# AlbertoEsc/PyFaceAnalysis

Measured on AMD Instinct MI355X. Metric: 128x128 sub-images/sec through 11L HiGSFA net, higher is better.
Workload: dtype f32; 1 GPU; configs[1]: U11L-128 (11-layer net, trained random-init weights), 4096 synthetic 128x128 sub-images per GPU per step, float32 input resident in HBM, first 20 slow features out; rows_per_gpu=4096, global_rows=4096, plan=fused, parallelism=row-shard x1

## Files before the change

### pyfaceanalysis_amd/csrc/hg_fused.hip

```cpp
#include <hip/hip_runtime.h>

#include <algorithm>
#include <cmath>
#include <cstdlib>
#include <map>
#include <sstream>
#include <tuple>

#include "hg_fused_dev.hpp"

namespace hg {

namespace {

using namespace fused;

#ifndef HG_A_PINGPONG
#define HG_A_PINGPONG 1
#endif
#ifdef HIGSFA_DIAG
#define HG_HOT(blk) ((P.whatif & 1) ? ((blk) & 1) : (blk))
#else
#define HG_HOT(blk) (blk)
#endif
// ... 348 lines not shown
#pragma unroll
                                for (int t = 0; t < T; ++t) z[t] = MFMA16(a1[k][r], bf[k][t][r], z[t]);
                            }
                    }
                }
            }
        }
        if (rem1) {
#pragma unroll
            for (int t = 0; t < T; ++t) add_rem4(z[t], d4[t]);
        }
        if (!P.has_exp) {
#pragma unroll
            for (int t = 0; t < T; ++t)
                if (tile[t] < P.n_tiles) P.out[((size_t)tile[t] * P.nb_out + node * P.mto + w) * 64 + lane] = z[t];
            return;
        }
        for (int fi = 0; fi < nf; ++fi) {
            const int fk = (P.funcp >> (4 * fi)) & 15;
            const float ex = P.expo[fi];
#pragma unroll
            for (int t = 0; t < T; ++t) smem[((fi * mt1n + w) * T + t) * 64 + lane] = apply_func_uniform(fk, ex, z[t]);
        }
    } else if (!P.has_exp) {
        return;
    }
    __syncthreads();
    if (w >= mt2n) return;
#pragma unroll
    for (int t = 0; t < T; ++t) d4[t] = f32x4{0.f, 0.f, 0.f, 0.f};
    f32x4 y[T];
    {
        const f32x4 bb = *(const f32x4*)(bnode + (mt1n + w) * 16);
#pragma unroll
        for (int t = 0; t < T; ++t) y[t] = bb;
    }
#pragma unroll
    for (int k = 0; k < KB; ++k) {
        if (k >= k2n) continue;
        const int mt1 = k / nf, fi = k - mt1 * nf;
        const int nk = (P.nk2p[mt1] >> (4 * fi)) & 15;
        f32x4 e[T];
#pragma unroll
        for (int t = 0; t < T; ++t) e[t] = smem[((fi * mt1n + mt1) * T + t) * 64 + lane];
        if (REM && rem2) {
#pragma unroll
            for (int r = 0; r < 4; ++r)
                if (r < nk) {
#pragma unroll
                    for (int t = 0; t < T; ++t) d4[t] = MFMA4(a2[k][r], e[t][r], d4[t]);
                }
        } else if (nk == 4) {
#pragma unroll
            for (int r = 0; r < 4; ++r)
#pragma unroll
                for (int t = 0; t < T; ++t) y[t] = MFMA16(a2[k][r], e[t][r], y[t]);
        } else {
#pragma unroll
            for (int r = 0; r < 4; ++r)
                if (r < nk) {
#pragma unroll
                    for (int t = 0; t < T; ++t) y[t] = MFMA16(a2[k][r], e[t][r], y[t]);
                }
        }
    }
    if (rem2) {
#pragma unroll
        for (int t = 0; t < T; ++t) add_rem4(y[t], d4[t]);
    }
    if (REM && P.pack_base > 0) {
        if (rem2) {
            const int slot = __builtin_amdgcn_readfirstlane(P.pack_slot[node]);
#pragma unroll
            for (int t = 0; t < T; ++t)
                if (tile[t] < P.n_tiles) *packed_slot_ptr(P, tile[t], slot, lane) = y[t][0];
        } else {
#pragma unroll
            for (int t = 0; t < T; ++t)
                if (tile[t] < P.n_tiles) P.out[((size_t)tile[t] * P.nb_out + node * (mt2n - 1) + w) * 64 + lane] = y[t];
        }
        return;
    }
#pragma unroll
    for (int t = 0; t < T; ++t)
        if (tile[t] < P.n_tiles) P.out[((size_t)tile[t] * P.nb_out + node * P.mto + w) * 64 + lane] = y[t];
}

template <typename YT>
__global__ void k_unpack(const float* __restrict__ act, int nb, const int32_t* __restrict__ col_base, YT* __restrict__ y,
                         int64_t ldy, int64_t n, int cols) {
    int64_t total = n * cols;
    for (int64_t idx = (int64_t)blockIdx.x * blockDim.x + threadIdx.x; idx < total; idx += (int64_t)gridDim.x * blockDim.x) {
        int64_t row = idx / cols;
        int c = (int)(idx - row * cols);
        int64_t tile = row >> 4;
        int jj = (int)(row & 15);
        y[row * ldy + c] = (YT)act[tile * nb * 256 + col_base[c] + jj * 4];
    }
}


template <int MT1, int MT2>
StageFn pick_stage_t(int T) {
    if (T == 2) return k_stage<MT1, MT2, 2>;
    return k_stage<MT1, MT2, 1>;
}
template <int MT1>
StageFn pick_stage_m2(int mt2, int T) {
    switch (mt2) {
        case 1: return pick_stage_t<MT1, 1>(T);
        case 2: return pick_stage_t<MT1, 2>(T);
        case 3: return pick_stage_t<MT1, 3>(T);
        default: return pick_stage_t<MT1, 4>(T);
    }
}
StageFn pick_stage(int mt1, int mt2, int T, bool rem = false, int kbf = 0, bool fs = false, int pk = -1) {
    if (pk >= 0) {
        if (pk == 1 && kbf == 3 && T == 2 && rem && mt1 == 3 && mt2 == 3) return fs ? (StageFn)k_stage<3, 3, 2, false, true, 3, true, 1> : (StageFn)k_stage<3, 3, 2, false, true, 3, false, 1>;
        if (pk == 1 && kbf == 3 && T == 2 && rem && mt1 == 2 && mt2 == 2) return (StageFn)k_stage<2, 2, 2, false, true, 3, false, 1>;
        return nullptr;
    }
    if (fs) {
        if (kbf == 3 && T == 2 && rem && mt1 == 3 && mt2 == 3) return (StageFn)k_stage<3, 3, 2, false, true, 3, true>;
        if (kbf == 4 && T == 2 && !rem && mt1 == 3 && mt2 == 3) return (StageFn)k_stage<3, 3, 2, false, false, 4, true>;
        if (kbf == 0 && !rem && mt1 == 4 && mt2 == 4) return T == 2 ? (StageFn)k_stage<4, 4, 2, false, false, 0, true> : (StageFn)k_stage<4, 4, 1, false, false, 0, true>;
    }
    if (kbf == 4 && T == 2) {
        if (rem && mt1 == 3 && mt2 == 3) return (StageFn)k_stage<3, 3, 2, false, true, 4>;
        if (rem && mt1 == 2 && mt2 == 2) return (StageFn)k_stage<2, 2, 2, false, true, 4>;
        if (!rem && mt1 == 3 && mt2 == 3) return (StageFn)k_stage<3, 3, 2, false, false, 4>;
        if (!rem && mt1 == 2 && mt2 == 2) return (StageFn)k_stage<2, 2, 2, false, false, 4>;
    }
    if (kbf == 3 && T == 2) {
        if (rem && mt1 == 3 && mt2 == 3) return (StageFn)k_stage<3, 3, 2, false, true, 3>;
        if (rem && mt1 == 2 && mt2 == 2) return (StageFn)k_stage<2, 2, 2, false, true, 3>;
    }
    if (rem) {
        if (mt1 == 3 && mt2 == 3) return T == 2 ? (StageFn)k_stage<3, 3, 2, false, true> : (StageFn)k_stage<3, 3, 1, false, true>;
        if (mt1 == 2 && mt2 == 2) return T == 2 ? (StageFn)k_stage<2, 2, 2, false, true> : (StageFn)k_stage<2, 2, 1, false, true>;
    }
    switch (mt1) {
        case 1: return pick_stage_m2<1>(mt2, T);
        case 2: return pick_stage_m2<2>(mt2, T);
        case 3: return pick_stage_m2<3>(mt2, T);
        default: return pick_stage_m2<4>(mt2, T);
    }
}


constexpr int kWeightLdsKiB = 64;

struct StageDev {
    DevBuf afrag, bias, kb1tab, chunks, runs, piece, koff, kmean, kcol, gcol, etab, pack_slot;
};
struct SubRunDev {
    DevBuf nodes[kMaxTail], tab[kMaxTail];
};

struct WorkQueue {
    DevBuf ctr;
    uint32_t base = 0;
};

constexpr int kMaxLanes = 2;
struct Lane {
    DevBuf bufA, bufB;
    int64_t cap_rows = 0;
    WorkQueue wq_front, wq_direct, wq_direct_wg;
    int32_t* err_host = nullptr;
    int32_t* err_dev = nullptr;
};

class FusedExecutor : public Executor {
public:
    explicit FusedExecutor(std::unique_ptr<const FusedPlan> plan) : plan_(std::move(plan)) {}

    int plan_kind() const override { return HG_PLAN_FUSED; }
    int n_stages() const override { return (int)plan_->stages.size() + 1; }
    std::string stage_name(int i) const override {
        if (i < (int)plan_->stages.size()) return plan_->stages[i].name;
        return plan_->tail_begin >= 0 ? std::string("row-major y written by the top-of-hierarchy launch (no unpack pass)")
                                      : std::string("fused unpack (fragment order -> row-major y)");
    }
    std::string describe() const override {
        std::ostringstream os;
        os << "plan: FUSED (fragment-order activations, v_mfma_f32_16x16x4_f32)\n";
        for (int i = 0; i < n_stages(); ++i) os << "  [" << i << "] " << stage_name(i) << "\n";
        return os.str();
    }
    int64_t weight_bytes() const override {
        int64_t t = 0;
        for (auto& s : plan_->stages) t += (int64_t)(s.afrag.size() + s.bias.size()) * 4;
        return t;
    }
    int64_t padded_flops_per_row() const override { return plan_->padded_flops_given; }
    int64_t workspace_bytes() const override {
        int64_t t = 0;
        for (int l = 0; l < n_lanes_; ++l) t += (int64_t)(lanes_[l].bufA.bytes + lanes_[l].bufB.bytes);
        return t;
    }

    void to_device() override {
        dev_.resize(plan_->stages.size());
        for (size_t si = 0; si < dev_.size(); ++si) {
            const HostStage& s = plan_->stages[si];
            StageDev& d = dev_[si];
            d.afrag.upload(s.afrag.data(), s.afrag.size() * 4);
            d.bias.upload(s.bias.data(), s.bias.size() * 4);
            if (!s.kb1tab.empty()) d.kb1tab.upload(s.kb1tab.data(), s.kb1tab.size() * 4);
            if (!s.gcol.empty()) d.gcol.upload(s.gcol.data(), s.gcol.size() * 4);
            if (!s.etab.empty()) d.etab.upload(s.etab.data(), s.etab.size() * 4);
            if (!s.pack_slot.empty()) d.pack_slot.upload(s.pack_slot.data(), s.pack_slot.size() * 4);
            if (!s.chunks.empty()) {
                d.chunks.upload(s.chunks.data(), s.chunks.size() * sizeof(DChunk));
                d.runs.upload(s.runs.data(), s.runs.size() * sizeof(DRun));
                d.piece.upload(s.piece_col.data(), s.piece_col.size() * 4);
                d.koff.upload(s.koff.data(), s.koff.size() * 4);
                d.kmean.upload(s.kmean.data(), s.kmean.size() * 4);
                if (!s.kcol.empty()) d.kcol.upload(s.kcol.data(), s.kcol.size() * 4);
            }
        }
        sub_dev_.resize(plan_->sub_runs.size());
        for (size_t ri = 0; ri < sub_dev_.size(); ++ri) {
            const SubRun& r = plan_->sub_runs[ri];
            for (int k = 0; k < r.len; ++k) {
                sub_dev_[ri].nodes[k].upload(r.nodes[k].data(), r.nodes[k].size() * 4);
                if (k > 0) sub_dev_[ri].tab[k].upload(r.tab[k].data(), r.tab[k].size() * 4);
            }
        }
        d_col_base_.upload(plan_->col_base.data(), plan_->col_base.size() * 4);
        d_col_of_.upload(plan_->col_of.data(), plan_->col_of.size() * 4);
        int dev = 0;
        hipDeviceProp_t prop;
        if (hipGetDevice(&dev) == hipSuccess && hipGetDeviceProperties(&prop, dev) == hipSuccess && prop.multiProcessorCount > 0)
            n_cus_ = prop.multiProcessorCount;
    }

    void reserve(int64_t rows) override {
        for (int l = 0; l < n_lanes_; ++l) reserve_lane(lanes_[l], rows);
    }

    bool set_lanes(int n) override {
        if (n < 1 || n > kMaxLanes) return false;
        for (int l = n; l < n_lanes_; ++l) release_lane(lanes_[l]);
        for (int l = n_lanes_; l < n; ++l) reserve_lane(lanes_[l], lanes_[0].cap_rows);
        n_lanes_ = n;
        return true;
    }
    int lanes() const override { return n_lanes_; }

    void run(const void* x, int x_dtype, int64_t n, int64_t ldx, void* y, int y_dtype, int64_t y_cols, int64_t ldy,
             hipStream_t st, hipEvent_t* ev) override {
        run_in(lanes_[0], x, x_dtype, n, ldx, y, y_dtype, y_cols, ldy, st, ev);
    }
    void run_lane(int lane, const void* x, int x_dtype, int64_t n, int64_t ldx, void* y, int y_dtype, int64_t y_cols, int64_t ldy,
                  hipStream_t st) override {
        if (lane < 0 || lane >= n_lanes_) fail(HG_ERR_ARG, "lane %d outside 0..%d", lane, n_lanes_ - 1);
        run_in(lanes_[lane], x, x_dtype, n, ldx, y, y_dtype, y_cols, ldy, st, nullptr);
    }

    void run_in(Lane& L, const void* x, int x_dtype, int64_t n, int64_t ldx, void* y, int y_dtype, int64_t y_cols, int64_t ldy,
                hipStream_t st, hipEvent_t* ev) {
        check_device_error();
        if (dev_.size() != plan_->stages.size()) fail(HG_ERR_STATE, "fused: the plan is not on a device");
        if (n > L.cap_rows) {
            if (n_lanes_ > 1) HG_HIP(hipStreamSynchronize(st));
            reserve_lane(L, n);
        }
        run_range(L, x, x_dtype, n, ldx, y, y_dtype, y_cols, ldy, st, ev);
    }

    void run_range(Lane& L, const void* x, int x_dtype, int64_t n, int64_t ldx, void* y, int y_dtype, int64_t y_cols, int64_t ldy,
                   hipStream_t st, hipEvent_t* ev) {
        const int n_tiles = (int)((n + 15) / 16);
        const int sub_set = plan_->pick_sub_set(n_tiles);
        int e = 0;
        auto record = [&](int k) {
            if (ev)
                for (int i = 0; i < k; ++i) HG_HIP(hipEventRecord(ev[e++], st));
        };
        record(1);
        f32x4* cur = (f32x4*)L.bufA.p;
        f32x4* nxt = (f32x4*)L.bufB.p;
        for (int si = 0; si < (int)plan_->stages.size(); ++si) {
            if (plan_->tail_begin >= 0 && si == plan_->tail_start(n_tiles)) {
                launch_top(si, cur, n_tiles, y, y_dtype, y_cols, ldy, n, st);
                record((int)plan_->stages.size() + 1 - si);
                HG_HIP(hipGetLastError());
                return;
            }
            const SubRun* sr = nullptr;
            const SubRunDev* sd = nullptr;
            for (size_t ri = 0; ri < plan_->sub_runs.size(); ++ri) {
                const SubRun& r = plan_->sub_runs[ri];
                if (r.begin == si && r.set == sub_set && plan_->sub_run_pays(r, n_tiles)) { sr = &r; sd = &sub_dev_[ri]; }
            }
            if (sr) {
                launch_subtrees(*sr, *sd, cur, nxt, n_tiles, st);
                std::swap(cur, nxt);
                record(sr->len);
                si += sr->len - 1;
                continue;
            }
            const HostStage& s = plan_->stages[si];
            const StageDev& d = dev_[si];
            StageParams P = stage_params(s, d, cur, nxt, n_tiles);
            int covered = 1;
            if (s.kind == 1)
                launch_im2frag(x, x_dtype, ldx, n, n_tiles, s.nb_out, (const int32_t*)d.gcol.p, nxt, vec4_ok(s, x, ldx, x_dtype) ? 1 : 0, st);
            else if (s.kind == 2)
                launch_igsfa(s, P, n_tiles, si, st);
            else if (s.from_x)
                covered = launch_front(L, s, d, P, x, x_dtype, ldx, n, n_tiles, cur, st) ? 2 : 1;
            else if (s.kind == 3)
                launch_prod(s, d, P, n_tiles, st);
            else if (!launch_splitm(s, P, n_tiles, st))
                launch_stage(s, P, n_tiles, si, st);
            if (covered == 1) std::swap(cur, nxt);
            record(covered);
            si += covered - 1;
        }
        launch_unpack(cur, n, y, y_dtype, y_cols, ldy, st);
        record(1);
        HG_HIP(hipGetLastError());
    }

    void release() override {
        for (Lane& L : lanes_) release_lane(L);
        n_lanes_ = 1;
        d_col_base_.free();
        d_col_of_.free();
        sub_dev_.clear();
        dev_.clear();
    }

private:
    void reserve_lane(Lane& L, int64_t rows) {
        int64_t tiles = (rows + 15) / 16;
        size_t need = (size_t)tiles * plan_->max_nb * 1024;
        L.bufA.alloc(need);
        L.bufB.alloc(need);
        L.cap_rows = std::max(L.cap_rows, tiles * 16);
    }
    void release_lane(Lane& L) {
        L.bufA.free();
        L.bufB.free();
        L.wq_front.ctr.free();
        L.wq_direct.ctr.free();
        L.wq_direct_wg.ctr.free();
        L.wq_front.base = L.wq_direct.base = L.wq_direct_wg.base = 0;
        if (L.err_host) (void)hipHostFree(L.err_host);
        L.err_host = nullptr;
        L.err_dev = nullptr;
        L.cap_rows = 0;
    }

    int resident_blocks(StageFn fn, int threads, size_t lds) {
        set_lds_limit(fn, lds);
        auto key = std::make_tuple((const void*)fn, threads, lds);
        auto it = occ_.find(key);
        if (it != occ_.end()) return it->second;
        int nb = 0;
        if (hipOccupancyMaxActiveBlocksPerMultiprocessor(&nb, (const void*)fn, threads, lds) != hipSuccess || nb < 1) nb = 1;
        occ_[key] = nb;
        return nb;
    }

    uint32_t* work_counters(WorkQueue& q, int n, hipStream_t st) {
        const size_t need = (size_t)n * 64;
        if (q.ctr.bytes < need) {
            q.ctr.alloc(std::max<size_t>(need, 64 * 1024));
            HG_HIP(hipMemsetD32Async((hipDeviceptr_t)q.ctr.p, (int)plan_->opt.wq_start, q.ctr.bytes / 4, st));
            q.base = plan_->opt.wq_start;
        }
        return (uint32_t*)q.ctr.p;
    }

    int32_t* device_error_word(Lane& L) {
        if (!L.err_host) {
            HG_HIP(hipHostMalloc((void**)&L.err_host, 64, hipHostMallocMapped));
            *L.err_host = 0;
            HG_HIP(hipHostGetDevicePointer((void**)&L.err_dev, L.err_host, 0));
        }
        return L.err_dev;
    }
    void check_errors() override { check_device_error(); }
    void check_device_error() {
        for (const Lane& L : lanes_)
            if (L.err_host && *(volatile int32_t*)L.err_host != 0)
                fail(HG_ERR_DEVICE, "fused: a bounded poll in a persistent kernel ran out (code %d); the features of that call are invalid", (int)*L.err_host);
    }

    void set_lds_limit(StageFn fn, size_t bytes) {
        if (bytes <= 64 * 1024) return;
        if (bytes > 160 * 1024) fail(HG_ERR_FORMAT, "fused: a node needs %zu bytes of LDS (> 160 KiB)", bytes);
        auto it = lds_set_.find((const void*)fn);
        if (it != lds_set_.end() && it->second >= bytes) return;
        HG_HIP(hipFuncSetAttribute((const void*)fn, hipFuncAttributeMaxDynamicSharedMemorySize, (int)(160 * 1024)));
        lds_set_[(const void*)fn] = 160 * 1024;
    }

    StageParams stage_params(const HostStage& hs, const StageDev& d, const f32x4* in, f32x4* out, int n_tiles) const {
        StageParams R{};
        R.afrag = (const f32x4*)d.afrag.p;
        R.bias = (const float*)d.bias.p;
        R.kb1tab = (const int2*)d.kb1tab.p;
        R.in = in;
        R.out = out;
        R.n_nodes = hs.n_nodes;
        R.kb1 = hs.kb1;
        R.nf = hs.nf;
        R.has_exp = hs.has_exp ? 1 : 0;
        R.node_blocks = hs.node_blocks;
        R.bias_floats = hs.bias_floats;
        R.n_tiles = n_tiles;
        R.nb_in = hs.nb_in;
        R.nb_out = hs.nb_out;
        R.mto = hs.mto;
        R.pack_base = hs.pack_out ? hs.n_nodes * (hs.mto - 1) : 0;
        R.pack_soa = hs.pack_soa ? 1 : 0;
        R.pack_in = hs.pack_in;
        R.pack_slot = (const int32_t*)d.pack_slot.p;
        R.a4x4 = hs.rem4 ? 1 : 0;
        R.sum_in = hs.sum_in ? 1 : 0;
        R.n_kids = hs.n_kids;
        for (int fi = 0; fi < hs.nf; ++fi) {
            R.funcp |= (uint32_t)hs.funcs[fi].kind << (4 * fi);
            R.expo[fi] = (float)hs.funcs[fi].expo;
            for (int mt1 = 0; mt1 < hs.mt1; ++mt1) R.nk2p[mt1] |= (uint32_t)hs.nk2[mt1][fi] << (4 * fi);
        }
        return R;
    }

    static bool vec4_ok(const HostStage& s, const void* x, int64_t ldx, int x_dtype) {
        const size_t esz = dtype_size(x_dtype), valign = x_dtype == HG_U8 ? 4 : 16;
        return s.vec_ok && ldx % 4 == 0 && ((uintptr_t)x % valign) == 0 && (ldx * esz) % valign == 0;
    }

    struct Shape {
        int nw, T;
    };
    template <size_t N>
    static Shape sweep_shape(const int (&cand)[N][2], int n_tiles, int n_groups) {
        Shape sh{4, 1};
        for (auto& c : cand) {
            const int64_t tg = (n_tiles + c[0] * c[1] - 1) / (c[0] * c[1]);
            if (c[0] * c[1] <= n_tiles && tg * n_groups >= 256) {
                sh = {c[0], c[1]};
                break;
            }
        }
        while (sh.nw * sh.T > std::max(n_tiles, 1) && sh.nw > 1) sh.nw >>= 1;
        return sh;
    }

    static int sweep_tile_parts(int n_groups, int tile_groups, int occ) {
        const double capacity = 256.0 * occ;
        const int64_t g8 = (int64_t)(n_groups + 7) / 8 * 8;
        int tile_parts = 1;
        double best = 1e300;
        for (int pp = 1; pp <= tile_groups; ++pp) {
            const double rounds = std::ceil(g8 * pp / capacity);
            const double cost = rounds * (0.35 + (double)((tile_groups + pp - 1) / pp));
            if (cost < best - 1e-9) {
                best = cost;
                tile_parts = pp;
            }
        }
        return tile_parts;
    }

    void launch_top(int si, const f32x4* in, int n_tiles, void* y, int y_dtype, int64_t y_cols, int64_t ldy, int64_t n, hipStream_t st) {
        TailParams TP = tail_params(si, in, n_tiles, y, y_dtype, y_cols, ldy, n);
        const int T = (n_tiles >= 512 && tail_waves(TP) <= 8 && tail_lds_bytes(TP, 2) <= (size_t)160 * 1024) ? 2 : 1;
#ifdef HIGSFA_DIAG
        const bool stamped = plan_->opt.stamp_stage == si;
        if (stamped) tail_stamps_begin(TP, (size_t)((n_tiles + T - 1) / T), st);
#endif
        launch_tail(TP, T, st);
#ifdef HIGSFA_DIAG
        if (stamped) tail_stamps_report("top-of-hierarchy launch", si, TP.n_stages, (size_t)((n_tiles + T - 1) / T), st);
#endif
    }

    void launch_subtrees(const SubRun& sr, const SubRunDev& sd, const f32x4* in, f32x4* out, int n_tiles, hipStream_t st) {
        TailParams TP = subtree_params(sr, sd, in, out, n_tiles);
#ifdef HIGSFA_DIAG
        const bool stamped = plan_->opt.stamp_stage == sr.begin;
        if (stamped) tail_stamps_begin(TP, (size_t)sr.n * n_tiles, st);
#endif
        launch_subtree(TP, st);
#ifdef HIGSFA_DIAG
        if (stamped) tail_stamps_report("sub-tree launch", sr.begin, TP.n_stages, (size_t)sr.n * n_tiles, st);
#endif
    }

    void launch_igsfa(const HostStage& s, StageParams& P, int n_tiles, int si, hipStream_t st) {
        if (s.ig_folded && s.n_nodes <= 8 && s.nf <= 2 && s.kb1 <= 8 && (int64_t)s.n_nodes * n_tiles <= 16384) {
            P.ig_folded = 1;
            launch_igfold_split(P, s.mt2, n_tiles, st);
            return;
        }
        const size_t ig_lds = (size_t)s.node_blocks * 1024 + (size_t)s.bias_floats * 4 + (size_t)s.kb1 * 8;
        int nwt = 1, T = 1;
        static const int cand[][2] = {{12, 2}, {8, 2}, {4, 2}};
        for (auto& c : cand) {
            if (c[0] == 12 && (s.ig_folded || !(s.kb1 == 5 || s.kb1 == 6))) continue;
            const int64_t tg = (n_tiles + c[0] * c[1] - 1) / (c[0] * c[1]);
            if (c[0] * c[1] <= std::max(n_tiles, 1) && tg * s.n_nodes >= 256) {
                nwt = c[0];
                T = c[1];
                break;
            }
        }
        if (nwt == 1 && T == 1) {
            T = n_tiles >= 2 ? 2 : 1;
            nwt = n_tiles >= 8 ? 4 : n_tiles >= 4 ? 2 : 1;
        }
        const bool ig_fs = s.ig_folded && s.nf == 2 && s.funcs[0].kind == E_IDENTITY && s.funcs[1].kind == E_ABS_POW && !plan_->opt.no_fspec;
        StageFn fn = s.ig_folded ? pick_igfold(s.mt2, T, ig_fs) : pick_igsfa(s.mt1, s.mt2, T, s.kb1);
        const int ig_occ = resident_blocks(fn, std::max(nwt, 4) * 64, ig_lds);
        const int nw = std::max(nwt, 4);
        P.nodes_per_wg = nwt;
        P.ig_has_lr = s.ig_has_lr ? 1 : 0;
        P.ig_folded = s.ig_folded ? 1 : 0;
        P.nk2p[0] = 0;
        for (int ms = 0; ms < s.mt1; ++ms) P.nk2p[0] |= (uint32_t)s.ig_nks[ms] << (4 * ms);
        P.tile_groups = (n_tiles + nwt * T - 1) / (nwt * T);
        const int npg = 1;
        P.nodes_per_group = npg;
        P.n_chunks = (s.n_nodes + npg - 1) / npg;
        P.tile_parts = std::max(1, std::min(P.tile_groups, 256 * ig_occ / std::max(1, P.n_chunks)));
        set_lds_limit(fn, ig_lds);
        if (plan_->opt.debug) fprintf(stderr, "[igsfa stage %d] nodes %d kb1 %d shape %dx%d occ %d lds %zu tile_groups %d parts %d\n", si, s.n_nodes, s.kb1, nwt, T, ig_occ, ig_lds, P.tile_groups, P.tile_parts);
        hipLaunchKernelGGL(fn, (unsigned)(P.n_chunks * P.tile_parts), nw * 64, ig_lds, st, P);
    }

    bool launch_front(Lane& L, const HostStage& s, const StageDev& d, StageParams& P, const void* x, int x_dtype, int64_t ldx, int64_t n, int n_tiles, f32x4* out1,
                      hipStream_t st) {
        P.chunks = (const DChunk*)d.chunks.p;
        P.runs = (const DRun*)d.runs.p;
        P.piece_col = (const int2*)d.piece.p;
        P.koff = (const int32_t*)d.koff.p;
        P.kmean = (const float*)d.kmean.p;
        P.kcol = (const int32_t*)d.kcol.p;
        P.x = x;
        P.ldx = ldx;
        P.n_rows = n;
        P.lds_stride = s.lds_stride;
        P.nk_last = s.nk_last;
        P.contig4 = s.contig4 ? 1 : 0;
        P.n_chunks = (int)s.chunks.size();
        P.vec4 = vec4_ok(s, x, ldx, x_dtype) ? 1 : 0;
        const int T = (n_tiles >= 4 && s.mt1 * s.mt2 <= 4) ? 4 : 1;
        const int groups = (n_tiles + T - 1) / T;
        const size_t lds_bytes = (size_t)T * 16 * s.lds_stride * 4;
        bool rem4 = false, fspec = false;
        if (plan_->fuse01) {
            rem4 = plan_->stages[1].rem4 || (plan_->stages[1].p_max <= 20 && plan_->stages[1].s_max <= 20 && plan_->stages[1].nk2[1][0] <= 1 &&
                                       plan_->stages[1].nk2[1][1] <= 1 && !plan_->opt.no_rem4);
            auto id_pow = [](const HostStage& hs) { return hs.nf == 2 && hs.funcs[0].kind == E_IDENTITY && hs.funcs[1].kind == E_ABS_POW; };
            fspec = id_pow(s) && id_pow(plan_->stages[1]) && !plan_->opt.no_fspec;
        }
        const int FT = stage01p_tiles(rem4, fspec);
        if (plan_->fuse01 && P.vec4 && n_tiles >= FT) {
            StageParams Q = stage_params(plan_->stages[1], dev_[1], nullptr, out1, n_tiles);
            const size_t esz = dtype_size(x_dtype);
            const bool direct = fspec && rem4 && s.direct_ok && plan_->stages[1].pack_out && (int64_t)16 * ldx * (int64_t)esz + 2048 < 0x7fffffffll && s.max_chunk_nodes <= 8 && !plan_->opt.no_direct;
            const bool wgq = !plan_->opt.no_wgq;
            StageFn2 fn = direct ? pick_stage01d(x_dtype, false, wgq) : pick_stage01p(x_dtype, false, rem4, fspec);
            const int thr01 = 64 * std::max(1, (s.max_chunk_nodes + 1) / 2);
            const size_t lds2 = direct ? (size_t)4 * 160 * 4 + 32 * 4 + (size_t)4 * 256 * 4
                                       : (size_t)(kDoubleBuffer01 ? 2 : 1) * FT * 16 * s.lds_stride * 4 + (size_t)(thr01 / 64) * 160 * 4 + 16;
            const int groups2 = (n_tiles + FT - 1) / FT;
            const int occ = resident_blocks((StageFn)fn, thr01, lds2);
            P.tile_parts = std::max(1, std::min(groups2, 256 * occ / std::max(1, P.n_chunks)));
            if (plan_->opt.debug) fprintf(stderr, "[front] occ %d threads %d lds %zu chunks %d tile_parts %d\n", occ, thr01, lds2, P.n_chunks, P.tile_parts);
#ifdef HIGSFA_DIAG
            if (plan_->opt.stamp_stage == 0 && x_dtype == HG_F32) {
                fn = direct ? pick_stage01d(HG_F32, true, wgq) : pick_stage01p(HG_F32, true, rem4, fspec);
                stamps_begin(P, P.n_chunks * P.tile_parts, 12, st);
            }
#endif
            P.err = device_error_word(L);
            {
                WorkQueue& wq = direct ? (wgq ? L.wq_direct_wg : L.wq_direct) : L.wq_front;
                P.work_ctr = work_counters(wq, direct && !wgq ? plan_->stages[1].n_nodes : P.n_chunks, st);
                P.work_base = wq.base;
                wq.base += (uint32_t)groups2;
            }
#ifdef HIGSFA_DIAG
            if (const char* e = getenv("HIGSFA_WHATIF")) P.whatif = atoi(e);
#endif
            hipLaunchKernelGGL(fn, (unsigned)(P.n_chunks * P.tile_parts), thr01, lds2, st, P, Q);
#ifdef HIGSFA_DIAG
            if (P.stamps) front_stamps_report(P.n_chunks, st);
#endif
            return true;
        }
        const bool persistent = T == 4 && P.vec4 && s.contig4 && s.has_exp && s.mt1 == 1 && s.mt2 == 1 && s.kb1 == 1 &&
                                s.nf <= 2 && s.max_chunk_nodes <= 16 && 64 * s.max_chunk_pieces <= 8 * 512;
        if (persistent) {
            StageFn fn = pick_stage0p(x_dtype);
            const int occ = resident_blocks(fn, 512, lds_bytes);
            P.tile_parts = std::max(1, std::min(groups, 256 * occ / std::max(1, P.n_chunks)));
            hipLaunchKernelGGL(fn, (unsigned)(P.n_chunks * P.tile_parts), 512, lds_bytes, st, P);
        } else {
            const int64_t blocks = (int64_t)groups * P.n_chunks;
            if (blocks > 0x7fffffffll) fail(HG_ERR_ARG, "batch too large");
            StageFn fn = pick_stage0(s.mt1, s.mt2, T, x_dtype);
            set_lds_limit(fn, lds_bytes);
            hipLaunchKernelGGL(fn, (unsigned)blocks, T == 4 ? 512 : 256, lds_bytes, st, P);
        }
        return false;
    }

    bool launch_splitm(const HostStage& s, const StageParams& P, int n_tiles, hipStream_t st) {
        const int T = n_tiles >= 2 * 256 / std::max(1, s.n_nodes) ? 2 : 1;
        const int groups = (n_tiles + T - 1) / T;
        const int64_t wgs = (int64_t)groups * s.n_nodes;
        if (!(s.kind == 0 && (!s.rem4 || s.mt1 == s.mt2) && (s.rem4 || !s.pack_out) && s.mt1 * s.nf <= 8 &&
              (s.n_nodes <= plan_->opt.splitm_max_nodes ? (int64_t)s.n_nodes * n_tiles <= 8192 : wgs <= plan_->opt.splitm_max_wgs)))
            return false;
        const int nwv = std::max(s.mt1, s.has_exp ? s.mt2 : 1);
        const size_t lds_bytes = (size_t)std::max(1, s.nf) * s.mt1 * T * 1024;
        const unsigned grid = (unsigned)(groups * s.n_nodes);
        if (s.rem4) {
            if (T == 2) hipLaunchKernelGGL((k_stage_splitm<2, true>), grid, nwv * 64, lds_bytes, st, P, s.mt1, s.mt2);
            else hipLaunchKernelGGL((k_stage_splitm<1, true>), grid, nwv * 64, lds_bytes, st, P, s.mt1, s.mt2);
        } else if (T == 2)
            hipLaunchKernelGGL(k_stage_splitm<2>, grid, nwv * 64, lds_bytes, st, P, s.mt1, s.mt2);
        else
            hipLaunchKernelGGL(k_stage_splitm<1>, grid, nwv * 64, lds_bytes, st, P, s.mt1, s.mt2);
        return true;
    }

    void launch_stage(const HostStage& s, StageParams& P, int n_tiles, int si, hipStream_t st) {
        const int npg = std::max(1, std::min(s.n_nodes, (s.sum_in ? plan_->opt.sum_lds_kib : kWeightLdsKiB) / std::max(1, s.node_blocks)));
        const int n_groups = (s.n_nodes + npg - 1) / npg;
        static const int shapes[][2] = {{8, 2}, {8, 1}, {4, 2}, {4, 1}};
        const Shape sh = sweep_shape(shapes, n_tiles, n_groups);
        const int nw = sh.nw, T = sh.T;
        const int tile_groups = (n_tiles + nw * T - 1) / (nw * T);
        const size_t lds_bytes = (size_t)npg * s.node_blocks * 1024 + (size_t)npg * s.bias_floats * 4 + (size_t)npg * s.kb1 * 8;
        const int kbf = (T == 2 && s.mt1 == s.mt2 && (s.mt1 == 2 || s.mt1 == 3)) ? (s.kb1 == 4 ? 4 : (s.kb1 == 3 && s.rem4 ? 3 : 0)) : 0;
        const bool fs = s.has_exp && s.nf == 2 && s.funcs[0].kind == E_IDENTITY && s.funcs[1].kind == E_ABS_POW && !plan_->opt.no_fspec;
        StageFn fn = s.pk_kbi >= 0 ? (kbf == 3 ? pick_stage(s.mt1, s.mt2, T, s.rem4, kbf, fs, s.pk_kbi) : nullptr) : pick_stage(s.mt1, s.mt2, T, s.rem4, kbf, fs);
        if (!fn) fn = pick_stage(s.mt1, s.mt2, T, s.rem4, 0, false);
        if (s.sum_in) fn = pick_stage_sum(s.mt1, s.mt2, T, fs);
        const int tile_parts = sweep_tile_parts(n_groups, tile_groups, resident_blocks(fn, nw * 64, lds_bytes));
        P.nodes_per_group = npg;
        P.nodes_per_wg = npg;
        P.n_chunks = n_groups;
        P.pair_chunks = (s.pack_out && !s.pack_soa && npg == 2 && n_groups % 16 == 0) ? 1 : 0;
        P.tile_groups = tile_groups;
        P.tile_parts = tile_parts;
        const int64_t blocks = (int64_t)((P.n_chunks + 7) / 8) * 8 * tile_parts;
        if (blocks > 0x7fffffffll) fail(HG_ERR_ARG, "batch too large");
#ifdef HIGSFA_DIAG
        const bool stamp_kbf3 = s.mt1 == 3 && s.mt2 == 3 && T == 2 && s.rem4 && kbf == 3;
        if (plan_->opt.stamp_stage == si && !s.sum_in && (stamp_kbf3 || (s.mt1 == s.mt2 && (s.mt1 == 4 || s.mt1 == 3) && T == 2 && !s.rem4 && kbf == 0))) {
            fn = stamp_kbf3 ? (StageFn)k_stage<3, 3, 2, true, true, 3> : s.mt1 == 4 ? (StageFn)k_stage<4, 4, 2, true> : (StageFn)k_stage<3, 3, 2, true>;
            stamps_begin(P, (int)blocks, 8, st);
        }
#endif
        set_lds_limit(fn, lds_bytes);
#ifdef HIGSFA_DIAG
        if (const char* e = getenv("HIGSFA_WHATIF")) P.whatif = atoi(e);
#endif
        hipLaunchKernelGGL(fn, (unsigned)blocks, nw * 64, lds_bytes, st, P);
#ifdef HIGSFA_DIAG
        if (P.stamps) stage_stamps_report(si, blocks, nw, st);
#endif
    }

    void launch_unpack(const f32x4* in, int64_t n, void* y, int y_dtype, int64_t y_cols, int64_t ldy, hipStream_t st) {
        const HostStage& last = plan_->stages.back();
        unsigned grid = (unsigned)std::min<int64_t>((n * y_cols + 255) / 256, 4096);
        if (y_dtype == HG_F32)
            hipLaunchKernelGGL(k_unpack<float>, grid, 256, 0, st, (const float*)in, last.nb_out, (const int32_t*)d_col_base_.p,
                               (float*)y, ldy, n, (int)y_cols);
        else if (y_dtype == HG_F64)
            hipLaunchKernelGGL(k_unpack<double>, grid, 256, 0, st, (const float*)in, last.nb_out, (const int32_t*)d_col_base_.p,
                               (double*)y, ldy, n, (int)y_cols);
        else
            fail(HG_ERR_ARG, "output dtype must be f32 or f64");
    }

    void launch_prod(const HostStage& s, const StageDev& d, StageParams& P, int n_tiles, hipStream_t st) {
        static const int shapes[][2] = {{8, 2}, {4, 2}, {4, 1}};
        const Shape sh = sweep_shape(shapes, n_tiles, s.n_nodes);
        const int nw = sh.nw, T = sh.T;
        const size_t zs_bytes = (size_t)nw * T * s.mt1 * 1024, et_bytes = (size_t)s.neb * 128;
        const size_t per_node = (size_t)s.node_blocks * 1024 + (size_t)s.bias_floats * 4 + (size_t)s.kb1 * 8;
        const size_t fixed = zs_bytes + et_bytes;
        const int npg = (int)std::max<size_t>(1, std::min<size_t>(s.n_nodes, fixed + per_node <= 52 * 1024 ? (52 * 1024 - fixed) / per_node : 1));
        const int n_groups = (s.n_nodes + npg - 1) / npg;
        const int tile_groups = (n_tiles + nw * T - 1) / (nw * T);
        const size_t lds_bytes = (size_t)npg * per_node + et_bytes + zs_bytes;
        StageFn fn = pick_prod(s.mt1, s.mt2, T);
        const int tile_parts = sweep_tile_parts(n_groups, tile_groups, resident_blocks(fn, nw * 64, lds_bytes));
        P.nodes_per_group = npg;
        P.nodes_per_wg = npg;
        P.n_chunks = n_groups;
        P.tile_groups = tile_groups;
        P.tile_parts = tile_parts;
        P.etab = (const int2*)d.etab.p;
        P.neb = s.neb;
        P.nk_last = s.nk_last;
        P.has_clip = s.has_clip ? 1 : 0;
        P.clip_lo = s.clip_lo;
        P.clip_hi = s.clip_hi;
        const int64_t blocks = (int64_t)((n_groups + 7) / 8) * 8 * tile_parts;
        if (blocks > 0x7fffffffll) fail(HG_ERR_ARG, "batch too large");
        set_lds_limit(fn, lds_bytes);
        hipLaunchKernelGGL(fn, (unsigned)blocks, nw * 64, lds_bytes, st, P);
    }

#ifdef HIGSFA_DIAG
    void tail_stamps_begin(TailParams& TP, size_t blocks, hipStream_t st) {
        stamp_buf_.alloc(blocks * 16 * 16 * 8);
        HG_HIP(hipMemsetAsync(stamp_buf_.p, 0, stamp_buf_.bytes, st));
        TP.stamps = (unsigned long long*)stamp_buf_.p;
    }
    void tail_stamps_report(const char* what, int si, int n_layers, size_t blocks, hipStream_t st) {
        HG_HIP(hipStreamSynchronize(st));
        std::vector<unsigned long long> h(blocks * 16 * 16);
        HG_HIP(hipMemcpy(h.data(), stamp_buf_.p, h.size() * 8, hipMemcpyDeviceToHost));
        unsigned long long t0 = ~0ull;
        for (size_t i = 0; i < h.size(); i += 16)
            if (h[i]) t0 = std::min(t0, h[i]);
        static const char* names[5] = {"loads in", "expanded", "barrier 1", "outputs stored", "barrier 2"};
        double sum[16] = {}, mx[16] = {}, cnt[16] = {};
        for (size_t i = 0; i < h.size(); i += 16)
            for (int k = 0; k < 16; ++k)
                if (h[i + k]) {
                    const double us = (double)(h[i + k] - t0) * 0.01;
                    sum[k] += us; cnt[k] += 1; mx[k] = std::max(mx[k], us);
                }
        fprintf(stderr, "[stamp stage %d] %s, %zu workgroups: us after the first wave's entry, mean (max) over the waves that took part\n", si, what, blocks);
        fprintf(stderr, "[stamp stage %d]   entry %.2f (%.2f)\n", si, cnt[0] ? sum[0] / cnt[0] : 0.0, mx[0]);
        for (int l = 0; l < n_layers; ++l) {
            fprintf(stderr, "[stamp stage %d]   layer %d:", si, l);
            for (int k = 0; k < 5; ++k) {
                const int q = 1 + 5 * l + k;
                fprintf(stderr, "  %s %.2f (%.2f; %.0f waves)", names[k], cnt[q] ? sum[q] / cnt[q] : 0.0, mx[q], cnt[q]);
            }
            fprintf(stderr, "\n");
        }
    }
    void stamps_begin(StageParams& P, int blocks, int words, hipStream_t st) {
        stamp_blocks_ = blocks;
        stamp_buf_.alloc((size_t)blocks * 8 * words * 8);
        HG_HIP(hipMemsetAsync(stamp_buf_.p, 0, stamp_buf_.bytes, st));
        P.stamps = (unsigned long long*)stamp_buf_.p;
    }
    void front_stamps_report(int n_chunks, hipStream_t st) {
        HG_HIP(hipStreamSynchronize(st));
        std::vector<unsigned long long> h((size_t)stamp_blocks_ * 8 * 12);
        HG_HIP(hipMemcpy(h.data(), stamp_buf_.p, h.size() * 8, hipMemcpyDeviceToHost));
        double a[7] = {0, 0, 0, 0, 0, 0, 0}, nwv = 0;
        unsigned long long lo[3] = {~0ull, ~0ull, ~0ull}, hi[3] = {0, 0, 0};
        for (size_t i = 0; i < h.size(); i += 12)
            if (h[i + 4]) {
                for (int k = 0; k < 7; ++k) a[k] += h[i + k];
                nwv += 1;
                for (int k = 0; k < 3; ++k) { lo[k] = std::min(lo[k], h[i + 7 + k]); hi[k] = std::max(hi[k], h[i + 7 + k]); }
            }
        {
            double xs[8][4] = {}, ps[16][3] = {};
            for (size_t i = 0, w = 0; i < h.size(); i += 12, ++w)
                if (h[i + 4]) {
                    const int blk = (int)(w / 8), xc = blk % 8, pt = std::min(15, blk / n_chunks);
                    const double life = (h[i + 9] - h[i + 8]) * 0.01, clk = (double)h[i + 4] / (double)h[i + 5] * 100.0;
                    xs[xc][0] += 1; xs[xc][1] += life; xs[xc][2] = std::max(xs[xc][2], life); xs[xc][3] += clk;
                    ps[pt][0] += 1; ps[pt][1] += life; ps[pt][2] = std::max(ps[pt][2], life);
                }
            for (int k = 0; k < 8; ++k)
                if (xs[k][0] > 0) fprintf(stderr, "[stamp stage 0+1] xcd %d: waves %.0f loop us mean %.1f max %.1f clock %.0f MHz\n", k, xs[k][0], xs[k][1] / xs[k][0], xs[k][2], xs[k][3] / xs[k][0]);
            for (int k = 0; k < 16; ++k)
                if (ps[k][0] > 0) fprintf(stderr, "[stamp stage 0+1] part %d: waves %.0f loop us mean %.1f max %.1f\n", k, ps[k][0], ps[k][1] / ps[k][0], ps[k][2]);
        }
        fprintf(stderr, "[stamp stage 0+1] wall clock, us after the first wave's entry: entries until %.1f, loop starts %.1f..%.1f, ends %.1f..%.1f\n",
                (hi[0] - lo[0]) * 0.01, (lo[1] - lo[0]) * 0.01, (hi[1] - lo[0]) * 0.01, (lo[2] - lo[0]) * 0.01, (hi[2] - lo[0]) * 0.01);
        fprintf(stderr, "[stamp stage 0+1] waves %.0f clock %.0f MHz lifetime %.1f us, iterations %.1f; cycles per iteration: "
                        "lds-write+barrier %.0f, fetch issue %.0f, layer0 %.0f, layer1+store %.0f (sum %.0f)\n",
                nwv, a[4] / a[5] * 100.0, a[5] / nwv / 100.0, a[6] / nwv, a[0] / a[6], a[1] / a[6], a[2] / a[6], a[3] / a[6],
                (a[0] + a[1] + a[2] + a[3]) / a[6]);
    }
    void stage_stamps_report(int si, int64_t blocks, int nw, hipStream_t st) {
        HG_HIP(hipStreamSynchronize(st));
        std::vector<unsigned long long> h((size_t)stamp_blocks_ * 8 * 8);
        HG_HIP(hipMemcpy(h.data(), stamp_buf_.p, h.size() * 8, hipMemcpyDeviceToHost));
        double c = 0, g1 = 0, tl = 0, all = 0, it = 0, nwv = 0, rt = 0;
        unsigned long long lo0 = ~0ull, hi0 = 0, lo1 = ~0ull, hi1 = 0;
        std::vector<unsigned long long> ends;
        for (size_t i = 0; i < h.size(); i += 8)
            if (h[i + 3]) {
                c += h[i]; g1 += h[i + 1]; tl += h[i + 2]; all += h[i + 3]; it += h[i + 4]; rt += h[i + 5]; nwv += 1;
                lo0 = std::min(lo0, h[i + 6]); hi0 = std::max(hi0, h[i + 6]); lo1 = std::min(lo1, h[i + 7]); hi1 = std::max(hi1, h[i + 7]);
                ends.push_back(h[i + 7]);
            }
        std::sort(ends.begin(), ends.end());
        if (!ends.empty())
            fprintf(stderr, "[stamp stage %d] wall clock, us after the first wave's start: starts until %.1f, ends %.1f (10%%) %.1f (50%%) %.1f (90%%) %.1f (last); grid %lld blocks x %d waves\n",
                    (int)si, (hi0 - lo0) * 0.01, (ends[ends.size() / 10] - lo0) * 0.01, (ends[ends.size() / 2] - lo0) * 0.01,
                    (ends[ends.size() * 9 / 10] - lo0) * 0.01, (hi1 - lo0) * 0.01, (long long)blocks, nw);
        fprintf(stderr, "[stamp stage %d] in-kernel clock %.0f MHz, wave lifetime %.1f us\n", (int)si, all / rt * 100.0, rt / nwv / 100.0);
        fprintf(stderr, "[stamp stage %d] waves %.0f  avg cycles/wave: total %.0f  copy+barrier %.0f  gemm1 %.0f  tail %.0f  node-iterations %.1f  (per iteration: gemm1 %.0f tail %.0f)\n",
                (int)si, nwv, all / nwv, c / nwv, g1 / nwv, tl / nwv, it / nwv, g1 / it, tl / it);
    }
#endif

    static void fill_tail_stage(TailStage& S, const HostStage& hs, const StageDev& d) {
        S.afrag = (const f32x4*)d.afrag.p;
        S.bias = (const float*)d.bias.p;
        S.kb1tab = (const int2*)d.kb1tab.p;
        S.n_nodes = hs.n_nodes;
        S.kb1 = hs.kb1;
        S.nf = hs.nf;
        S.has_exp = hs.has_exp ? 1 : 0;
        S.node_blocks = hs.node_blocks;
        S.bias_floats = hs.bias_floats;
        S.nb_out = hs.nb_out;
        S.mto = hs.mto;
        S.mt1 = hs.mt1;
        S.mt2 = hs.mt2;
        S.sum_in = hs.sum_in ? 1 : 0;
        S.n_kids = hs.n_kids;
        for (int fi = 0; fi < hs.nf; ++fi) {
            S.funcp |= (uint32_t)hs.funcs[fi].kind << (4 * fi);
            S.expo[fi] = (float)hs.funcs[fi].expo;
            for (int mt1 = 0; mt1 < hs.mt1; ++mt1) S.nk2p[mt1] |= (uint32_t)hs.nk2[mt1][fi] << (4 * fi);
        }
    }

    TailParams subtree_params(const SubRun& sr, const SubRunDev& sd, const f32x4* in, f32x4* out, int n_tiles) {
        const int sub_begin_ = sr.begin, sub_len_ = sr.len, sub_n_ = sr.n, sub_act_blocks_ = sr.act_blocks, sub_e_blocks_ = sr.e_blocks;
        TailParams TP{};
        TP.n_stages = sub_len_;
        for (int k = 0; k < sub_len_; ++k) {
            fill_tail_stage(TP.st[k], plan_->stages[sub_begin_ + k], dev_[sub_begin_ + k]);
            TP.st[k].n_nodes /= sub_n_;
            TP.sub_nodes[k] = (const int32_t*)sd.nodes[k].p;
            if (k > 0) TP.st[k].kb1tab = (const int2*)sd.tab[k].p;
        }
        TP.in = in;
        TP.out_frag = out;
        TP.n_sub = sub_n_;
        TP.nb_out_frag = plan_->stages[sub_begin_ + sub_len_ - 1].nb_out;
        TP.n_tiles = n_tiles;
        TP.nb_in = plan_->stages[sub_begin_].nb_in;
        TP.act_blocks = sub_act_blocks_;
        TP.e_blocks = sub_e_blocks_;
        return TP;
    }

    TailParams tail_params(int begin, const f32x4* in, int n_tiles, void* y, int y_dtype, int64_t y_cols, int64_t ldy, int64_t n) {
        TailParams TP{};
        const int ns = (int)plan_->stages.size();
        TP.n_stages = ns - begin;
        for (int k = 0; k < TP.n_stages; ++k) {
            fill_tail_stage(TP.st[k], plan_->stages[begin + k], dev_[begin + k]);
        }
        TP.in = in;
        TP.y = y;
        TP.col_of = (const int32_t*)d_col_of_.p;
        TP.ldy = ldy;
        TP.n_rows = n;
        TP.y_cols = (int32_t)y_cols;
        TP.y_f64 = y_dtype == HG_F64 ? 1 : 0;
        if (y_dtype != HG_F32 && y_dtype != HG_F64) fail(HG_ERR_ARG, "output dtype must be f32 or f64");
        TP.n_tiles = n_tiles;
        TP.nb_in = plan_->stages[begin].nb_in;
        TP.act_blocks = plan_->tail_act_blocks;
        TP.e_blocks = plan_->tail_e_blocks;
        return TP;
    }

    const std::unique_ptr<const FusedPlan> plan_;
    std::vector<StageDev> dev_;
    std::vector<SubRunDev> sub_dev_;
    DevBuf d_col_base_, d_col_of_;
    Lane lanes_[kMaxLanes];
    int n_lanes_ = 1;
#ifdef HIGSFA_DIAG
    DevBuf stamp_buf_;
    int stamp_blocks_ = 0;
#endif
    std::map<const void*, size_t> lds_set_;
    std::map<std::tuple<const void*, int, size_t>, int> occ_;
    int n_cus_ = 256;
};

}

std::unique_ptr<Executor> make_fused_executor(const TNode& root, std::string* why_not) {
    fused::FusedOptions opt = fused::FusedOptions::from_env();
    opt.hoist = getenv("HIGSFA_NO_HOIST") == nullptr;
    auto plan = fused::build_fused_plan(root, opt, why_not);
    if (!plan) return nullptr;
    return std::make_unique<FusedExecutor>(std::move(plan));
}

}
```

### pyfaceanalysis_amd/csrc/hg_fused_dev.hpp

```cpp
#pragma once
#include <hip/hip_runtime.h>

#include <algorithm>

#include "hg_fused_plan.hpp"

namespace hg {
namespace fused {

typedef float f32x4 __attribute__((ext_vector_type(4)));
typedef int i32x4 __attribute__((ext_vector_type(4)));

constexpr bool kDoubleBuffer01 = true;

struct StageParams {
    const f32x4* afrag;
    const float* bias;
    const int2* kb1tab;
    const f32x4* in;
    f32x4* out;
    int32_t n_nodes, kb1, nf, has_exp;
    int32_t node_blocks, bias_floats, n_tiles, nb_in, nb_out, mto;
    int32_t nodes_per_group, nodes_per_wg, n_chunks, tile_groups, tile_parts;
    uint32_t nk2p[kMaxMT];
    uint32_t funcp;
    float expo[kMaxFuncs];
    const DChunk* chunks;
    const DRun* runs;
    const int2* piece_col;
    const int32_t* koff;
    const float* kmean;
    const int32_t* kcol;
    const void* x;
    int64_t ldx, n_rows;
    int32_t lds_stride, nk_last, vec4, contig4;
    int32_t ig_has_lr, ig_folded;
    unsigned long long* stamps;
    int32_t pack_base;
    int32_t pack_soa;
    int32_t pair_chunks;
    int32_t pack_in;
    const int32_t* pack_slot;
    int32_t a4x4;
    const int2* etab;
    int32_t neb, has_clip;
    float clip_lo, clip_hi;
    uint32_t* work_ctr;
    uint32_t work_base;
    int32_t* err;
    int32_t whatif;
    int32_t sum_in, n_kids;
};

__device__ __forceinline__ unsigned long long stamp_now() {
    unsigned long long t;
    asm volatile("s_memtime %0\n\ts_waitcnt lgkmcnt(0)" : "=s"(t)::"memory");
    return t;
}

__device__ __forceinline__ float pow_abs(float v, float p) {
    return __builtin_amdgcn_exp2f(p * __builtin_amdgcn_logf(__builtin_fabsf(v)));
}

__device__ __forceinline__ f32x4 pow_abs4(f32x4 z, float p) {
    f32x4 e;
#pragma unroll
    for (int r = 0; r < 4; ++r) e[r] = pow_abs(z[r], p);
    return e;
}

__device__ __forceinline__ f32x4 apply_func(int func, float expo, f32x4 z) {
    f32x4 e;
    if (func == (int)E_IDENTITY) {
        e = z;
    } else if (func == (int)E_ABS_POW) {
#pragma unroll
        for (int r = 0; r < 4; ++r) e[r] = pow_abs(z[r], expo);
    } else {
#pragma unroll
        for (int r = 0; r < 4; ++r) e[r] = __builtin_copysignf(pow_abs(z[r], expo), z[r]);
    }
    return e;
}

__device__ __forceinline__ f32x4 apply_func_uniform(int func, float expo, f32x4 z) {
    if (func == (int)E_IDENTITY) return z;
    asm volatile("" ::: "memory");
    f32x4 e;
#pragma unroll
    for (int r = 0; r < 4; ++r) {
        const float p = pow_abs(z[r], expo);
        e[r] = func == (int)E_SIGNED_POW ? __builtin_copysignf(p, z[r]) : p;
    }
    return e;
}

#ifndef HG_POW_PREFETCH
#define HG_POW_PREFETCH 1
#endif
#define MFMA16(a, b, c) __builtin_amdgcn_mfma_f32_16x16x4f32((a), (b), (c), 0, 0, 0)

template <int MT, int T, bool KOUT = false, typename WP>
__device__ __forceinline__ void gemm_block(WP wp, const f32x4 (&b)[T], f32x4 (&acc)[MT][T], int nk, int r0 = 0) {
#ifndef HG_GEMM4_KOUTER
    if constexpr (MT >= 4 && T >= 2 && !KOUT) {
#pragma unroll
        for (int mt = 0; mt < MT; ++mt) {
            const f32x4 a = wp[mt * 64];
#pragma unroll
            for (int r = 0; r < 4; ++r)
                if (r >= r0 && r < nk) {
#pragma unroll
                    for (int t = 0; t < T; ++t) acc[mt][t] = MFMA16(a[r], b[t][r], acc[mt][t]);
                }
        }
        return;
    }
#endif
    {
        f32x4 a[MT];
#pragma unroll
        for (int mt = 0; mt < MT; ++mt) a[mt] = wp[mt * 64];
#pragma unroll
        for (int r = 0; r < 4; ++r)
            if (r >= r0 && r < nk) {
#pragma unroll
                for (int mt = 0; mt < MT; ++mt)
#pragma unroll
                    for (int t = 0; t < T; ++t) acc[mt][t] = MFMA16(a[mt][r], b[t][r], acc[mt][t]);
            }
    }
}

template <int MT, int T>
__device__ __forceinline__ void gemm_block_regs(const f32x4 (&a)[MT], const f32x4 (&b)[T], f32x4 (&acc)[MT][T], int nk, int r0 = 0) {
#pragma unroll
    for (int r = 0; r < 4; ++r)
        if (r >= r0 && r < nk) {
#pragma unroll
            for (int mt = 0; mt < MT; ++mt)
#pragma unroll
                for (int t = 0; t < T; ++t) acc[mt][t] = MFMA16(a[mt][r], b[t][r], acc[mt][t]);
        }
}

#define MFMA4(a, b, c) __builtin_amdgcn_mfma_f32_4x4x1f32((a), (b), (c), 0, 0, 0)

__device__ __forceinline__ float rem4_total(f32x4 d) {
    const auto p = __builtin_amdgcn_permlane16_swap(__float_as_uint(d[0]), __float_as_uint(d[1]), false, false);
    const float t = __uint_as_float(p[0]) + __uint_as_float(p[1]);
    const auto q = __builtin_amdgcn_permlane16_swap(__float_as_uint(d[2]), __float_as_uint(d[3]), false, false);
    const float u = __uint_as_float(q[0]) + __uint_as_float(q[1]);
    const auto r = __builtin_amdgcn_permlane32_swap(__float_as_uint(t), __float_as_uint(u), false, false);
    return __uint_as_float(r[0]) + __uint_as_float(r[1]);
}

__device__ __forceinline__ float rem4_total_lds(f32x4 d, float* scratch, int lane) {
    *(f32x4*)(scratch + lane * 4) = d;
    const int g = lane >> 4, j = lane & 15;
    const float v0 = scratch[(0 * 16 + j) * 4 + g], v1 = scratch[(1 * 16 + j) * 4 + g], v2 = scratch[(2 * 16 + j) * 4 + g], v3 = scratch[(3 * 16 + j) * 4 + g];
    return (v0 + v1) + (v2 + v3);
}

__device__ __forceinline__ void add_rem4(f32x4& acc, f32x4 d) { acc[0] += rem4_total(d); }

template <int MT, int T, typename WP>
__device__ __forceinline__ void gemm_block_rem(WP wp, const f32x4 (&b)[T], f32x4 (&acc)[MT][T], f32x4 (&d4)[T], int nk, int r0 = 0) {
    f32x4 a[MT];
#pragma unroll
    for (int mt = 0; mt < MT; ++mt) a[mt] = wp[mt * 64];
#pragma unroll
    for (int r = 0; r < 4; ++r)
        if (r >= r0 && r < nk) {
#pragma unroll
            for (int mt = 0; mt < MT - 1; ++mt)
#pragma unroll
                for (int t = 0; t < T; ++t) acc[mt][t] = MFMA16(a[mt][r], b[t][r], acc[mt][t]);
#pragma unroll
            for (int t = 0; t < T; ++t) d4[t] = MFMA4(a[MT - 1][r], b[t][r], d4[t]);
        }
}

template <int T, bool TWO>
__device__ __forceinline__ void load_kblock_soa(const StageParams& P, const uint32_t (&row)[T], int sb, int y, int lane, f32x4 (&b)[T]) {
    const int s0 = y >> 16, s1 = min(s0 + 1, 3);
#pragma unroll
    for (int t = 0; t < T; ++t) {
        const float* f = (const float*)(P.in + (size_t)(row[t] + (uint32_t)sb) * 64) + lane;
        b[t] = f32x4{f[s0 * 64], f[s1 * 64], 0.f, 0.f};
    }
    if constexpr (!TWO) {
        if ((y & 255) > 2) {
            const int s2 = min(s0 + 2, 3), s3 = min(s0 + 3, 3);
#pragma unroll
            for (int t = 0; t < T; ++t) {
                const float* f = (const float*)(P.in + (size_t)(row[t] + (uint32_t)sb) * 64) + lane;
                b[t][2] = f[s2 * 64];
                b[t][3] = f[s3 * 64];
            }
        }
    }
}

template <int T>
// ... 4 lines not shown
    }
#pragma unroll
    for (int t = 0; t < T; ++t) b[t] = P.in[(size_t)(row[t] + (uint32_t)sb) * 64 + lane];
}

__device__ __forceinline__ float* packed_slot_ptr(const StageParams& P, int tile, int slot, int lane) {
    float* blk = (float*)(P.out + ((size_t)tile * P.nb_out + P.pack_base + (slot >> 2)) * 64);
    return P.pack_soa ? blk + (slot & 3) * 64 + lane : blk + lane * 4 + (slot & 3);
}

template <int MT1, int MT2, int T, bool REM = false, bool FS = false, bool LEAN = false, typename WP, typename BP>
__device__ __forceinline__ void node_tail(const StageParams& P, WP wA2, BP b2, int node, f32x4 (&z)[MT1][T],
                                          const int (&tile)[T], int lane, float* rscr = nullptr) {
    const int g = lane >> 4;
    const int out_blk = node * P.mto;
#ifdef HIGSFA_DIAG
    const bool no_store = (P.whatif & 2) != 0;
#else
    constexpr bool no_store = false;
#endif
    if (!P.has_exp) {
#pragma unroll
        for (int mt = 0; mt < MT1; ++mt)
#pragma unroll
            for (int t = 0; t < T; ++t)
                if (tile[t] < P.n_tiles) P.out[((size_t)tile[t] * P.nb_out + out_blk + mt) * 64 + lane] = z[mt][t];
        return;
    }
    f32x4 y[MT2][T];
#pragma unroll
    for (int mt = 0; mt < MT2; ++mt) {
        f32x4 bb = *(const f32x4*)(b2 + mt * 16 + g * 4);
#pragma unroll
        for (int t = 0; t < T; ++t) y[mt][t] = bb;
    }
    const float ex0 = P.expo[0], ex1 = P.expo[1], ex2 = P.expo[2], ex3 = P.expo[3];
    const uint32_t funcp = P.funcp;
    const int nf = P.nf;
    f32x4 d4[T];
#pragma unroll
    for (int t = 0; t < T; ++t) d4[t] = f32x4{0.f, 0.f, 0.f, 0.f};
    if constexpr (FS) {
#pragma unroll
        for (int mt1 = 0; mt1 < MT1; ++mt1) {
            const uint32_t nkp = P.nk2p[mt1];
            const int nk0 = nkp & 15, nk1 = (nkp >> 4) & 15;
            if constexpr (REM) {
                gemm_block_rem<MT2, T>(wA2 + (mt1 * 2) * MT2 * 64, z[mt1], y, d4, nk0);
                f32x4 e[T];
#pragma unroll
                for (int t = 0; t < T; ++t) e[t] = pow_abs4(z[mt1][t], ex1);
                gemm_block_rem<MT2, T>(wA2 + (mt1 * 2 + 1) * MT2 * 64, e, y, d4, nk1);
            } else if constexpr (LEAN) {
                gemm_block<MT2, T>(wA2 + (mt1 * 2) * MT2 * 64, z[mt1], y, nk0);
                f32x4 e[T];
#pragma unroll
                for (int t = 0; t < T; ++t) e[t] = pow_abs4(z[mt1][t], ex1);
                gemm_block<MT2, T>(wA2 + (mt1 * 2 + 1) * MT2 * 64, e, y, nk1);
            } else if constexpr (!HG_POW_PREFETCH) {
                gemm_block<MT2, T, true>(wA2 + (mt1 * 2) * MT2 * 64, z[mt1], y, nk0);
                f32x4 e[T];
#pragma unroll
                for (int t = 0; t < T; ++t) e[t] = pow_abs4(z[mt1][t], ex1);
                gemm_block<MT2, T, true>(wA2 + (mt1 * 2 + 1) * MT2 * 64, e, y, nk1);
            } else {
                gemm_block<MT2, T, true>(wA2 + (mt1 * 2) * MT2 * 64, z[mt1], y, nk0);
                f32x4 ap[MT2];
#pragma unroll
                for (int mt = 0; mt < MT2; ++mt) ap[mt] = (wA2 + (mt1 * 2 + 1) * MT2 * 64)[mt * 64];
                f32x4 e[T];
#pragma unroll
                for (int t = 0; t < T; ++t) e[t] = pow_abs4(z[mt1][t], ex1);
                gemm_block_regs<MT2, T>(ap, e, y, nk1);
            }
        }
    } else
#pragma unroll
    for (int mt1 = 0; mt1 < MT1; ++mt1) {
        const uint32_t nkp = P.nk2p[mt1];
        for (int fi = 0; fi < nf; ++fi) {
            const int nk = (nkp >> (4 * fi)) & 15;
            if (nk == 0) continue;
            f32x4 e[T];
            const int fk = (funcp >> (4 * fi)) & 15;
            const float ex = fi == 0 ? ex0 : (fi == 1 ? ex1 : (fi == 2 ? ex2 : ex3));
#pragma unroll
            for (int t = 0; t < T; ++t) e[t] = apply_func(fk, ex, z[mt1][t]);
            if constexpr (REM) gemm_block_rem<MT2, T>(wA2 + (mt1 * nf + fi) * MT2 * 64, e, y, d4, nk);
            else gemm_block<MT2, T>(wA2 + (mt1 * nf + fi) * MT2 * 64, e, y, nk);
        }
    }
    if constexpr (REM) {
#pragma unroll
        for (int t = 0; t < T; ++t) {
            if (rscr) y[MT2 - 1][t][0] += rem4_total_lds(d4[t], rscr, lane);
            else add_rem4(y[MT2 - 1][t], d4[t]);
        }
        if (P.pack_base > 0) {
#pragma unroll
            for (int mt = 0; mt < MT2 - 1; ++mt)
#pragma unroll
                for (int t = 0; t < T; ++t)
                    if (tile[t] < P.n_tiles && !no_store) P.out[((size_t)tile[t] * P.nb_out + node * (MT2 - 1) + mt) * 64 + lane] = y[mt][t];
            const int slot = __builtin_amdgcn_readfirstlane(P.pack_slot[node]);
#pragma unroll
            for (int t = 0; t < T; ++t)
                if (tile[t] < P.n_tiles && !no_store)
                    *packed_slot_ptr(P, tile[t], slot, lane) = y[MT2 - 1][t][0];
            return;
        }
    }
#pragma unroll
    for (int mt = 0; mt < MT2; ++mt)
#pragma unroll
        for (int t = 0; t < T; ++t)
            if (tile[t] < P.n_tiles && !no_store) P.out[((size_t)tile[t] * P.nb_out + out_blk + mt) * 64 + lane] = y[mt][t];
}


struct TailStage {
    const f32x4* afrag;
    const float* bias;
    const int2* kb1tab;
    int32_t n_nodes, kb1, nf, has_exp, node_blocks, bias_floats, nb_out, mto, mt1, mt2;
    int32_t sum_in, n_kids;
    uint32_t nk2p[kMaxMT], funcp;
    float expo[kMaxFuncs];
};
struct TailParams {
    TailStage st[kMaxTail];
    const f32x4* in;
    void* y;
    const int32_t* col_of;
    int64_t ldy, n_rows;
    int32_t y_cols, y_f64;
    int32_t n_stages, n_tiles, nb_in;
    int32_t act_blocks, e_blocks;
    f32x4* out_frag;
    const int32_t* sub_nodes[kMaxTail];
    int32_t n_sub, nb_out_frag;
    unsigned long long* stamps;
};
size_t tail_lds_bytes(const TailParams& P, int T);
int tail_waves(const TailParams& P);
void launch_tail(const TailParams& P, int T, hipStream_t st);
void launch_subtree(const TailParams& P, hipStream_t st);


typedef void (*StageFn)(StageParams);
typedef void (*StageFn2)(StageParams, StageParams);

StageFn pick_stage0(int mt1, int mt2, int T, int x_dtype);
StageFn pick_stage0p(int x_dtype);
StageFn2 pick_stage01p(int x_dtype, bool stamp, bool rem4, bool fspec);
int stage01p_tiles(bool rem4, bool fspec);
StageFn2 pick_stage01d(int x_dtype, bool stamp, bool wgq);
StageFn pick_igsfa(int ms, int mo, int T, int kb1);
StageFn pick_igfold(int mo, int T, bool fs = false);
StageFn pick_prod(int mt1, int mt2, int T);
StageFn pick_stage_sum(int mt1, int mt2, int T, bool fs);
void launch_igfold_split(const StageParams& P, int mo, int n_tiles, hipStream_t st);
void launch_im2frag(const void* x, int x_dtype, int64_t ldx, int64_t n_rows, int n_tiles, int nb, const int32_t* gcol, f32x4* out,
                    int vec4, hipStream_t st);

template <typename XT> struct Vec4Load;
typedef uint32_t u32x4_t __attribute__((ext_vector_type(4)));
constexpr int kBufferFlags = 0x00020000;
template <> struct Vec4Load<float> {
    static __device__ __forceinline__ f32x4 ld(const float* p) { return *(const f32x4*)p; }
    static __device__ __forceinline__ f32x4 buf(__amdgpu_buffer_rsrc_t r, uint32_t off) {
        return __builtin_bit_cast(f32x4, __builtin_amdgcn_raw_buffer_load_b128(r, off, 0, 0));
    }
};
template <> struct Vec4Load<uint8_t> {
    static __device__ __forceinline__ f32x4 ld(const uint8_t* p) {
        uint32_t w = *(const uint32_t*)p;
        f32x4 v;
        v[0] = (float)(w & 0xff);
        v[1] = (float)((w >> 8) & 0xff);
        v[2] = (float)((w >> 16) & 0xff);
        v[3] = (float)(w >> 24);
        return v;
    }
    static __device__ __forceinline__ f32x4 buf(__amdgpu_buffer_rsrc_t r, uint32_t off) {
        const uint32_t w = __builtin_amdgcn_raw_buffer_load_b32(r, off, 0, 0);
        return f32x4{(float)(w & 0xff), (float)((w >> 8) & 0xff), (float)((w >> 16) & 0xff), (float)(w >> 24)};
    }
};
template <> struct Vec4Load<double> {
    static __device__ __forceinline__ f32x4 ld(const double* p) {
        typedef double f64x2 __attribute__((ext_vector_type(2)));
        f64x2 a = *(const f64x2*)p, b = *(const f64x2*)(p + 2);
        f32x4 v;
        v[0] = (float)a[0];
        v[1] = (float)a[1];
        v[2] = (float)b[0];
        v[3] = (float)b[1];
        return v;
    }
    static __device__ __forceinline__ f32x4 buf(__amdgpu_buffer_rsrc_t r, uint32_t off) {
        typedef double f64x2 __attribute__((ext_vector_type(2)));
        const f64x2 a = __builtin_bit_cast(f64x2, __builtin_amdgcn_raw_buffer_load_b128(r, off, 0, 0));
        const f64x2 b = __builtin_bit_cast(f64x2, __builtin_amdgcn_raw_buffer_load_b128(r, off + 16, 0, 0));
        return f32x4{(float)a[0], (float)a[1], (float)b[0], (float)b[1]};
    }
};


}
}
```

### pyfaceanalysis_amd/csrc/hg_fused_front.hip

```cpp
#include "hg_fused_dev.hpp"

namespace hg {
namespace fused {

template <int MT1, int MT2, int T, typename XT>
__global__ void __launch_bounds__(512) k_stage0(StageParams P) {
    extern __shared__ __attribute__((aligned(16))) f32x4 smem[];
    float* lds = (float*)smem;
    const int tid = threadIdx.x, nthr = blockDim.x, lane = tid & 63, wave = tid >> 6, nw = nthr >> 6, g = lane >> 4, j = lane & 15;
    const int ci = blockIdx.x % P.n_chunks, grp = blockIdx.x / P.n_chunks;
    const DChunk ck = P.chunks[ci];
    int tile[T];
#pragma unroll
    for (int t = 0; t < T; ++t) tile[t] = grp * T + t;
    const XT* x = (const XT*)P.x;
    const int stride = P.lds_stride;
    if (P.vec4) {
        const int pps = ck.n_pieces;
        const int total = T * 16 * pps;
        constexpr int NB = 8;
        for (int base = 0; base < total; base += nthr * NB) {
            f32x4 v[NB];
            int dsto[NB];
#pragma unroll
// ... 34 lines not shown
    __syncthreads();
    for (int ni = ck.node_begin + wave; ni < ck.node_begin + ck.node_count; ni += nw) {
        const f32x4* wA1 = P.afrag + (size_t)ni * P.node_blocks * 64 + lane;
        const f32x4* wA2 = wA1 + P.kb1 * MT1 * 64;
        const float* b1 = P.bias + (size_t)ni * P.bias_floats;
        f32x4 z[MT1][T];
#pragma unroll
        for (int mt = 0; mt < MT1; ++mt) {
            f32x4 bb = *(const f32x4*)(b1 + mt * 16 + g * 4);
#pragma unroll
            for (int t = 0; t < T; ++t) z[mt][t] = bb;
        }
        for (int kbi = 0; kbi < P.kb1; ++kbi) {
            const size_t ent = ((size_t)ni * P.kb1 + kbi) * 16 + g * 4;
            const i32x4 off = *(const i32x4*)(P.koff + ent);
            const f32x4 mu = *(const f32x4*)(P.kmean + ent);
            f32x4 bf[T];
            if (P.contig4) {
#pragma unroll
                for (int t = 0; t < T; ++t) bf[t] = *(const f32x4*)(lds + (t * 16 + j) * stride + off[0]) - mu;
            } else {
#pragma unroll
                for (int t = 0; t < T; ++t) {
                    const float* base = lds + (t * 16 + j) * stride;
#pragma unroll
                    for (int r = 0; r < 4; ++r) bf[t][r] = base[off[r]] - mu[r];
                }
            }
            gemm_block<MT1, T>(wA1 + kbi * MT1 * 64, bf, z, kbi == P.kb1 - 1 ? P.nk_last : 4);
        }
        node_tail<MT1, MT2, T>(P, wA2, b1 + MT1 * 16, ni, z, tile, lane);
    }
}

template <int T, typename XT>
__global__ void __launch_bounds__(512) k_stage0p(StageParams P) {
    extern __shared__ __attribute__((aligned(16))) f32x4 smem[];
    float* lds = (float*)smem;
    constexpr int NB = 8, NPW = 2;
    const int tid = threadIdx.x, nthr = blockDim.x, lane = tid & 63, nw = nthr >> 6, g = lane >> 4, j = lane & 15;
    const int wave = __builtin_amdgcn_readfirstlane(tid >> 6);
    const int ci = blockIdx.x % P.n_chunks, part = blockIdx.x / P.n_chunks;
    const DChunk ck = P.chunks[ci];
    const XT* x = (const XT*)P.x;
    const int stride = P.lds_stride;
    const int n_groups = (P.n_tiles + T - 1) / T;
    const int pps = ck.n_pieces, total = T * 16 * pps;
    int p_col[NB], p_dst[NB];
#pragma unroll
    for (int k = 0; k < NB; ++k) {
        const int idx = k * nthr + tid;
        p_col[k] = 0;
        p_dst[k] = -1;
        if (idx < total) {
            const int sj = idx / pps, pc = idx - sj * pps;
            const int2 pcol = P.piece_col[ck.piece_begin + pc];
            p_col[k] = pcol.x;
            p_dst[k] = (sj << 24) | (sj * stride + pcol.y);
        }
    }
    int w_off[NPW];
    f32x4 w_mu[NPW], w_a1[NPW], w_a2[NPW][2], w_b1[NPW], w_b2[NPW];
    bool w_ok[NPW];
#pragma unroll
    for (int sl = 0; sl < NPW; ++sl) {
        const int nl = wave + sl * nw;
        w_ok[sl] = nl < ck.node_count;
        const int ni = ck.node_begin + (w_ok[sl] ? nl : 0);
        const size_t ent = (size_t)ni * 16 + g * 4;
        w_off[sl] = P.koff[ent];
        w_mu[sl] = *(const f32x4*)(P.kmean + ent);
        const f32x4* wp = P.afrag + (size_t)ni * P.node_blocks * 64 + lane;
        w_a1[sl] = wp[0];
        w_a2[sl][0] = wp[64];
        w_a2[sl][1] = P.nf > 1 ? wp[128] : wp[64];
        const float* bp = P.bias + (size_t)ni * P.bias_floats + g * 4;
        w_b1[sl] = *(const f32x4*)bp;
        w_b2[sl] = *(const f32x4*)(bp + 16);
    }
    const int nk1 = P.nk_last;
    const int nk2a = P.nk2p[0] & 15, nk2b = (P.nk2p[0] >> 4) & 15;
    const int fk0 = P.funcp & 15, fk1 = (P.funcp >> 4) & 15;
    const float ex0 = P.expo[0], ex1 = P.expo[1];

    auto fetch = [&](int grp, f32x4 (&v)[NB]) {
#pragma unroll
        for (int k = 0; k < NB; ++k) {
            const int64_t row = (int64_t)grp * (T * 16) + (p_dst[k] >> 24);
            if (p_dst[k] >= 0 && row < P.n_rows)
                v[k] = Vec4Load<XT>::ld(x + row * P.ldx + p_col[k]);
            else
                v[k] = f32x4{0.f, 0.f, 0.f, 0.f};
        }
    };
    f32x4 v[NB];
    if (part < n_groups) fetch(part, v);
    for (int grp = part; grp < n_groups; grp += P.tile_parts) {
#pragma unroll
        for (int k = 0; k < NB; ++k)
            if (p_dst[k] >= 0) *(f32x4*)(lds + (p_dst[k] & 0xffffff)) = v[k];
        if (tid < T * 16) lds[tid * stride + stride - 1] = 0.f;
        __syncthreads();
        if (grp + P.tile_parts < n_groups) fetch(grp + P.tile_parts, v);
        int tile[T];
#pragma unroll
        for (int t = 0; t < T; ++t) tile[t] = grp * T + t;
#pragma unroll
        for (int sl = 0; sl < NPW; ++sl) {
            if (!w_ok[sl]) continue;
            const int ni = ck.node_begin + wave + sl * nw;
            f32x4 z[1][T], y[1][T], bf[T];
#pragma unroll
            for (int t = 0; t < T; ++t) {
                bf[t] = *(const f32x4*)(lds + (t * 16 + j) * stride + w_off[sl]) - w_mu[sl];
                z[0][t] = w_b1[sl];
                y[0][t] = w_b2[sl];
            }
#pragma unroll
            for (int r = 0; r < 4; ++r)
                if (r < nk1) {
#pragma unroll
                    for (int t = 0; t < T; ++t) z[0][t] = MFMA16(w_a1[sl][r], bf[t][r], z[0][t]);
                }
            {
                f32x4 e[T];
#pragma unroll
                for (int t = 0; t < T; ++t) e[t] = apply_func(fk0, ex0, z[0][t]);
#pragma unroll
                for (int r = 0; r < 4; ++r)
                    if (r < nk2a) {
#pragma unroll
                        for (int t = 0; t < T; ++t) y[0][t] = MFMA16(w_a2[sl][0][r], e[t][r], y[0][t]);
                    }
            }
            if (P.nf > 1) {
                f32x4 e[T];
#pragma unroll
                for (int t = 0; t < T; ++t) e[t] = apply_func(fk1, ex1, z[0][t]);
#pragma unroll
                for (int r = 0; r < 4; ++r)
                    if (r < nk2b) {
#pragma unroll
                        for (int t = 0; t < T; ++t) y[0][t] = MFMA16(w_a2[sl][1][r], e[t][r], y[0][t]);
                    }
            }
#pragma unroll
            for (int t = 0; t < T; ++t)
                if (tile[t] < P.n_tiles) P.out[((size_t)tile[t] * P.nb_out + ni) * 64 + lane] = y[0][t];
        }
        __syncthreads();
    }
}

template <typename XT, bool STAMP = false, bool REM4 = false, int TT = 2, int FSPEC = 0>
__global__ void __launch_bounds__(512) __attribute__((amdgpu_waves_per_eu(TT == 2 ? 3 : TT == 1 ? 4 : 2, TT == 2 ? 3 : TT == 1 ? 4 : 2))) k_stage01p(StageParams P, StageParams Q) {
    extern __shared__ __attribute__((aligned(16))) f32x4 smem[];
    float* lds = (float*)smem;
    unsigned long long rt_entry = 0;
    if (STAMP) rt_entry = __builtin_amdgcn_s_memrealtime();
    constexpr int T = TT, NB = 2 * TT, NPW = 2;
    const int tid = threadIdx.x, nthr = blockDim.x, lane = tid & 63, g = lane >> 4, j = lane & 15;
    const int wave = __builtin_amdgcn_readfirstlane(tid >> 6);
    const int ci = blockIdx.x % P.n_chunks, part = blockIdx.x / P.n_chunks;
    const DChunk ck = P.chunks[ci];
    const XT* x = (const XT*)P.x;
    const int stride = P.lds_stride;
    const int n_groups = (P.n_tiles + T - 1) / T;
    const int pps = ck.n_pieces, total = T * 16 * pps;
    const XT* p_src[NB];
    int p_dst[NB];
#pragma unroll
    for (int k = 0; k < NB; ++k) {
        const int idx = k * nthr + tid;
        p_src[k] = x;
        p_dst[k] = -1;
        if (idx < total) {
            const int sj = idx / pps, pc = idx - sj * pps;
            const int2 pcol = P.piece_col[ck.piece_begin + pc];
            p_src[k] = x + (int64_t)sj * P.ldx + pcol.x;
            p_dst[k] = (sj << 24) | (sj * stride + pcol.y);
        }
    }
    const int64_t grp_step = (int64_t)(T * 16) * P.ldx;
    float* cst = lds + (kDoubleBuffer01 ? 2 : 1) * (T * 16 * stride) + wave * 160;
    enum { C_MU = 0, C_B1 = 2, C_B2 = 4, C_QB1 = 6, C_QB2 = 8 };
    int w_off[NPW];
    f32x4 w_a1[NPW], w_a2[NPW][2];
    const bool w_ok = 2 * wave + 1 < ck.node_count;
#pragma unroll
    for (int sl = 0; sl < NPW; ++sl) {
        const int ni = ck.node_begin + (w_ok ? 2 * wave + sl : 0);
        const size_t ent = (size_t)ni * 16 + g * 4;
        w_off[sl] = P.koff[ent];
        if (j == 0) *(f32x4*)(cst + (C_MU + sl) * 16 + g * 4) = *(const f32x4*)(P.kmean + ent);
        const f32x4* wp = P.afrag + (size_t)ni * P.node_blocks * 64 + lane;
        w_a1[sl] = wp[0];
        w_a2[sl][0] = wp[64];
        w_a2[sl][1] = P.nf > 1 ? wp[128] : wp[64];
        const float* bp = P.bias + (size_t)ni * P.bias_floats + g * 4;
        if (j == 0) {
            *(f32x4*)(cst + (C_B1 + sl) * 16 + g * 4) = *(const f32x4*)bp;
            *(f32x4*)(cst + (C_B2 + sl) * 16 + g * 4) = *(const f32x4*)(bp + 16);
        }
    }
    const int n1 = (ck.node_begin >> 1) + (w_ok ? wave : 0);
    f32x4 q_a1[2][2], q_a2[2][2][2];
    {
        const f32x4* wq = Q.afrag + (size_t)n1 * Q.node_blocks * 64 + lane;
#pragma unroll
        for (int kb = 0; kb < 2; ++kb)
#pragma unroll
            for (int mt = 0; mt < 2; ++mt) q_a1[kb][mt] = wq[(kb * 2 + mt) * 64];
        const f32x4* wq2 = wq + Q.kb1 * 2 * 64;
#pragma unroll
        for (int m1 = 0; m1 < 2; ++m1)
#pragma unroll
            for (int fi = 0; fi < 2; ++fi)
#pragma unroll
                for (int mt = 0; mt < 2; ++mt) q_a2[m1][fi][mt] = wq2[((m1 * Q.nf + (fi < Q.nf ? fi : 0)) * 2 + mt) * 64];
        const float* bq = Q.bias + (size_t)n1 * Q.bias_floats + g * 4;
#pragma unroll
        for (int mt = 0; mt < 2; ++mt)
            if (j == 0) {
                *(f32x4*)(cst + (C_QB1 + mt) * 16 + g * 4) = *(const f32x4*)(bq + mt * 16);
                *(f32x4*)(cst + (C_QB2 + mt) * 16 + g * 4) = *(const f32x4*)(bq + 32 + mt * 16);
            }
    }
    if (REM4 && !Q.a4x4) {
        const int src = ((lane & 48) | ((lane & 3) << 2)) << 2;
#pragma unroll
        for (int r = 0; r < 4; ++r) {
#pragma unroll
            for (int kb = 0; kb < 2; ++kb)
                q_a1[kb][1][r] = __int_as_float(__builtin_amdgcn_ds_bpermute(src, __float_as_int(q_a1[kb][1][r])));
#pragma unroll
            for (int m1 = 0; m1 < 2; ++m1)
#pragma unroll
                for (int fi = 0; fi < 2; ++fi)
                    q_a2[m1][fi][1][r] = __int_as_float(__builtin_amdgcn_ds_bpermute(src, __float_as_int(q_a2[m1][fi][1][r])));
        }
    }
    const int fk0 = P.funcp & 15, fk1 = (P.funcp >> 4) & 15;
    const float ex0 = P.expo[0], ex1 = P.expo[1];
    const int qfk0 = Q.funcp & 15, qfk1 = (Q.funcp >> 4) & 15;
    const float qex0 = Q.expo[0], qex1 = Q.expo[1];

    auto fetch = [&](int grp, f32x4 (&v)[NB]) {
        const int64_t goff = (int64_t)grp * grp_step;
        const int64_t rows_left = P.n_rows - (int64_t)grp * (T * 16);
#pragma unroll
        for (int k = 0; k < NB; ++k) {
            if (p_dst[k] >= 0 && (p_dst[k] >> 24) < rows_left)
                v[k] = Vec4Load<XT>::ld(p_src[k] + goff);
            else
                v[k] = f32x4{0.f, 0.f, 0.f, 0.f};
        }
    };
    f32x4 v[NB];
    int* qslot = (int*)(lds + (kDoubleBuffer01 ? 2 : 1) * (T * 16 * stride) + (nthr >> 6) * 160);
    uint32_t* qctr = P.work_ctr + (size_t)ci * 16;
    const uint32_t q_dyn = (uint32_t)(n_groups - P.tile_parts);
    auto grab_raw = [&]() -> uint32_t { return __builtin_amdgcn_atomic_inc32(qctr, 0xffffffffu, __ATOMIC_RELAXED, "agent"); };
    auto grab_group = [&](uint32_t raw) -> int {
        const uint32_t k = raw - P.work_base;
        return k < q_dyn ? (int)(P.tile_parts + k) : n_groups;
    };
    uint32_t q_raw = 0;
    bool q_more = tid == 0;
    if (q_more) q_raw = grab_raw();
    if (part < n_groups) fetch(part, v);
    const int buf_words = T * 16 * stride;
    float* lds0 = lds;
    int flip = 0;
    unsigned long long t_w = 0, t_f = 0, t_l0 = 0, t_l1 = 0, t_all0 = 0, rt0 = 0, ts = 0;
    int n_it = 0;
    if (STAMP) {
        t_all0 = stamp_now();
        rt0 = __builtin_amdgcn_s_memrealtime();
    }
    constexpr bool DEFER = REM4 && FSPEC == 1;
    f32x4 st_y0[T];
    float st_y1[T];
    int st_grp = -1;
    const int pk_slot = (REM4 && Q.pack_base > 0) ? __builtin_amdgcn_readfirstlane(Q.pack_slot[n1]) : 0;
    auto flush = [&]() {
        if (st_grp < 0) return;
#pragma unroll
        for (int t = 0; t < T; ++t) {
            const int tl = st_grp * T + t;
            if (tl < P.n_tiles) {
                Q.out[((size_t)tl * Q.nb_out + n1) * 64 + lane] = st_y0[t];
                *packed_slot_ptr(Q, tl, pk_slot, lane) = st_y1[t];
            }
        }
        st_grp = -1;
    };
    for (int grp = part; grp < n_groups;) {
        if (STAMP) ts = stamp_now();
        const int slot = flip;
        if (kDoubleBuffer01) {
            lds = lds0 + flip * buf_words;
        } else {
            __syncthreads();
        }
        flip ^= 1;
#pragma unroll
        for (int k = 0; k < NB; ++k)
            if (p_dst[k] >= 0) *(f32x4*)(lds + (p_dst[k] & 0xffffff)) = v[k];
        if (tid < T * 16) lds[tid * stride + stride - 1] = 0.f;
        if (tid == 0) {
            const int q_next = q_more ? grab_group(q_raw) : n_groups;
            q_more = q_next < n_groups;
            qslot[slot] = q_next;
        }
        __syncthreads();
        const int grp_next = __builtin_amdgcn_readfirstlane(qslot[slot]);
        if (STAMP) { unsigned long long t = stamp_now(); t_w += t - ts; ts = t; }
        if (grp_next < n_groups) fetch(grp_next, v);
        if (DEFER) flush();
        if (q_more) q_raw = grab_raw();
        if (STAMP) { unsigned long long t = stamp_now(); t_f += t - ts; ts = t; }
        if (w_ok) {
            int tile[T];
#pragma unroll
            for (int t = 0; t < T; ++t) tile[t] = grp * T + t;
            f32x4 y0[NPW][T];
#pragma unroll
            for (int sl = 0; sl < NPW; ++sl) {
                f32x4 z[T], bf[T];
                const f32x4 mu = *(const f32x4*)(cst + (C_MU + sl) * 16 + g * 4);
                const f32x4 cb1 = *(const f32x4*)(cst + (C_B1 + sl) * 16 + g * 4), cb2 = *(const f32x4*)(cst + (C_B2 + sl) * 16 + g * 4);
#pragma unroll
                for (int t = 0; t < T; ++t) {
                    bf[t] = *(const f32x4*)(lds + (t * 16 + j) * stride + w_off[sl]) - mu;
                    z[t] = cb1;
                    y0[sl][t] = cb2;
                }
#pragma unroll
                for (int r = 0; r < 4; ++r)
#pragma unroll
                    for (int t = 0; t < T; ++t) z[t] = MFMA16(w_a1[sl][r], bf[t][r], z[t]);
                {
                    f32x4 e[T];
#pragma unroll
                    for (int t = 0; t < T; ++t) e[t] = FSPEC == 1 ? z[t] : apply_func(fk0, ex0, z[t]);
#pragma unroll
                    for (int r = 0; r < 4; ++r)
#pragma unroll
                        for (int t = 0; t < T; ++t) y0[sl][t] = MFMA16(w_a2[sl][0][r], e[t][r], y0[sl][t]);
                }
                {
                    f32x4 e[T];
#pragma unroll
                    for (int t = 0; t < T; ++t) e[t] = FSPEC == 1 ? pow_abs4(z[t], ex1) : apply_func(fk1, ex1, z[t]);
#pragma unroll
                    for (int r = 0; r < 4; ++r)
#pragma unroll
                        for (int t = 0; t < T; ++t) y0[sl][t] = MFMA16(w_a2[sl][1][r], e[t][r], y0[sl][t]);
                }
            }
            if (STAMP) { unsigned long long t = stamp_now(); t_l0 += t - ts; ts = t; }
            f32x4 z1[2][T], y1[2][T];
#pragma unroll
            for (int mt = 0; mt < 2; ++mt)
#pragma unroll
                for (int t = 0; t < T; ++t) {
                    z1[mt][t] = *(const f32x4*)(cst + (C_QB1 + mt) * 16 + g * 4);
                    y1[mt][t] = *(const f32x4*)(cst + (C_QB2 + mt) * 16 + g * 4);
                }
            f32x4 d4[T];
#pragma unroll
            for (int t = 0; t < T; ++t) d4[t] = f32x4{0.f, 0.f, 0.f, 0.f};
#pragma unroll
            for (int kb = 0; kb < 2; ++kb)
#pragma unroll
                for (int r = 0; r < 4; ++r) {
#pragma unroll
                    for (int t = 0; t < T; ++t) z1[0][t] = MFMA16(q_a1[kb][0][r], y0[kb][t][r], z1[0][t]);
#pragma unroll
                    for (int t = 0; t < T; ++t) {
                        if constexpr (REM4) d4[t] = MFMA4(q_a1[kb][1][r], y0[kb][t][r], d4[t]);
                        else z1[1][t] = MFMA16(q_a1[kb][1][r], y0[kb][t][r], z1[1][t]);
                    }
                }
            if constexpr (REM4) {
#pragma unroll
                for (int t = 0; t < T; ++t) {
                    add_rem4(z1[1][t], d4[t]);
                    d4[t] = f32x4{0.f, 0.f, 0.f, 0.f};
                }
            }
#pragma unroll
            for (int fi = 0; fi < 2; ++fi) {
                f32x4 e[T];
#pragma unroll
                for (int t = 0; t < T; ++t)
                    e[t] = FSPEC == 1 ? (fi == 0 ? z1[0][t] : pow_abs4(z1[0][t], qex1)) : apply_func(fi == 0 ? qfk0 : qfk1, fi == 0 ? qex0 : qex1, z1[0][t]);
#pragma unroll
                for (int r = 0; r < 4; ++r) {
#pragma unroll
                    for (int t = 0; t < T; ++t) y1[0][t] = MFMA16(q_a2[0][fi][0][r], e[t][r], y1[0][t]);
#pragma unroll
                    for (int t = 0; t < T; ++t) {
                        if constexpr (REM4) d4[t] = MFMA4(q_a2[0][fi][1][r], e[t][r], d4[t]);
                        else y1[1][t] = MFMA16(q_a2[0][fi][1][r], e[t][r], y1[1][t]);
                    }
                }
            }
#pragma unroll
            for (int fi = 0; fi < 2; ++fi) {
                const int nk = (FSPEC == 1 && REM4) ? 1 : (int)((Q.nk2p[1] >> (4 * fi)) & 15);
                f32x4 e[T];
#pragma unroll
                for (int t = 0; t < T; ++t)
                    e[t] = FSPEC == 1 ? (fi == 0 ? z1[1][t] : pow_abs4(z1[1][t], qex1)) : apply_func(fi == 0 ? qfk0 : qfk1, fi == 0 ? qex0 : qex1, z1[1][t]);
#pragma unroll
                for (int r = 0; r < 4; ++r)
                    if (r < nk) {
#pragma unroll
                        for (int t = 0; t < T; ++t) y1[0][t] = MFMA16(q_a2[1][fi][0][r], e[t][r], y1[0][t]);
#pragma unroll
                        for (int t = 0; t < T; ++t) {
                            if constexpr (REM4) d4[t] = MFMA4(q_a2[1][fi][1][r], e[t][r], d4[t]);
                            else y1[1][t] = MFMA16(q_a2[1][fi][1][r], e[t][r], y1[1][t]);
                        }
                    }
            }
            if constexpr (REM4) {
#pragma unroll
                for (int t = 0; t < T; ++t) add_rem4(y1[1][t], d4[t]);
            }
            if (REM4 && Q.pack_base > 0) {
#pragma unroll
                for (int t = 0; t < T; ++t) {
                    st_y0[t] = y1[0][t];
                    st_y1[t] = y1[1][t][0];
                }
                st_grp = grp;
                if (!DEFER) flush();
            } else {
#pragma unroll
                for (int mt = 0; mt < 2; ++mt)
#pragma unroll
                    for (int t = 0; t < T; ++t)
                        if (tile[t] < P.n_tiles) Q.out[((size_t)tile[t] * Q.nb_out + (size_t)n1 * Q.mto + mt) * 64 + lane] = y1[mt][t];
            }
            if (STAMP) { unsigned long long t = stamp_now(); t_l1 += t - ts; ts = t; ++n_it; }
        }
        grp = grp_next;
    }
    if (DEFER) flush();
    if (STAMP && lane == 0 && P.stamps) {
        unsigned long long* o = P.stamps + ((size_t)blockIdx.x * 8 + wave) * 12;
        const unsigned long long rt1 = __builtin_amdgcn_s_memrealtime();
        o[0] = t_w; o[1] = t_f; o[2] = t_l0; o[3] = t_l1;
        o[4] = stamp_now() - t_all0;
        o[5] = rt1 - rt0;
        o[6] = (unsigned long long)n_it;
        o[7] = rt_entry; o[8] = rt0; o[9] = rt1;
    }
}

template <typename XT, bool STAMP = false, bool WGQ = true>
__global__ void __launch_bounds__(256) __attribute__((amdgpu_waves_per_eu(4, 4))) k_stage01d(StageParams P, StageParams Q) {
    extern __shared__ __attribute__((aligned(16))) f32x4 smem[];
    unsigned long long rt_entry = 0;
    if (STAMP) rt_entry = __builtin_amdgcn_s_memrealtime();
    const int tid = threadIdx.x, lane = tid & 63, g = lane >> 4, j = lane & 15;
    const int wave = __builtin_amdgcn_readfirstlane(tid >> 6);
    const int ci = blockIdx.x % P.n_chunks, part = blockIdx.x / P.n_chunks;
    const DChunk ck = P.chunks[ci];
    unsigned long long* const ring = (unsigned long long*)((float*)smem + 4 * 160);
    int* const prog = (int*)(ring + 8);
#ifndef HG_REM4_LDS
#define HG_REM4_LDS 1
#endif
    float* const rscr = (float*)smem + 4 * 160 + 32 + wave * 256;
    if (WGQ) {
        if (tid < 8) ring[tid] = ~0ull;
        if (tid < 4) prog[tid] = 0;
        __syncthreads();
    }
    if (2 * wave + 1 >= ck.node_count) return;
    const int n_active = ck.node_count >> 1;
    const XT* x = (const XT*)P.x;
    float* cst = (float*)smem + wave * 160;
    enum { C_MU = 0, C_B1 = 2, C_B2 = 4, C_QB1 = 6, C_QB2 = 8 };
    uint32_t src[2];
    f32x4 w_a1[2], w_a2[2][2];
#pragma unroll
    for (int sl = 0; sl < 2; ++sl) {
        const int ni = ck.node_begin + 2 * wave + sl;
        const size_t ent = (size_t)ni * 16 + g * 4;
        src[sl] = (uint32_t)(j * (int)P.ldx + P.kcol[ni * 4 + g]) * (uint32_t)sizeof(XT);
        if (j == 0) *(f32x4*)(cst + (C_MU + sl) * 16 + g * 4) = *(const f32x4*)(P.kmean + ent);
        const f32x4* wp = P.afrag + (size_t)ni * P.node_blocks * 64 + lane;
        w_a1[sl] = wp[0];
        w_a2[sl][0] = wp[64];
        w_a2[sl][1] = wp[128];
        const float* bp = P.bias + (size_t)ni * P.bias_floats + g * 4;
        if (j == 0) {
            *(f32x4*)(cst + (C_B1 + sl) * 16 + g * 4) = *(const f32x4*)bp;
            *(f32x4*)(cst + (C_B2 + sl) * 16 + g * 4) = *(const f32x4*)(bp + 16);
        }
    }
    const int n1 = (ck.node_begin >> 1) + wave;
    f32x4 q_a1[2][2], q_a2[2][2];
    float q_a2t[2][2];
    {
        const f32x4* wq = Q.afrag + (size_t)n1 * Q.node_blocks * 64 + lane;
#pragma unroll
        for (int kb = 0; kb < 2; ++kb)
#pragma unroll
            for (int mt = 0; mt < 2; ++mt) q_a1[kb][mt] = wq[(kb * 2 + mt) * 64];
        const f32x4* wq2 = wq + Q.kb1 * 2 * 64;
#pragma unroll
        for (int fi = 0; fi < 2; ++fi)
#pragma unroll
            for (int mt = 0; mt < 2; ++mt) {
                q_a2[fi][mt] = wq2[(fi * 2 + mt) * 64];
                q_a2t[fi][mt] = wq2[((2 + fi) * 2 + mt) * 64][0];
            }
        const float* bq = Q.bias + (size_t)n1 * Q.bias_floats + g * 4;
#pragma unroll
        for (int mt = 0; mt < 2; ++mt)
            if (j == 0) {
                *(f32x4*)(cst + (C_QB1 + mt) * 16 + g * 4) = *(const f32x4*)(bq + mt * 16);
                *(f32x4*)(cst + (C_QB2 + mt) * 16 + g * 4) = *(const f32x4*)(bq + 32 + mt * 16);
            }
    }
    if (!Q.a4x4) {
        const int bsrc = ((lane & 48) | ((lane & 3) << 2)) << 2;
#pragma unroll
        for (int r = 0; r < 4; ++r) {
#pragma unroll
            for (int kb = 0; kb < 2; ++kb)
                q_a1[kb][1][r] = __int_as_float(__builtin_amdgcn_ds_bpermute(bsrc, __float_as_int(q_a1[kb][1][r])));
#pragma unroll
            for (int fi = 0; fi < 2; ++fi)
                q_a2[fi][1][r] = __int_as_float(__builtin_amdgcn_ds_bpermute(bsrc, __float_as_int(q_a2[fi][1][r])));
        }
#pragma unroll
        for (int fi = 0; fi < 2; ++fi) q_a2t[fi][1] = __int_as_float(__builtin_amdgcn_ds_bpermute(bsrc, __float_as_int(q_a2t[fi][1])));
    }
    const float ex1 = P.expo[1], qex1 = Q.expo[1];
    const int n_tiles = P.n_tiles;
    const int64_t tile_step = (int64_t)16 * P.ldx;

    const uint32_t row_bytes = (uint32_t)P.ldx * (uint32_t)sizeof(XT);
    auto fetch = [&](int tile, f32x4 (&v)[2]) {
#ifdef HIGSFA_DIAG
        if (P.whatif & 1) tile = part;
#endif
        const int64_t rows = P.n_rows - (int64_t)tile * 16;
        const __amdgpu_buffer_rsrc_t r =
            __builtin_amdgcn_make_buffer_rsrc((void*)(x + tile * tile_step), 0, (int)((rows < 16 ? (uint32_t)rows : 16u) * row_bytes), kBufferFlags);
#pragma unroll
        for (int sl = 0; sl < 2; ++sl) v[sl] = Vec4Load<XT>::buf(r, src[sl]);
    };
    uint32_t* qctr = P.work_ctr + (size_t)(WGQ ? ci : n1) * 16;
    const bool grabber = !WGQ || wave == 0;
    const uint32_t q_dyn = (uint32_t)(n_tiles - P.tile_parts);
    auto grab_raw = [&]() -> uint32_t { return __builtin_amdgcn_atomic_inc32(qctr, 0xffffffffu, __ATOMIC_RELAXED, "agent"); };
    uint32_t q_raw = 0;
    bool q_more = true;
    if (grabber && lane == 0) q_raw = grab_raw();
    f32x4 v[2];
    int pass = 0;
    auto decode = [&](uint32_t raw) -> int {
        const uint32_t k = (uint32_t)__builtin_amdgcn_readfirstlane((int)raw) - P.work_base;
        return k < q_dyn ? (int)(P.tile_parts + k) : n_tiles;
    };
    int tile = part;
    if (tile < n_tiles) fetch(tile, v);
    f32x4 st_y0;
    float st_y1 = 0.f;
    int st_tile = -1;
    const int pk_slot = __builtin_amdgcn_readfirstlane(Q.pack_slot[n1]);
    const uint32_t pk_off = (uint32_t)(Q.pack_base + (pk_slot >> 2)) * 1024u + (uint32_t)(pk_slot & 3) * (Q.pack_soa ? 256u : 4u);
    const uint32_t pk_lane = (uint32_t)lane * (Q.pack_soa ? 4u : 16u);
    const uint32_t out_tile_bytes = (uint32_t)Q.nb_out * 1024u;
    auto flush = [&]() {
        if (st_tile < 0) return;
#ifdef HIGSFA_DIAG
        if (P.whatif & 2) { st_tile = -1; return; }
#endif
        const __amdgpu_buffer_rsrc_t r = __builtin_amdgcn_make_buffer_rsrc((void*)(Q.out + (size_t)st_tile * Q.nb_out * 64), 0, (int)out_tile_bytes, kBufferFlags);
        __builtin_amdgcn_raw_buffer_store_b128(__builtin_bit_cast(u32x4_t, st_y0), r, (uint32_t)lane * 16u, (uint32_t)n1 * 1024u, 0);
        __builtin_amdgcn_raw_buffer_store_b32(__float_as_uint(st_y1), r, pk_lane, pk_off, 0);
        st_tile = -1;
    };
    unsigned long long t_top = 0, t_l0 = 0, t_l1 = 0, t_all0 = 0, rt0 = 0, ts = 0;
    int n_it = 0;
    if (STAMP) {
        t_all0 = stamp_now();
        rt0 = __builtin_amdgcn_s_memrealtime();
    }
    while (tile < n_tiles) {
        asm volatile("" ::: "memory");
        if (STAMP) ts = stamp_now();
        int next = n_tiles;
        if (grabber && q_more) {
            next = decode(q_raw);
            q_more = next < n_tiles;
        }
        if (WGQ) {
            constexpr int kSpinLimit = 1 << 22;
            if (wave == 0) {
                if (pass >= 7) {
                    for (int w = 1; w < n_active; ++w) {
                        int spins = 0;
                        while (__builtin_amdgcn_readfirstlane(*(volatile int*)(prog + w)) < pass - 7 && ++spins < kSpinLimit) __builtin_amdgcn_s_sleep(2);
                        if (spins >= kSpinLimit && lane == 0) *P.err = 2;
                    }
                }
                if (lane == 0) *(volatile unsigned long long*)(ring + ((pass + 1) & 7)) = ((unsigned long long)(uint32_t)(pass + 1) << 32) | (uint32_t)next;
            } else {
                int spins = 0, e_pass, e_tile;
                do {
                    const unsigned long long e = *(volatile unsigned long long*)(ring + ((pass + 1) & 7));
                    e_pass = __builtin_amdgcn_readfirstlane((int)(e >> 32));
                    e_tile = __builtin_amdgcn_readfirstlane((int)(uint32_t)e);
                    if (e_pass == pass + 1) break;
                    __builtin_amdgcn_s_sleep(2);
                } while (++spins < kSpinLimit);
                next = e_pass == pass + 1 ? e_tile : n_tiles;
                if (e_pass != pass + 1 && lane == 0) *P.err = 3;
                if (lane == 0) *(volatile int*)(prog + wave) = pass + 1;
            }
            ++pass;
        }
        f32x4 z0[2];
#pragma unroll
        for (int sl = 0; sl < 2; ++sl) {
            const f32x4 bf = v[sl] - *(const f32x4*)(cst + (C_MU + sl) * 16 + g * 4);
            z0[sl] = *(const f32x4*)(cst + (C_B1 + sl) * 16 + g * 4);
#pragma unroll
            for (int r = 0; r < 4; ++r) z0[sl] = MFMA16(w_a1[sl][r], bf[r], z0[sl]);
        }
        if (next < n_tiles) fetch(next, v);
        flush();
        if (grabber && q_more && lane == 0) q_raw = grab_raw();
        if (STAMP) { unsigned long long t = stamp_now(); t_top += t - ts; ts = t; }
        f32x4 y0[2];
#pragma unroll
        for (int sl = 0; sl < 2; ++sl) {
            y0[sl] = *(const f32x4*)(cst + (C_B2 + sl) * 16 + g * 4);
#pragma unroll
            for (int r = 0; r < 4; ++r) y0[sl] = MFMA16(w_a2[sl][0][r], z0[sl][r], y0[sl]);
            const f32x4 e = pow_abs4(z0[sl], ex1);
#pragma unroll
            for (int r = 0; r < 4; ++r) y0[sl] = MFMA16(w_a2[sl][1][r], e[r], y0[sl]);
        }
        if (STAMP) { unsigned long long t = stamp_now(); t_l0 += t - ts; ts = t; }
        f32x4 z1[2], y1[2];
#pragma unroll
        for (int mt = 0; mt < 2; ++mt) {
            z1[mt] = *(const f32x4*)(cst + (C_QB1 + mt) * 16 + g * 4);
            y1[mt] = *(const f32x4*)(cst + (C_QB2 + mt) * 16 + g * 4);
        }
        f32x4 d4 = f32x4{0.f, 0.f, 0.f, 0.f};
#pragma unroll
        for (int kb = 0; kb < 2; ++kb)
#pragma unroll
            for (int r = 0; r < 4; ++r) {
                z1[0] = MFMA16(q_a1[kb][0][r], y0[kb][r], z1[0]);
                d4 = MFMA4(q_a1[kb][1][r], y0[kb][r], d4);
            }
        if constexpr (HG_REM4_LDS) z1[1][0] += rem4_total_lds(d4, rscr, lane);
        else add_rem4(z1[1], d4);
        d4 = f32x4{0.f, 0.f, 0.f, 0.f};
#pragma unroll
        for (int fi = 0; fi < 2; ++fi) {
            const f32x4 e = fi == 0 ? z1[0] : pow_abs4(z1[0], qex1);
#pragma unroll
            for (int r = 0; r < 4; ++r) {
                y1[0] = MFMA16(q_a2[fi][0][r], e[r], y1[0]);
                d4 = MFMA4(q_a2[fi][1][r], e[r], d4);
            }
        }
#pragma unroll
        for (int fi = 0; fi < 2; ++fi) {
            const float e0 = fi == 0 ? z1[1][0] : pow_abs(z1[1][0], qex1);
            y1[0] = MFMA16(q_a2t[fi][0], e0, y1[0]);
            d4 = MFMA4(q_a2t[fi][1], e0, d4);
        }
        if constexpr (HG_REM4_LDS) y1[1][0] += rem4_total_lds(d4, rscr, lane);
        else add_rem4(y1[1], d4);
        st_y0 = y1[0];
        st_y1 = y1[1][0];
        st_tile = tile;
        if (STAMP) { unsigned long long t = stamp_now(); t_l1 += t - ts; ts = t; ++n_it; }
        tile = next;
    }
    flush();
    if (STAMP && lane == 0 && P.stamps) {
        unsigned long long* o = P.stamps + ((size_t)blockIdx.x * 8 + wave) * 12;
        const unsigned long long rt1 = __builtin_amdgcn_s_memrealtime();
        o[0] = t_top; o[1] = 0; o[2] = t_l0; o[3] = t_l1;
        o[4] = stamp_now() - t_all0;
        o[5] = rt1 - rt0;
        o[6] = (unsigned long long)n_it;
        o[7] = rt_entry; o[8] = rt0; o[9] = rt1;
    }
}

StageFn2 pick_stage01d(int x_dtype, bool stamp, bool wgq) {
#ifdef HIGSFA_DIAG
    if (stamp && x_dtype == HG_F32) return wgq ? (StageFn2)k_stage01d<float, true, true> : (StageFn2)k_stage01d<float, true, false>;
#endif
    if (!wgq) return x_dtype == HG_U8 ? (StageFn2)k_stage01d<uint8_t, false, false> : x_dtype == HG_F32 ? (StageFn2)k_stage01d<float, false, false> : (StageFn2)k_stage01d<double, false, false>;
    return x_dtype == HG_U8 ? (StageFn2)k_stage01d<uint8_t> : x_dtype == HG_F32 ? (StageFn2)k_stage01d<float> : (StageFn2)k_stage01d<double>;
}

template <int MT1, int MT2, typename XT>
static StageFn pick_stage0_t(int T) {
    if (T == 4) return k_stage0<MT1, MT2, 4, XT>;
    return k_stage0<MT1, MT2, 1, XT>;
}
template <int MT1, typename XT>
static StageFn pick_stage0_m2(int mt2, int T) {
    switch (mt2) {
        case 1: return pick_stage0_t<MT1, 1, XT>(T);
        case 2: return pick_stage0_t<MT1, 2, XT>(T);
        case 3: return pick_stage0_t<MT1, 3, XT>(T);
        default: return pick_stage0_t<MT1, 4, XT>(T);
    }
}
template <typename XT>
static StageFn pick_stage0_x(int mt1, int mt2, int T) {
    switch (mt1) {
        case 1: return pick_stage0_m2<1, XT>(mt2, T);
        case 2: return pick_stage0_m2<2, XT>(mt2, T);
        case 3: return pick_stage0_m2<3, XT>(mt2, T);
        default: return pick_stage0_m2<4, XT>(mt2, T);
    }
}
StageFn pick_stage0(int mt1, int mt2, int T, int x_dtype) {
    switch (x_dtype) {
        case HG_U8: return pick_stage0_x<uint8_t>(mt1, mt2, T);
        case HG_F32: return pick_stage0_x<float>(mt1, mt2, T);
        default: return pick_stage0_x<double>(mt1, mt2, T);
    }
}
StageFn pick_stage0p(int x_dtype) {
    return x_dtype == HG_U8 ? (StageFn)k_stage0p<4, uint8_t> : x_dtype == HG_F32 ? (StageFn)k_stage0p<4, float> : (StageFn)k_stage0p<4, double>;
}
int stage01p_tiles(bool rem4, bool fspec) { return fspec ? 1 : 2; }

StageFn2 pick_stage01p(int x_dtype, bool stamp, bool rem4, bool fspec) {
    if (rem4) {
#ifdef HIGSFA_DIAG
        if (stamp && x_dtype == HG_F32) return fspec ? (StageFn2)k_stage01p<float, true, true, 1, 1> : (StageFn2)k_stage01p<float, true, true>;
#endif
        if (fspec)
            return x_dtype == HG_U8 ? (StageFn2)k_stage01p<uint8_t, false, true, 1, 1>
                                    : x_dtype == HG_F32 ? (StageFn2)k_stage01p<float, false, true, 1, 1> : (StageFn2)k_stage01p<double, false, true, 1, 1>;
        return x_dtype == HG_U8 ? (StageFn2)k_stage01p<uint8_t, false, true>
                                : x_dtype == HG_F32 ? (StageFn2)k_stage01p<float, false, true> : (StageFn2)k_stage01p<double, false, true>;
    }
#ifdef HIGSFA_DIAG
    if (stamp && x_dtype == HG_F32) return (StageFn2)k_stage01p<float, true>;
#endif
    if (fspec)
        return x_dtype == HG_U8 ? (StageFn2)k_stage01p<uint8_t, false, false, 1, 1>
                                : x_dtype == HG_F32 ? (StageFn2)k_stage01p<float, false, false, 1, 1> : (StageFn2)k_stage01p<double, false, false, 1, 1>;
    return x_dtype == HG_U8 ? (StageFn2)k_stage01p<uint8_t> : x_dtype == HG_F32 ? (StageFn2)k_stage01p<float> : (StageFn2)k_stage01p<double>;
}

}
}
```

### pyfaceanalysis_amd/csrc/hg_fused_plan.cpp

```cpp
#include <algorithm>
#include <cmath>
#include <map>
#include <sstream>
#include <tuple>

#include "hg_fused_plan.hpp"
#include "hg_fused_stages.hpp"

namespace hg {
namespace fused {

namespace {

Aff aff_of(const TNode& n) { return Aff{(int)n.in_dim, (int)n.out_dim, n.a, n.W, n.b}; }

Aff fold(const Aff& f, const Aff& s) {
    Aff r;
    r.in = f.in;
    r.out = s.out;
    r.a = f.a;
    r.W.assign((size_t)f.in * s.out, 0.0);
    for (int i = 0; i < f.in; ++i)
        for (int k = 0; k < f.out; ++k) {
            double w = f.W[(size_t)i * f.out + k];
            if (w == 0.0) continue;
            for (int j = 0; j < s.out; ++j) r.W[(size_t)i * s.out + j] += w * s.W[(size_t)k * s.out + j];
        }
    r.b = s.b;
    for (int k = 0; k < f.out; ++k) {
        double d = f.b[k] - s.a[k];
        for (int j = 0; j < s.out; ++j) r.b[j] += d * s.W[(size_t)k * s.out + j];
    }
    return r;
}

typedef std::vector<const TNode*> LeafSeq;

bool flatten_leafs(const TNode& n, LeafSeq& s, std::string& why) {
    switch (n.kind) {
        case K_AFFINE:
        case K_EXPANSION:
        case K_HEAD:
        case K_CUTOFF:
        case K_IGSFA: s.push_back(&n); return true;
        case K_IDENTITY: return true;
        case K_FLOWNODE:
        case K_FLOW:
            for (auto& c : n.ch)
                if (!flatten_leafs(*c, s, why)) return false;
            return true;
        default: why = std::string("node kind ") + kind_name(n.kind) + " inside a layer is not covered by the fused plan"; return false;
    }
}

struct ChainT {
    int in_dim, out_dim;
    LeafSeq seq;
};

bool to_chains(const TNode& n, std::vector<ChainT>& out, std::string& why) {
    auto one = [&](const TNode& c) {
        ChainT ch{(int)c.in_dim, (int)c.out_dim, {}};
        if (!flatten_leafs(c, ch.seq, why)) return false;
        out.push_back(std::move(ch));
        return true;
    };
    if (n.kind == K_LAYER) {
        for (auto& c : n.ch)
            if (!one(*c)) return false;
        return true;
    }
    if (n.kind == K_CLONELAYER) {
        for (uint32_t i = 0; i < n.aux; ++i)
            if (!one(*n.ch[0])) return false;
        return true;
    }
    return one(n);
}

bool igsfa_affine(const FNode& fn, Aff& A2, bool nofold) {
    const int d = fn.in_dim, k = fn.ig_k, q = fn.ig_pca.out;
    if (nofold) return false;
    int E = 0, id_off = -1;
    for (const ExpFunc& f : fn.funcs) {
        if (f.kind == E_IDENTITY && f.used(d) == d && id_off < 0) id_off = E;
        E += f.out_dim(d);
    }
    if (id_off < 0 || fn.ig_sfa.in != E || fn.ig_sfa.out != k) return false;
    const Aff &S = fn.ig_sfa, &Lr = fn.ig_lr, &Pc = fn.ig_pca;
    std::vector<double> cs(k), Wsl((size_t)E * d, 0.0), cl(d, 0.0);
    for (int j = 0; j < k; ++j) {
        double v = S.b[j];
        for (int e = 0; e < E; ++e) v -= S.a[e] * S.W[(size_t)e * k + j];
        cs[j] = v;
    }
    if (fn.ig_has_lr) {
        for (int e = 0; e < E; ++e)
            for (int j = 0; j < k; ++j) {
                const double w = S.W[(size_t)e * k + j];
                if (w == 0.0) continue;
                for (int c = 0; c < d; ++c) Wsl[(size_t)e * d + c] += w * Lr.W[(size_t)j * d + c];
            }
        for (int c = 0; c < d; ++c) {
            double v = Lr.b[c];
            for (int j = 0; j < k; ++j) v += (cs[j] - Lr.a[j]) * Lr.W[(size_t)j * d + c];
            cl[c] = v;
        }
    }
    A2 = Aff();
    A2.in = E;
    A2.out = k + q;
    A2.a.assign(E, 0.0);
    A2.W.assign((size_t)E * (k + q), 0.0);
    A2.b.assign(k + q, 0.0);
    for (int e = 0; e < E; ++e) {
        for (int j = 0; j < k; ++j) A2.W[(size_t)e * (k + q) + j] = S.W[(size_t)e * k + j];
        for (int c = 0; c < d; ++c) {
            const double m = ((e == id_off + c) ? 1.0 : 0.0) - Wsl[(size_t)e * d + c];
            if (m == 0.0) continue;
            for (int j = 0; j < q; ++j) A2.W[(size_t)e * (k + q) + k + j] += m * Pc.W[(size_t)c * q + j];
        }
    }
    for (int j = 0; j < k; ++j) A2.b[j] = cs[j];
    for (int j = 0; j < q; ++j) {
        double v = Pc.b[j];
        for (int c = 0; c < d; ++c) v += (-cl[c] - Pc.a[c]) * Pc.W[(size_t)c * q + j];
        A2.b[k + j] = v;
    }
    return true;
}

void fold_igsfa(FNode& fn, bool nofold) {
    const int d = fn.in_dim;
    Aff A2;
    if (d > 16 * kMaxMT || !igsfa_affine(fn, A2, nofold)) return;
    Aff A1;
    A1.in = A1.out = d;
    A1.a = fn.ig_mean;
    A1.a.resize(d, 0.0);
    A1.W.assign((size_t)d * d, 0.0);
    for (int c = 0; c < d; ++c) A1.W[(size_t)c * d + c] = 1.0;
    A1.b.assign(d, 0.0);
    fn.A1 = std::move(A1);
    fn.A2 = std::move(A2);
    fn.is_ig = false;
}

bool canon(const ChainT& c, int in_off, FNode& fn, std::string& why, const FusedOptions& opt) {
    fn.in_off = in_off;
    fn.in_dim = c.in_dim;
    fn.out_dim = c.out_dim;
    for (const TNode* l : c.seq)
        if (l->kind == K_IGSFA) {
            if (c.seq.size() != 1) { why = "iGSFA node combined with other nodes in one chain"; return false; }
            if (l->sfa->out_dim != l->aux) { why = "iGSFA node whose sfa_node has more outputs than it preserves"; return false; }
            if (l->in_dim > 128 || l->out_dim > 16 * kMaxMT) { why = "iGSFA node with more than 128 inputs or 64 outputs"; return false; }
            fn.is_ig = true;
            fn.ig_k = (int)l->aux;
            fn.ig_mean = l->x_mean;
            fn.ig_sfa = aff_of(*l->sfa);
            for (int r = 0; r < fn.ig_sfa.in; ++r)
                for (int cc = 0; cc < fn.ig_sfa.out; ++cc) fn.ig_sfa.W[(size_t)r * fn.ig_sfa.out + cc] *= l->magn[cc];
            {
                for (int cc = 0; cc < fn.ig_sfa.out; ++cc) fn.ig_sfa.b[cc] *= l->magn[cc];
            }
            fn.ig_has_lr = (bool)l->lr;
            if (l->lr) fn.ig_lr = aff_of(*l->lr);
            fn.ig_pca = aff_of(*l->pca);
            if (l->exp_node) {
                for (const ExpFunc& f : l->exp_node->funcs)
                    if (f.kind > E_SIGNED_POW) { why = "expansion with cross-column products (QT / pair products)"; return false; }
                fn.funcs = l->exp_node->funcs;
            } else {
                fn.funcs = {ExpFunc{E_IDENTITY, 0, 0, 1.0}};
            }
            fn.has_exp = true;
            fold_igsfa(fn, opt.ig_nofold);
            return true;
        }
    int phase = 0;
    auto head = [](Aff& a, int keep) {
        Aff r;
        r.in = a.in;
        r.out = keep;
        r.a = a.a;
        r.W.resize((size_t)a.in * keep);
        for (int i = 0; i < a.in; ++i)
            for (int o = 0; o < keep; ++o) r.W[(size_t)i * keep + o] = a.W[(size_t)i * a.out + o];
        r.b.assign(a.b.begin(), a.b.begin() + keep);
        a = std::move(r);
    };
    for (const TNode* l : c.seq) {
        if (l->kind == K_AFFINE) {
            if (phase == 0) { fn.A1 = aff_of(*l); phase = 1; }
            else if (phase == 1) fn.A1 = fold(fn.A1, aff_of(*l));
            else if (phase == 2) { fn.A2 = aff_of(*l); phase = 3; }
            else fn.A2 = fold(fn.A2, aff_of(*l));
        } else if (l->kind == K_HEAD) {
            if (phase == 1) head(fn.A1, (int)l->out_dim);
            else if (phase == 3) head(fn.A2, (int)l->out_dim);
            else { why = "HeadNode that does not follow an affine node"; return false; }
        } else if (l->kind == K_CUTOFF) {
            if (phase != 2 || fn.has_clip) { why = "CutoffNode anywhere but between the expansion and the second affine"; return false; }
            fn.has_clip = true;
            fn.clip_lo = l->lo;
            fn.clip_hi = l->hi;
        } else {
            if (phase != 1) { why = "node chain is not [affine][expansion][affine]"; return false; }
            for (const ExpFunc& f : l->funcs)
                if (f.kind > E_SIGNED_POW) fn.has_prod = true;
            fn.funcs = l->funcs;
            fn.has_exp = true;
            phase = 2;
        }
    }
    if (phase == 0) { why = "layer node without an affine part"; return false; }
    if (phase == 2) { why = "node chain ends in an expansion"; return false; }
    if (fn.A1.out > 16 * kMaxMT || (fn.has_exp && fn.A2.out > 16 * kMaxMT)) {
        why = "affine with more than 64 outputs";
        return false;
    }
    return true;
}

}

bool build_stages(const TNode& root, std::vector<FStage>& stages, std::string& why, const FusedOptions& opt) {
    std::vector<int32_t> pending;
    bool have_pending = false;
    std::vector<ChainT> group;
    int frame_w = root.in_dim;

    auto close_group = [&]() -> bool {
        if (group.empty()) return true;
        FStage st;
        int in_w = 0;
        for (auto& c : group) in_w += c.in_dim;
        if (have_pending) {
            if ((int)pending.size() != in_w) { why = "internal: connection count"; return false; }
            st.conn = pending;
        } else {
            if (in_w != frame_w) { why = "internal: frame width"; return false; }
            st.conn.resize(in_w);
            for (int i = 0; i < in_w; ++i) st.conn[i] = i;
        }
        int off = 0;
        for (auto& c : group) {
            FNode fn;
            if (!canon(c, off, fn, why, opt)) return false;
            off += c.in_dim;
            st.out_w += fn.out_dim;
            st.nodes.push_back(std::move(fn));
        }
        frame_w = st.out_w;
        stages.push_back(std::move(st));
        group.clear();
        pending.clear();
        have_pending = false;
        return true;
    };

    for (auto& cp : root.ch) {
        const TNode& c = *cp;
        if (c.kind == K_SWITCHBOARD) {
            if (!close_group()) return false;
            if (have_pending) {
                std::vector<int32_t> comp(c.conn.size());
                for (size_t i = 0; i < c.conn.size(); ++i) comp[i] = pending[c.conn[i]];
                pending.swap(comp);
            } else {
                pending = c.conn;
                have_pending = true;
            }
            continue;
        }
        if (c.kind == K_IDENTITY) continue;
        std::vector<ChainT> chains;
        if (!to_chains(c, chains, why)) return false;
        bool merged = false;
        if (!group.empty() && group.size() == chains.size()) {
            merged = true;
            for (size_t k = 0; k < chains.size(); ++k)
                if (group[k].out_dim != chains[k].in_dim) { merged = false; break; }
            if (merged)
                for (size_t k = 0; k < chains.size() && merged; ++k) {
                    int n_exp = 0, n_ig = 0;
                    for (auto* l : group[k].seq) { n_exp += l->kind == K_EXPANSION; n_ig += l->kind == K_IGSFA; }
                    for (auto* l : chains[k].seq) { n_exp += l->kind == K_EXPANSION; n_ig += l->kind == K_IGSFA; }
                    if (n_exp > 1 || n_ig > 0) merged = false;
                }
            if (merged)
                for (size_t k = 0; k < chains.size(); ++k) {
                    group[k].out_dim = chains[k].out_dim;
                    for (auto* l : chains[k].seq) group[k].seq.push_back(l);
                }
        }
        if (!merged) {
            if (!close_group()) return false;
            group = std::move(chains);
        }
    }
    if (!close_group()) return false;
    if (have_pending) { why = "flow ends in a switchboard"; return false; }
    if (stages.empty()) { why = "no layer in the flow"; return false; }
    return true;
}

std::vector<int> hoist_first_affines(std::vector<FStage>& fs, const FusedOptions& opt) {
    (void)opt;
    std::vector<int> parents;
    auto ordinary = [](const FStage& st) {
        for (auto& n : st.nodes)
            if (n.is_ig || n.has_prod || n.has_clip || !n.has_exp) return false;
        return true;
    };
    auto rem_tile = [](int d) {
        const int r = d - 16 * ((d + 15) / 16 - 1);
        return r >= 1 && r <= 4;
    };
    for (size_t l = 1; l + 1 < fs.size(); ++l) {
        FStage& ch = fs[l];
        FStage& pa = fs[l + 1];
        if (!ordinary(ch) || !ordinary(pa)) continue;
        const int nc = (int)ch.nodes.size(), np = (int)pa.nodes.size();
        std::vector<int> owner, col0(nc, 0);
        for (int ci = 0; ci < nc; ++ci) {
            col0[ci] = (int)owner.size();
            owner.insert(owner.end(), ch.nodes[ci].out_dim, ci);
        }
        std::vector<int> reads(owner.size(), 0), parent_of(nc, -1);
        std::vector<std::vector<int>> kids(np);
        bool ok = true;
        int p_max = 0;
        for (int pj = 0; pj < np && ok; ++pj) {
            const FNode& pn = pa.nodes[pj];
            p_max = std::max(p_max, pn.A1.out);
            if (pn.A1.in != pn.in_dim || !pn.sum_bias.empty()) ok = false;
            for (int c = 0; c < pn.in_dim && ok; ++c) {
                const int pc = pa.conn[pn.in_off + c];
                if (pc < 0 || pc >= (int)owner.size() || ++reads[pc] > 1) { ok = false; break; }
                const int ci = owner[pc];
                if (parent_of[ci] < 0) {
                    parent_of[ci] = pj;
                    kids[pj].push_back(ci);
                } else if (parent_of[ci] != pj) {
                    ok = false;
                }
            }
            if (kids[pj].empty() || kids[pj].size() > 8) ok = false;
        }
        for (int r : reads) ok = ok && r == 1;
        for (int ci = 0; ci < nc && ok; ++ci) {
            if (parent_of[ci] < 0) { ok = false; break; }
            const FNode& cn = ch.nodes[ci];
            if (cn.A2.out != cn.out_dim || pa.nodes[parent_of[ci]].A1.out > cn.A2.out) ok = false;
        }
        if (!ok || rem_tile(p_max)) continue;

        for (int pj = 0; pj < np; ++pj) {
            FNode& pn = pa.nodes[pj];
            const int P = pn.A1.out;
            pn.sum_bias = pn.A1.b;
            pn.kids = kids[pj];
            std::vector<std::vector<double>> Wf(nc);
            for (int ci : kids[pj]) Wf[ci].assign((size_t)ch.nodes[ci].A2.in * P, 0.0);
            for (int c = 0; c < pn.in_dim; ++c) {
                const int pc = pa.conn[pn.in_off + c], ci = owner[pc], k = pc - col0[ci];
                const Aff& A2 = ch.nodes[ci].A2;
                const double* w1 = &pn.A1.W[(size_t)c * P];
                const double d = A2.b[k] - pn.A1.a[c];
                for (int o = 0; o < P; ++o) pn.sum_bias[o] += d * w1[o];
                std::vector<double>& W = Wf[ci];
                for (int e = 0; e < A2.in; ++e) {
                    const double w2 = A2.W[(size_t)e * A2.out + k];
                    if (w2 == 0.0) continue;
                    for (int o = 0; o < P; ++o) W[(size_t)e * P + o] += w2 * w1[o];
                }
            }
            for (int ci : kids[pj]) {
                FNode& cn = ch.nodes[ci];
                for (int e = 0; e < cn.A2.in; ++e) {
                    const double a = cn.A2.a[e];
                    if (a == 0.0) continue;
                    for (int o = 0; o < P; ++o) pn.sum_bias[o] -= a * Wf[ci][(size_t)e * P + o];
                }
                Aff f;
                f.in = cn.A2.in;
                f.out = P;
                f.a.assign(f.in, 0.0);
                f.W = std::move(Wf[ci]);
                f.b.assign(P, 0.0);
                cn.A2 = std::move(f);
                cn.out_dim = P;
            }
            pn.A1.a.clear();
            pn.A1.W.clear();
            pn.A1.b.clear();
        }
        ch.out_w = 0;
        for (auto& cn : ch.nodes) ch.out_w += cn.out_dim;
        pa.sum_in = true;
        parents.push_back((int)l + 1);
    }
    return parents;
}

namespace {

inline int q_of_row(int i) { return 4 * (i & 3) + (i >> 2); }

constexpr int kStage0ChunkCols = 128;
struct Planner : FusedPlan {
    Planner(const TNode& root, std::vector<FStage>&& fs, const FusedOptions& options) {
        opt = options;
        out_dim = root.out_dim;
        std::vector<int32_t> prev_blk, prev_q;
        int prev_nb = 0;
        bool prev_packed = false;
        for (size_t si = 0; si < fs.size(); ++si) {
            FStage& st = fs[si];
            if (st.nodes[0].is_ig) {
                if (stages.empty()) add_gather0(st, prev_blk, prev_q, prev_nb);
                build_ig_stage(st, prev_blk, prev_q, prev_nb);
                prev_packed = false;
                continue;
            }
            {
                bool table_driven = st.nodes[0].has_clip;
                for (auto& nd : st.nodes) table_driven = table_driven || nd.has_prod;
                if (table_driven) {
                    if (stages.empty()) add_gather0(st, prev_blk, prev_q, prev_nb);
                    build_prod_stage(st, prev_blk, prev_q, prev_nb, (int)si);
                    prev_packed = false;
                    continue;
                }
            }
            if (si > 0 && stages.empty()) fail(HG_ERR_FORMAT, "internal: stage order");
            stages.emplace_back();
            HostStage& hs = stages.back();
            hs.from_x = si == 0;
            const int n = (int)st.nodes.size();
            hs.n_nodes = n;
            hs.has_exp = st.nodes[0].has_exp;
            hs.funcs = st.nodes[0].funcs;
            hs.nf = (int)hs.funcs.size();
            int p_max = 0;
            for (auto& nd : st.nodes) {
                hs.mt1 = std::max(hs.mt1, (nd.A1.out + 15) / 16);
                if (nd.has_exp) hs.mt2 = std::max(hs.mt2, (nd.A2.out + 15) / 16);
                p_max = std::max(p_max, nd.A1.out);
                if (nd.has_exp) hs.s_max = std::max(hs.s_max, nd.A2.out);
            }
            hs.p_max = p_max;
            if (!hs.has_exp) hs.mt2 = 1;
            hs.mto = hs.has_exp ? hs.mt2 : hs.mt1;
            hs.nb_in = prev_nb;
            for (int mt1 = 0; mt1 < hs.mt1; ++mt1)
                for (int fi = 0; fi < hs.nf; ++fi) {
                    int valid = std::max(0, std::min(16, hs.funcs[fi].used(p_max) - 16 * mt1));
                    hs.nk2[mt1][fi] = (uint8_t)((valid + 3) / 4);
                }

            struct NodeK {
                std::vector<int> src, nk;
                std::vector<std::vector<int>> kpos;
            };
            std::vector<NodeK> nks(n);
            if (si == 0) plan_stage0_inputs(st, hs);
            for (int ni = 0; ni < n; ++ni) {
                FNode& nd = st.nodes[ni];
                NodeK& K = nks[ni];
                if (st.sum_in) {
                    const HostStage& below = stages[stages.size() - 2];
                    if (below.kind != 0 || below.pack_out || below.mto != hs.mt1) fail(HG_ERR_FORMAT, "internal: hoisted link over a layer of another layout");
                    for (int ci : nd.kids)
                        for (int mt = 0; mt < hs.mt1; ++mt) {
                            K.src.push_back(ci * below.mto + mt);
                            K.nk.push_back(1);
                            for (int qq = 0; qq < 16; ++qq) K.kpos.emplace_back();
                        }
                } else if (si == 0) {
                    const int nkb = (nd.in_dim + 15) / 16;
                    for (int kb = 0; kb < nkb; ++kb) {
                        int valid = std::min(16, nd.in_dim - kb * 16), nk = 0;
                        K.src.push_back(0);
                        for (int q = 0; q < 16; ++q) {
                            K.kpos.emplace_back();
                            const int pos = s0_pos(q >> 2, q & 3);
                            if (pos < valid) {
                                K.kpos.back().push_back(kb * 16 + pos);
                                nk = std::max(nk, (q >> 2) + 1);
                            }
                        }
                        K.nk.push_back(nk);
                    }
                } else {
                    std::map<int, int> blk_index;
                    for (int c = 0; c < nd.in_dim; ++c) {
                        int pc = st.conn[nd.in_off + c];
                        int blk = prev_blk[pc], q = prev_q[pc];
                        auto it = blk_index.find(blk);
                        int kb;
                        if (it == blk_index.end()) {
                            kb = (int)K.src.size();
                            blk_index[blk] = kb;
                            K.src.push_back(blk);
                            K.nk.push_back(0);
                            for (int qq = 0; qq < 16; ++qq) K.kpos.emplace_back();
                        } else {
                            kb = it->second;
                        }
                        K.kpos[kb * 16 + q].push_back(c);
                        K.nk[kb] = std::max(K.nk[kb], q / 4 + 1);
                    }
                }
                hs.kb1 = std::max(hs.kb1, (int)K.src.size());
            }
            hs.sum_in = st.sum_in;
            hs.n_kids = st.sum_in ? hs.kb1 / hs.mt1 : 0;
            const int a1_blocks = st.sum_in ? 0 : hs.kb1 * hs.mt1;
            hs.node_blocks = a1_blocks + (hs.has_exp ? hs.mt1 * hs.nf * hs.mt2 : 0);
            hs.bias_floats = (hs.mt1 + (hs.has_exp ? hs.mt2 : 0)) * 16;
            if (si > 0 && (size_t)hs.node_blocks * 1024 + (size_t)hs.bias_floats * 4 + (size_t)hs.kb1 * 8 > 150 * 1024)
                fail(HG_ERR_FORMAT, "fused: one node needs %d KiB of weight fragments, more than a workgroup's LDS", hs.node_blocks);
            hs.afrag.assign((size_t)n * hs.node_blocks * 256, 0.f);
            hs.bias.assign((size_t)n * hs.bias_floats, 0.f);
            if (si > 0) hs.kb1tab.assign((size_t)n * hs.kb1 * 2, 0);

            std::vector<int32_t> cur_blk, cur_q, node_out;
            for (int ni = 0; ni < n; ++ni) {
                FNode& nd = st.nodes[ni];
                NodeK& K = nks[ni];
                const int p = nd.A1.out;
                float* wnode = hs.afrag.data() + (size_t)ni * hs.node_blocks * 256;
                float* bnode = hs.bias.data() + (size_t)ni * hs.bias_floats;
                std::vector<double> bias1 = st.sum_in ? nd.sum_bias : nd.A1.b;
                for (int c = 0; c < nd.in_dim && !st.sum_in; ++c) {
                    double av = si == 0 ? nd.A1.a[c] - (double)(float)nd.A1.a[c] : nd.A1.a[c];
// ... 13 lines not shown
                        hs.kb1tab[((size_t)ni * hs.kb1 + kb) * 2 + 1] = K.nk[kb] | (r0 << 8);
                    }
                    if (st.sum_in) continue;
                    hs.mfma_per_tile += (int64_t)(K.nk[kb] - r0) * hs.mt1;
                    hs.ks1_tile += K.nk[kb] - r0;
                    for (int mt = 0; mt < hs.mt1; ++mt) {
                        float* blk = wnode + ((size_t)kb * hs.mt1 + mt) * 256;
                        for (int lane = 0; lane < 64; ++lane) {
                            int i = lane & 15, gg = lane >> 4;
                            int fo = 16 * mt + q_of_row(i);
                            if (fo >= p) continue;
                            for (int r = 0; r < 4; ++r) {
                                double w = 0;
                                for (int c : K.kpos[kb * 16 + 4 * r + gg]) w += nd.A1.W[(size_t)c * p + fo];
                                blk[lane * 4 + r] = (float)w;
                            }
                        }
                    }
                }
                if (si > 0)
                    for (int kb = (int)K.src.size(); kb < hs.kb1; ++kb) hs.kb1tab[((size_t)ni * hs.kb1 + kb) * 2] = K.src[0];
                if (si == 0 && (int)K.src.size() == hs.kb1) hs.nk_last = std::max(ni == 0 ? 0 : hs.nk_last, K.nk.back());
                for (int mt = 0; mt < hs.mt1; ++mt)
                    for (int gg = 0; gg < 4; ++gg)
                        for (int r = 0; r < 4; ++r) {
                            int fo = 16 * mt + 4 * r + gg;
                            bnode[mt * 16 + gg * 4 + r] = fo < p ? (float)bias1[fo] : 0.f;
                        }
                int n_out = p;
                if (hs.has_exp) {
                    const int s = nd.A2.out;
                    n_out = s;
                    std::vector<int> foff(nd.funcs.size());
                    int eo = 0;
                    for (size_t fi = 0; fi < nd.funcs.size(); ++fi) {
                        foff[fi] = eo;
                        eo += nd.funcs[fi].out_dim(p);
                    }
                    if (eo != nd.A2.in) fail(HG_ERR_DIM, "fused: expansion width %d != second affine input_dim %d", eo, nd.A2.in);
                    std::vector<double> bias2 = nd.A2.b;
                    for (int c = 0; c < nd.A2.in; ++c)
                        for (int o = 0; o < s; ++o) bias2[o] -= nd.A2.a[c] * nd.A2.W[(size_t)c * s + o];
                    float* w2 = wnode + (size_t)a1_blocks * 256;
                    for (int mt1 = 0; mt1 < hs.mt1; ++mt1)
                        for (int fi = 0; fi < hs.nf; ++fi) {
                            const int used = nd.funcs[fi].used(p);
                            hs.mfma_per_tile += (int64_t)hs.nk2[mt1][fi] * hs.mt2;
                            hs.ks2_tile += hs.nk2[mt1][fi];
                            for (int mt2 = 0; mt2 < hs.mt2; ++mt2) {
                                float* blk = w2 + ((size_t)(mt1 * hs.nf + fi) * hs.mt2 + mt2) * 256;
                                for (int lane = 0; lane < 64; ++lane) {
                                    int i = lane & 15, gg = lane >> 4;
                                    int fo = 16 * mt2 + q_of_row(i);
                                    if (fo >= s) continue;
                                    for (int r = 0; r < 4; ++r) {
                                        int fz = 16 * mt1 + 4 * r + gg;
                                        if (fz >= used) continue;
                                        blk[lane * 4 + r] = (float)nd.A2.W[(size_t)(foff[fi] + fz) * s + fo];
                                    }
                                }
                            }
                        }
                    for (int mt = 0; mt < hs.mt2; ++mt)
                        for (int gg = 0; gg < 4; ++gg)
                            for (int r = 0; r < 4; ++r) {
                                int fo = 16 * mt + 4 * r + gg;
                                bnode[hs.mt1 * 16 + mt * 16 + gg * 4 + r] = fo < s ? (float)bias2[fo] : 0.f;
                            }
                }
                node_out.push_back(n_out);
            }
            {
                const int r1 = hs.p_max - 16 * (hs.mt1 - 1), r2 = hs.s_max - 16 * (hs.mt2 - 1);
                hs.rem4 = si >= 1 && hs.has_exp && n > 4 && hs.mt1 == hs.mt2 && (hs.mt1 == 2 || hs.mt1 == 3) && r1 >= 1 && r1 <= 4 &&
                          r2 >= 1 && r2 <= 4 && !opt.no_rem4 && !st.sum_in;
                if (hs.rem4) {
                    auto to4x4 = [](float* blk) {
                        float old[256];
                        std::copy(blk, blk + 256, old);
                        for (int l = 0; l < 64; ++l) {
                            const int src = (l & 48) | ((l & 3) << 2);
                            for (int r = 0; r < 4; ++r) blk[l * 4 + r] = old[src * 4 + r];
                        }
                    };
                    for (int ni = 0; ni < n; ++ni) {
                        float* wnode = hs.afrag.data() + (size_t)ni * hs.node_blocks * 256;
                        for (int kb = 0; kb < hs.kb1; ++kb) to4x4(wnode + ((size_t)kb * hs.mt1 + hs.mt1 - 1) * 256);
                        float* w2 = wnode + (size_t)hs.kb1 * hs.mt1 * 256;
                        for (int b2 = 0; b2 < hs.mt1 * hs.nf; ++b2) to4x4(w2 + ((size_t)b2 * hs.mt2 + hs.mt2 - 1) * 256);
                    }
                }
            }
            hs.pack_out = false;
            if (hs.rem4 && n % 4 == 0 && !opt.no_pack && si + 1 < fs.size()) {
                const FStage& nx = fs[si + 1];
                bool ok = nx.nodes.size() > 16;
                for (auto& nd : nx.nodes) ok = ok && !nd.is_ig && !nd.has_prod && !nd.has_clip && nd.has_exp;
                hs.pack_out = ok;
            }
            if (hs.pack_out) {
                const FStage& nx = fs[si + 1];
                std::vector<int> col0(n, 0), reader(n, 1 << 30);
                for (int ni = 1; ni < n; ++ni) col0[ni] = col0[ni - 1] + node_out[ni - 1];
                std::vector<int> owner;
                for (int ni = 0; ni < n; ++ni) owner.insert(owner.end(), node_out[ni], ni);
                for (size_t pj = 0; pj < nx.nodes.size(); ++pj)
                    for (int c = 0; c < nx.nodes[pj].in_dim; ++c) {
                        const int col = nx.conn[nx.nodes[pj].in_off + c];
                        const int ni = owner[col];
                        if (col - col0[ni] >= 16 * (hs.mto - 1)) reader[ni] = std::min(reader[ni], (int)pj);
                    }
                std::vector<int> order(n);
                for (int ni = 0; ni < n; ++ni) order[ni] = ni;
                std::stable_sort(order.begin(), order.end(), [&](int a, int b) { return reader[a] < reader[b]; });
                hs.pack_slot.assign(n, 0);
                for (int rk = 0; rk < n; ++rk) hs.pack_slot[order[rk]] = rk;
            }
            for (int ni = 0; ni < n; ++ni)
                for (int f = 0; f < node_out[ni]; ++f) {
                    if (hs.pack_out && f >= 16 * (hs.mto - 1)) {
                        cur_blk.push_back(n * (hs.mto - 1) + hs.pack_slot[ni] / 4);
                        cur_q.push_back(4 * (hs.pack_slot[ni] % 4) + (f - 16 * (hs.mto - 1)));
                    } else {
                        cur_blk.push_back(ni * (hs.pack_out ? hs.mto - 1 : hs.mto) + f / 16);
                        cur_q.push_back(f % 16);
                    }
                }
            hs.nb_out = hs.pack_out ? n * (hs.mto - 1) + n / 4 : n * hs.mto;
            prev_packed = hs.pack_out;
            prev_blk.swap(cur_blk);
            prev_q.swap(cur_q);
            prev_nb = hs.nb_out;
            max_nb = std::max(max_nb, hs.nb_out);
            {
                const bool front_rem = si == 1 && hs.has_exp && hs.mt1 == 2 && hs.mt2 == 2 && hs.p_max <= 20 && hs.s_max <= 20 && hs.nk2[1][0] <= 1 &&
                                       hs.nk2[1][1] <= 1 && !opt.no_rem4;
                const int rem = (hs.rem4 || front_rem) ? 1 : 0;
                hs.mfma16_tile = hs.ks1_tile * (hs.mt1 - rem) + (hs.has_exp ? hs.ks2_tile * (hs.mt2 - rem) : 0);
                hs.mfma4_tile = rem ? hs.ks1_tile + hs.ks2_tile : 0;
            }
            padded_flops += (hs.mfma16_tile * 2048 + hs.mfma4_tile * 512) / 16;
            std::ostringstream os;
            os << "fused stage " << si << (hs.rem4 ? (hs.pack_out ? " (4x4 remainder tiles, packed four to a block)" : " (4x4 remainder tiles)") : "") << ": " << hs.n_nodes << " nodes, K-blocks " << hs.kb1 << ", tiles " << hs.mt1 << "x" << hs.mt2
               << (hs.sum_in ? " (first affine folded into the layer below's second, plain 16-row tiles only: z = bias + the tiles of " + std::to_string(hs.n_kids) + " children)" : "")
               << ", " << hs.mfma_per_tile << " MFMA/tile (issued: " << hs.mfma16_tile << " x 16x16x4 + " << hs.mfma4_tile << " x 4x4x1), " << hs.afrag.size() * 4 / 1024
               << " KiB weights, out " << hs.nb_out << " blocks/tile";
            hs.name = os.str();
        }
        plan_slot_major();
        fuse01 = can_fuse01();
        if (fuse01) {
            stages[0].name += "  [+ stage 1 fused in the same persistent kernel when the input allows 16-byte loads]";
        }
        col_base.resize(out_dim);
        col_of.assign((size_t)std::max(prev_nb, 1) * 16, -1);
        for (int c = 0; c < out_dim; ++c) {
            int q = prev_q[c];
            col_base[c] = prev_blk[c] * 256 + (q & 3) * 64 + (q >> 2);
            col_of[(size_t)prev_blk[c] * 16 + q] = c;
        }
        for (auto& hs : stages)
            if (!hs.kb1tab.empty()) hs.kb1tab.resize(hs.kb1tab.size() + 16, 0);
        plan_tail();
        plan_subtree();
        for (auto& hs : stages)
            if (!hs.chunks.empty()) hs.piece_col.resize(std::max<size_t>(hs.piece_col.size(), 2));
    }

    void plan_stage0_inputs(const FStage& st, HostStage& hs) {
        const int n = (int)st.nodes.size();
        int kb1 = 0, max_in = 0;
        for (auto& nd : st.nodes) {
            kb1 = std::max(kb1, (nd.in_dim + 15) / 16);
            max_in = std::max(max_in, nd.in_dim);
        }
        s0_transpose = true;
        for (auto& nd : st.nodes) {
            for (int c = 0; c < nd.in_dim && s0_transpose; c += 4)
                for (int r = 1; r < 4 && c + r < nd.in_dim; ++r)
                    if (st.conn[nd.in_off + c + r] != st.conn[nd.in_off + c] + r) s0_transpose = false;
            if (nd.in_dim % 4) s0_transpose = false;
        }
        const int col_budget = std::max(kStage0ChunkCols, (max_in + 3) / 4 * 4);
        if (col_budget > 2048) fail(HG_ERR_FORMAT, "fused: first-layer node with %d inputs", max_in);
        hs.koff.assign((size_t)n * kb1 * 16, -1);
        hs.kmean.assign((size_t)n * kb1 * 16, 0.f);
        int max_cols = 0, ni = 0;
        bool vec_ok = true, contig = true;
        while (ni < n) {
            std::vector<int32_t> cols;
            int n1 = ni;
            while (n1 < n) {
                std::vector<int32_t> c2 = cols;
                const FNode& nd = st.nodes[n1];
                for (int c = 0; c < nd.in_dim; ++c) c2.push_back(st.conn[nd.in_off + c]);
                std::sort(c2.begin(), c2.end());
                c2.erase(std::unique(c2.begin(), c2.end()), c2.end());
                if ((int)c2.size() > col_budget && n1 > ni) break;
                cols.swap(c2);
                ++n1;
            }
            DChunk ck{ni, n1 - ni, (int)hs.runs.size(), 0, 0, (int)hs.piece_col.size() / 2, 0, 0};
            std::map<int32_t, int32_t> lds_of;
            int n_runs = 0, max_len = 0;
            for (size_t i = 0; i < cols.size();) {
                size_t k = i + 1;
                while (k < cols.size() && cols[k] == cols[k - 1] + 1) ++k;
                ++n_runs;
                max_len = std::max(max_len, (int)(k - i));
                i = k;
            }
            const bool packed4 = s0_transpose && n_runs == 4 && max_len <= 32;
            static const int packed_off[4] = {0, 64, 32, 96};
            int off = 0, run_i = 0, hi = 0;
            for (size_t i = 0; i < cols.size(); ++run_i) {
                size_t k = i + 1;
                while (k < cols.size() && cols[k] == cols[k - 1] + 1) ++k;
                const int len = (int)(k - i);
                off = packed4 ? packed_off[run_i] : (off + 63) / 64 * 64;
                hs.runs.push_back(DRun{cols[i], len, off, 0});
                if (cols[i] % 4 || len % 4) vec_ok = false;
                for (size_t m = i; m < k; ++m) lds_of[cols[m]] = off + (int)(m - i);
                for (int pc = 0; pc + 3 < len; pc += 4) {
                    hs.piece_col.push_back(cols[i] + pc);
                    hs.piece_col.push_back(off + pc);
                    ++ck.n_pieces;
                }
                off += len;
                hi = std::max(hi, off);
                i = k;
                ++ck.run_count;
            }
            off = hi;
            ck.n_cols = off;
            max_cols = std::max(max_cols, off);
            for (int k = ni; k < n1; ++k) {
                const FNode& nd = st.nodes[k];
                for (int kb = 0; kb < kb1; ++kb)
                    for (int g = 0; g < 4; ++g)
                        for (int r = 0; r < 4; ++r) {
                            int c = kb * 16 + s0_pos(r, g);
                            size_t e = (((size_t)k * kb1 + kb) * 4 + g) * 4 + r;
                            if (c < nd.in_dim) {
                                hs.koff[e] = lds_of[st.conn[nd.in_off + c]];
                                hs.kmean[e] = (float)nd.A1.a[c];
                            }
                        }
            }
            hs.chunks.push_back(ck);
            hs.max_chunk_nodes = std::max(hs.max_chunk_nodes, ck.node_count);
            hs.max_chunk_pieces = std::max(hs.max_chunk_pieces, ck.n_pieces);
            ni = n1;
        }
        int stride = max_cols + 1;
        while (stride % 64 != 4) ++stride;
        hs.lds_stride = stride;
        for (size_t e = 0; e < hs.koff.size(); e += 4) {
            bool any_pad = false;
            for (int r = 0; r < 4; ++r)
                if (hs.koff[e + r] < 0) {
                    hs.koff[e + r] = stride - 1;
                    any_pad = true;
                }
            if (any_pad || hs.koff[e] % 4) contig = false;
            for (int r = 1; r < 4; ++r)
                if (hs.koff[e + r] != hs.koff[e] + r) contig = false;
        }
        hs.contig4 = contig;
        hs.vec_ok = vec_ok;
        bool direct = contig && vec_ok && s0_transpose && kb1 == 1;
        hs.kcol.assign((size_t)n * 4, 0);
        for (int k = 0; k < n && direct; ++k) {
            const FNode& nd = st.nodes[k];
            if (nd.in_dim != 16) { direct = false; break; }
            for (int g = 0; g < 4; ++g) {
                const int c0 = s0_pos(0, g), col = st.conn[nd.in_off + c0];
                for (int r = 0; r < 4; ++r)
                    if (s0_pos(r, g) != c0 + r || st.conn[nd.in_off + c0 + r] != col + r) direct = false;
                if (col % 4) direct = false;
                hs.kcol[(size_t)k * 4 + g] = col;
            }
        }
        hs.direct_ok = direct;
        if (!direct) hs.kcol.clear();
    }

    void add_gather0(FStage& st, std::vector<int32_t>& prev_blk, std::vector<int32_t>& prev_q, int& prev_nb) {
        stages.emplace_back();
        HostStage& hs = stages.back();
        hs.kind = 1;
        hs.from_x = true;
        const int n = (int)st.nodes.size();
        int KB = 0;
        bool tr = true;
        for (auto& nd : st.nodes) {
            KB = std::max(KB, (nd.in_dim + 15) / 16);
            for (int c = 0; c < nd.in_dim && tr; c += 4)
                for (int r = 1; r < 4 && c + r < nd.in_dim; ++r)
                    if (st.conn[nd.in_off + c + r] != st.conn[nd.in_off + c] + r) tr = false;
            if (nd.in_dim % 4) tr = false;
        }
        hs.n_nodes = n;
        hs.kb1 = KB;
        hs.nb_out = n * KB;
        hs.gcol.assign((size_t)n * KB * 16, -1);
        const int in_w = (int)st.conn.size();
// ... 411 lines not shown
                    pk = kb;
                }
                if (seen != 1) ok = false;
            }
            if (!ok || pk != 1) continue;
            for (int ni = 0; ni < co.n_nodes; ++ni) {
                int32_t& y = co.kb1tab[((size_t)ni * co.kb1 + pk) * 2 + 1];
                const int nk = y & 255, r0 = y >> 8;
                float* wnode = co.afrag.data() + (size_t)ni * co.node_blocks * 256;
                for (int mt = 0; mt < co.mt1; ++mt) {
                    float* blk = wnode + ((size_t)pk * co.mt1 + mt) * 256;
                    for (int lane = 0; lane < 64; ++lane) {
                        float v[4] = {0.f, 0.f, 0.f, 0.f};
                        for (int r = r0; r < nk; ++r) v[r - r0] = blk[lane * 4 + r];
                        for (int r = 0; r < 4; ++r) blk[lane * 4 + r] = v[r];
                    }
                }
                y = (nk - r0) | (r0 << 16);
            }
            pr.pack_soa = true;
            co.pack_in = base;
            co.pk_kbi = pk;
            pr.name += "  [packed blocks slot-major]";
        }
    }

    void plan_tail() {
        tail_begin = -1;
        if (opt.tail_max <= 0) return;
        const int ns = (int)stages.size();
        int b = ns;
        int act_blocks = 0, e_blocks = 0;
        while (b > (fuse01 ? 2 : 1) && ns - b < opt.tail_max) {
            const HostStage& s = stages[b - 1];
            if (s.kind != 0 || s.from_x || s.rem4 || s.pack_out || s.pk_kbi >= 0 || s.pack_in != INT32_MAX || s.nf > kMaxFuncs) break;
            if (s.has_exp && s.mt1 * s.nf > 8) break;
            const int waves = s.n_nodes * (s.has_exp ? std::max(s.mt1, s.mt2) : s.mt1);
            if (waves > 16) break;
            const int act = b - 1 < ns - 1 ? std::max(act_blocks, s.nb_out) : act_blocks;
            const int eb = std::max(e_blocks, s.has_exp ? s.n_nodes * s.nf * s.mt1 : 0);
            if (((size_t)2 * act + eb) * 1024 > 150 * 1024) break;
            act_blocks = act;
            e_blocks = eb;
            --b;
        }
        if (b == ns) return;
        tail_begin = b;
        tail_act_blocks = act_blocks;
        tail_e_blocks = e_blocks;
        for (int i = b; i < ns; ++i)
            stages[i].name += i == b ? (ns - b > 1 ? "  [this and the layers above: ONE launch, activations in LDS, writes the caller's rows]"
                                                    : "  [writes the caller's rows: no unpack pass]")
                                      : "  [in the top-of-hierarchy launch]";
    }

    void plan_subtree() {
        sub_runs.clear();
        if (opt.subtree_max_tiles <= 0) return;
        const int ns = (int)stages.size();
        const int end = tail_begin < 0 ? ns : (ns - tail_begin >= 3 ? tail_begin + 1 : tail_begin);
        plan_subtree_set(end, 0);
        if (!sub_runs.empty()) plan_subtree_set(end - 1, 1);
    }

    void plan_subtree_set(int end, int set) {
        while (end - 1 >= 2) {
            const int last = end - 1;
            const int k = stages[last].n_nodes;
            int b = last + 1, act_blocks = 0, e_blocks = 0;
            std::vector<std::vector<int32_t>> members(kMaxTail), tabs(kMaxTail);
            while (k >= 4 && b > (fuse01 ? 2 : 1) && last + 1 - b < kMaxTail) {
                const HostStage& s = stages[b - 1];
                if (s.kind != 0 || s.from_x || s.rem4 || s.pack_out || s.pk_kbi >= 0 || s.pack_in != INT32_MAX || s.nf > kMaxFuncs ||
                    s.n_nodes % k)
                    break;
                if (s.has_exp && s.mt1 * s.nf > 8) break;
                const int per = s.n_nodes / k;
                if (per * (s.has_exp ? std::max(s.mt1, s.mt2) : s.mt1) > 16) break;
                std::vector<int32_t> mem((size_t)k * per, -1), tab;
                if (b - 1 == last) {
                    for (int j = 0; j < k; ++j) mem[j] = j;
                } else {
                    const HostStage& up = stages[b];
                    const std::vector<int32_t>& mup = members[last - b];
                    const int per_up = up.n_nodes / k;
                    std::vector<int32_t> owner(s.n_nodes, -1), pos(s.n_nodes, -1);
                    bool ok = s.nb_out == s.n_nodes * s.mto;
                    tab.assign(up.kb1tab.size(), 0);
                    for (int j = 0; j < k && ok; ++j) {
                        int have = 0;
                        for (int q = 0; q < per_up && ok; ++q) {
                            const int ni = mup[(size_t)j * per_up + q];
                            for (int kb = 0; kb < up.kb1 && ok; ++kb) {
                                const size_t at = ((size_t)ni * up.kb1 + kb) * 2;
                                const int src = up.kb1tab[at];
                                if (src < 0 || src >= s.nb_out) { ok = false; break; }
                                const int sn = src / s.mto;
                                if (owner[sn] < 0) {
                                    if (have == per) { ok = false; break; }
                                    owner[sn] = j;
                                    pos[sn] = have;
                                    mem[(size_t)j * per + have++] = sn;
                                } else if (owner[sn] != j) {
                                    ok = false;
                                    break;
                                }
                                tab[at] = pos[sn] * s.mto + src % s.mto;
                                tab[at + 1] = up.kb1tab[at + 1];
                            }
                        }
                        if (have != per) ok = false;
                    }
                    if (!ok) break;
                }
                const int act = b - 1 < last ? std::max(act_blocks, per * s.mto) : act_blocks;
                const int eb = std::max(e_blocks, s.has_exp ? per * s.nf * s.mt1 : 0);
                if (((size_t)2 * act + eb) * 1024 > 150 * 1024) break;
                act_blocks = act;
                e_blocks = eb;
                members[last - (b - 1)] = std::move(mem);
                if (b - 1 < last) tabs[last - b] = std::move(tab);
                --b;
            }
            if (last + 1 - b < 2) {
                end = last;
                continue;
            }
            SubRun r;
            r.begin = b;
            r.len = last + 1 - b;
            r.n = k;
            r.act_blocks = act_blocks;
            r.e_blocks = e_blocks;
            r.set = set;
            for (int i = b; i <= last; ++i) {
                r.nodes[i - b] = members[last - i];
                if (i > b) r.tab[i - b] = tabs[last - i];
            }
            sub_runs.push_back(std::move(r));
            if (set != 0) {
                stages[b].name += "  [or, where more layers or more sub-trees can run that way: " + std::to_string(last + 1 - b) + " layers from here as " + std::to_string(k) + " sub-trees]";
                end = b;
                continue;
            }
            for (int i = b; i <= last; ++i) {
                stages[i].name += i == b ? "  [batches of up to " + std::to_string(std::min(opt.subtree_max_tiles, opt.subtree_max_wgs / k) * 16) + " rows: this and the next " +
                                                std::to_string(last - b) + " layer(s) as " + std::to_string(k) + " sub-trees in ONE launch]"
                                          : "  [in the sub-tree launch for short batches]";
            }
            end = b;
        }
    }

    bool can_fuse01() const {
        if (stages.size() < 2) return false;
        const HostStage& a = stages[0];
        const HostStage& b = stages[1];
        if (a.kind != 0 || b.kind != 0 || !a.from_x) return false;
        if (!(a.has_exp && a.mt1 == 1 && a.mt2 == 1 && a.kb1 == 1 && a.nf == 2 && a.contig4 && a.vec_ok)) return false;
        if (a.nk_last != 4 || a.nk2[0][0] != 4 || a.nk2[0][1] != 4) return false;
        if (a.max_chunk_nodes > 16 || a.max_chunk_pieces > 64) return false;
        for (auto& c : a.chunks)
            if ((c.node_begin & 1) || (c.node_count & 1)) return false;
        if (!(b.has_exp && b.mt1 == 2 && b.mt2 == 2 && b.kb1 == 2 && b.nf == 2 && b.nk2[0][0] == 4 && b.nk2[0][1] == 4)) return false;
        if (b.n_nodes * 2 != a.n_nodes) return false;
        for (int n = 0; n < b.n_nodes; ++n)
            if (b.kb1tab[(size_t)n * 4] != 2 * n || b.kb1tab[(size_t)n * 4 + 2] != 2 * n + 1) return false;
        return true;
    }

    int s0_pos(int r, int g) const { return s0_transpose ? 4 * g + r : 4 * r + g; }
};

}

bool FusedPlan::sub_run_pays(const SubRun& r, int n_tiles) const {
    return n_tiles <= opt.subtree_max_tiles && (int64_t)r.n * n_tiles <= opt.subtree_max_wgs;
}

int FusedPlan::pick_sub_set(int n_tiles) const {
    int best = 0, best_cov = -1, best_k = 0;
    for (int set = 0; set < 2; ++set) {
        int cov = 0, mink = 0x7fffffff;
        for (const SubRun& r : sub_runs)
            if (r.set == set && sub_run_pays(r, n_tiles)) {
                cov += r.len;
                mink = std::min(mink, r.n);
            }
        if (cov > best_cov || (cov == best_cov && cov > 0 && mink > best_k)) {
            best = set;
            best_cov = cov;
            best_k = mink;
        }
    }
    return best;
}

int FusedPlan::tail_start(int n_tiles) const {
    const int ns = (int)stages.size();
    bool short_batch = n_tiles < 96;
    const int sub_set = pick_sub_set(n_tiles);
    for (const SubRun& r : sub_runs)
        if (r.set == sub_set && r.begin <= tail_begin && tail_begin < r.begin + r.len && sub_run_pays(r, n_tiles)) short_batch = true;
    return (ns - tail_begin >= 3 && short_batch) ? tail_begin + 1 : tail_begin;
}

std::unique_ptr<const FusedPlan> build_fused_plan(const TNode& root, const FusedOptions& opt, std::string* why_not) {
    std::vector<FStage> stages;
    std::string why;
    if (!build_stages(root, stages, why, opt)) {
        if (why_not) *why_not = why;
        return nullptr;
    }
    for (auto& st : stages) {
        const FNode& f0 = st.nodes[0];
        bool table_driven = f0.has_clip;
        for (auto& n : st.nodes) table_driven = table_driven || n.has_prod;
        if (f0.funcs.size() > (size_t)kMaxFuncs && !table_driven) {
            if (why_not) *why_not = "more than 4 expansion functions";
            return nullptr;
        }
        for (auto& n : st.nodes) {
            bool same = n.has_exp == f0.has_exp && n.is_ig == f0.is_ig && n.funcs.size() == f0.funcs.size() && n.has_clip == f0.has_clip &&
                        (!n.has_clip || (n.clip_lo == f0.clip_lo && n.clip_hi == f0.clip_hi));
            for (size_t i = 0; same && i < n.funcs.size(); ++i)
                same = n.funcs[i].kind == f0.funcs[i].kind && n.funcs[i].expo == f0.funcs[i].expo && n.funcs[i].sel == f0.funcs[i].sel &&
                       n.funcs[i].k == f0.funcs[i].k;
            if (!same) {
                if (why_not) *why_not = "nodes of one layer use different expansions";
                return nullptr;
            }
        }
    }
    if (why_not) why_not->clear();
    int64_t given = -1;
    if (opt.hoist) {
        std::vector<FStage> plain = stages;
        if (!hoist_first_affines(stages, opt).empty()) {
            try {
                FusedOptions o = opt;
                o.hoist = false;
                given = Planner(root, std::move(plain), o).padded_flops;
            } catch (const Error&) {
            }
        }
    }
    try {
        Planner p(root, std::move(stages), opt);
        p.padded_flops_given = given >= 0 ? given : p.padded_flops;
        return std::make_unique<const FusedPlan>(std::move(static_cast<FusedPlan&>(p)));
    } catch (const Error& e) {
        if (why_not) *why_not = e.what();
        return nullptr;
    }
}

}
}
```

### pyfaceanalysis_amd/csrc/hg_fused_plan.hpp

```cpp
#pragma once
#include <algorithm>
#include <cstdlib>

#include "hg_common.hpp"

namespace hg {
namespace fused {

constexpr int kMaxMT = 4;

constexpr int kMaxFuncs = 4;

constexpr int kMaxTail = 3;

struct DChunk {
    int32_t node_begin, node_count, run_begin, run_count, n_cols, piece_begin, n_pieces, pad1;
};
struct DRun {
    int32_t start, len, lds_off, pad;
};

struct FusedOptions {
    bool no_rem4 = false, ig_nofold = false, debug = false;
    int stamp_stage = -1;
    bool no_pack = false;
    bool no_soa = false;
    uint32_t wq_start = 0;
    bool no_wgq = false;
    bool no_direct = false;
    int tail_max = 3;
    bool no_fspec = false;
    int subtree_max_tiles = 64;
    int subtree_max_wgs = 256;
    int splitm_max_nodes = 4;
    int splitm_max_wgs = 512;
    int sum_lds_kib = 32;
    bool hoist = false;
    static FusedOptions from_env() {
        FusedOptions o;
        o.no_rem4 = getenv("HIGSFA_NO_REM4") != nullptr;
        o.ig_nofold = getenv("HIGSFA_IG_NOFOLD") != nullptr;
        o.debug = getenv("HIGSFA_DEBUG") != nullptr;
        if (const char* e = getenv("HIGSFA_STAMP")) o.stamp_stage = atoi(e);

        o.no_pack = getenv("HIGSFA_NO_PACK") != nullptr;
        o.no_soa = getenv("HIGSFA_NO_SOA") != nullptr;
        o.no_fspec = getenv("HIGSFA_NO_FSPEC") != nullptr;
        o.no_direct = getenv("HIGSFA_NO_DIRECT") != nullptr;
        o.no_wgq = getenv("HIGSFA_NO_WGQ") != nullptr;
        if (const char* e = getenv("HIGSFA_WQ_START")) o.wq_start = (uint32_t)strtoul(e, nullptr, 0);
        if (const char* e = getenv("HIGSFA_SPLITM_MAX")) o.splitm_max_nodes = atoi(e);
        if (const char* e = getenv("HIGSFA_SPLITM_WGS")) o.splitm_max_wgs = atoi(e);
        if (const char* e = getenv("HIGSFA_SUBTREE")) o.subtree_max_tiles = std::max(0, atoi(e));
        if (const char* e = getenv("HIGSFA_SUBTREE_WGS")) o.subtree_max_wgs = std::max(0, atoi(e));
        if (const char* e = getenv("HIGSFA_SUM_LDS")) o.sum_lds_kib = std::max(1, atoi(e));
        if (const char* e = getenv("HIGSFA_TAIL")) o.tail_max = std::max(0, std::min(atoi(e), kMaxTail));
        return o;
    }
};

struct SubRun {
    int begin = 0, len = 0, n = 0, act_blocks = 0, e_blocks = 0, set = 0;
    std::vector<int32_t> nodes[kMaxTail], tab[kMaxTail];
};

struct HostStage {
    int mt1 = 1, mt2 = 1, mto = 1, nb_out = 0, nb_in = 0, n_nodes = 0, kb1 = 0, nf = 0;
    int node_blocks = 0, bias_floats = 0, nk_last = 4;
    int p_max = 0, s_max = 0;
    bool rem4 = false;
    bool pack_out = false;
    bool pack_soa = false;
    int pack_in = 0x7fffffff;
    int pk_kbi = -1;
    std::vector<int32_t> pack_slot;
    bool has_exp = false, contig4 = false, vec_ok = false;
    std::vector<ExpFunc> funcs;
    uint8_t nk2[kMaxMT][kMaxFuncs] = {};
    std::vector<float> afrag, bias;
    std::vector<int32_t> kb1tab;
    std::vector<DChunk> chunks;
    std::vector<DRun> runs;
    std::vector<int32_t> piece_col, koff;
    std::vector<float> kmean;
    std::vector<int32_t> kcol;
    bool direct_ok = false;
    int lds_stride = 0, max_chunk_nodes = 0, max_chunk_pieces = 0;
    int kind = 0;
    int neb = 0;
    bool has_clip = false;
    float clip_lo = 0, clip_hi = 0;
    std::vector<int32_t> etab;
    bool from_x = false;
    bool ig_has_lr = false, ig_folded = false;
    int ig_nks[kMaxMT] = {};
    std::vector<int32_t> gcol;
    int64_t mfma_per_tile = 0;
    int64_t mfma16_tile = 0, mfma4_tile = 0;
    int64_t ks1_tile = 0, ks2_tile = 0;
    std::string name;
    bool sum_in = false;
    int n_kids = 0;
};

struct FusedPlan {
    FusedOptions opt;
    int out_dim = 0;
    bool s0_transpose = false, fuse01 = false;
    std::vector<HostStage> stages;
    std::vector<int32_t> col_base, col_of;
    int tail_begin = -1;
    int tail_act_blocks = 0, tail_e_blocks = 0;
    std::vector<SubRun> sub_runs;
    int max_nb = 0;
    int64_t padded_flops = 0;
    int64_t padded_flops_given = 0;

    bool sub_run_pays(const SubRun& r, int n_tiles) const;
    int pick_sub_set(int n_tiles) const;
    int tail_start(int n_tiles) const;
};

std::unique_ptr<const FusedPlan> build_fused_plan(const TNode& root, const FusedOptions& opt, std::string* why_not);

}
}
```

### pyfaceanalysis_amd/csrc/hg_fused_stages.hpp

```cpp
#pragma once
#include <string>
#include <vector>

#include "hg_fused_plan.hpp"

namespace hg {
namespace fused {

struct Aff {
    int in = 0, out = 0;
    std::vector<double> a, W, b;
};

struct FNode {
    int in_off = 0, in_dim = 0, out_dim = 0;
    Aff A1, A2;
    bool has_exp = false;
    std::vector<ExpFunc> funcs;
    bool has_prod = false;
    bool has_clip = false;
    double clip_lo = 0, clip_hi = 0;
    bool is_ig = false, ig_has_lr = false;
    int ig_k = 0;
    std::vector<double> ig_mean;
    Aff ig_sfa, ig_lr, ig_pca;
    std::vector<int> kids;
    std::vector<double> sum_bias;
};

struct FStage {
    std::vector<int32_t> conn;
    std::vector<FNode> nodes;
    int out_w = 0;
    bool sum_in = false;
};

bool build_stages(const TNode& root, std::vector<FStage>& stages, std::string& why, const FusedOptions& opt);

std::vector<int> hoist_first_affines(std::vector<FStage>& stages, const FusedOptions& opt);

}
}
```

Before: 9.347 million sub-images/s.

## Fold layer-0 second affine into layer-1 first affine in the fused front kernel

At plan time, layer 0's second affine is multiplied into layer 1's first affine, giving per-node folded weight fragments and biases. The fused front kernel then skips computing layer 0's output y0 and the matmul that consumes it. Instead it applies the folded weights directly to the expanded [z0, |z0|^p] values. This cuts MFMA count and weight registers in the first two layers, but needs extra host-side folding and a scalar-load fallback path, and changes floating-point rounding.

```diff
diff --git a/pyfaceanalysis_amd/csrc/hg_fused.hip b/pyfaceanalysis_amd/csrc/hg_fused.hip
--- a/pyfaceanalysis_amd/csrc/hg_fused.hip
+++ b/pyfaceanalysis_amd/csrc/hg_fused.hip
@@ -524,6 +524,7 @@
 
 struct StageDev {
     DevBuf afrag, bias, kb1tab, chunks, runs, piece, koff, kmean, kcol, gcol, etab, pack_slot;
+    DevBuf fold_frag, fold_bias;
 };
 struct SubRunDev {
     DevBuf nodes[kMaxTail], tab[kMaxTail];
@@ -550,6 +551,8 @@
     int plan_kind() const override { return HG_PLAN_FUSED; }
     int n_stages() const override { return (int)plan_->stages.size() + 1; }
     std::string stage_name(int i) const override {
+        if (i == 1 && plan_->fuse01 && !plan_->opt.fold01)
+            return plan_->stages[i].name + "  [link 0 -> 1 stays as it is: switched off (HIGSFA_NO_FOLD01)]";
         if (i < (int)plan_->stages.size()) return plan_->stages[i].name;
         return plan_->tail_begin >= 0 ? std::string("row-major y written by the top-of-hierarchy launch (no unpack pass)")
                                       : std::string("fused unpack (fragment order -> row-major y)");
@@ -577,7 +580,19 @@
         for (size_t si = 0; si < dev_.size(); ++si) {
             const HostStage& s = plan_->stages[si];
             StageDev& d = dev_[si];
-            d.afrag.upload(s.afrag.data(), s.afrag.size() * 4);
+            if (plan_->fold01 && si < 2) {
+                const size_t first = si == 0 ? 0 : (size_t)s.kb1 * s.mt1, count = si == 0 ? (size_t)s.kb1 * s.mt1 : (size_t)s.node_blocks - first;
+                std::vector<float> part((size_t)s.n_nodes * count * 256);
+                for (int ni = 0; ni < s.n_nodes; ++ni)
+                    std::copy_n(s.afrag.data() + ((size_t)ni * s.node_blocks + first) * 256, count * 256, part.data() + (size_t)ni * count * 256);
+                d.afrag.upload(part.data(), part.size() * 4);
+                if (si == 1) {
+                    d.fold_frag.upload(s.fold_frag.data(), s.fold_frag.size() * 4);
+                    d.fold_bias.upload(s.fold_bias.data(), s.fold_bias.size() * 4);
+                }
+            } else {
+                d.afrag.upload(s.afrag.data(), s.afrag.size() * 4);
+            }
             d.bias.upload(s.bias.data(), s.bias.size() * 4);
             if (!s.kb1tab.empty()) d.kb1tab.upload(s.kb1tab.data(), s.kb1tab.size() * 4);
             if (!s.gcol.empty()) d.gcol.upload(s.gcol.data(), s.gcol.size() * 4);
@@ -796,6 +811,12 @@
         R.a4x4 = hs.rem4 ? 1 : 0;
         R.sum_in = hs.sum_in ? 1 : 0;
         R.n_kids = hs.n_kids;
+        if (plan_->fold01 && (&hs == &plan_->stages[0] || &hs == &plan_->stages[1])) {
+            const bool first = &hs == &plan_->stages[0];
+            R.node_blocks = first ? hs.kb1 * hs.mt1 : hs.node_blocks - hs.kb1 * hs.mt1;
+            R.fold_frag = (const f32x4*)d.fold_frag.p;
+            R.fold_bias = (const float*)d.fold_bias.p;
+        }
         for (int fi = 0; fi < hs.nf; ++fi) {
             R.funcp |= (uint32_t)hs.funcs[fi].kind << (4 * fi);
             R.expo[fi] = (float)hs.funcs[fi].expo;
@@ -935,12 +956,14 @@
             fspec = id_pow(s) && id_pow(plan_->stages[1]) && !plan_->opt.no_fspec;
         }
         const int FT = stage01p_tiles(rem4, fspec);
-        if (plan_->fuse01 && P.vec4 && n_tiles >= FT) {
+        const bool fold = plan_->fold01;
+        if (fold && !(rem4 && plan_->fuse01)) fail(HG_ERR_STATE, "internal: the link 0 -> 1 is folded but the front kernel's remainder-tile form does not apply");
+        if (plan_->fuse01 && ((P.vec4 && n_tiles >= FT) || fold)) {
             StageParams Q = stage_params(plan_->stages[1], dev_[1], nullptr, out1, n_tiles);
             const size_t esz = dtype_size(x_dtype);
-            const bool direct = fspec && rem4 && s.direct_ok && plan_->stages[1].pack_out && (int64_t)16 * ldx * (int64_t)esz + 2048 < 0x7fffffffll && s.max_chunk_nodes <= 8 && !plan_->opt.no_direct;
+            const bool direct = P.vec4 && fspec && rem4 && s.direct_ok && plan_->stages[1].pack_out && (int64_t)16 * ldx * (int64_t)esz + 2048 < 0x7fffffffll && s.max_chunk_nodes <= 8 && !plan_->opt.no_direct;
             const bool wgq = !plan_->opt.no_wgq;
-            StageFn2 fn = direct ? pick_stage01d(x_dtype, false, wgq) : pick_stage01p(x_dtype, false, rem4, fspec);
+            StageFn2 fn = direct ? pick_stage01d(x_dtype, false, wgq, fold) : pick_stage01p(x_dtype, false, rem4, fspec, fold, fold && !P.vec4);
             const int thr01 = 64 * std::max(1, (s.max_chunk_nodes + 1) / 2);
             const size_t lds2 = direct ? (size_t)4 * 160 * 4 + 32 * 4 + (size_t)4 * 256 * 4
                                        : (size_t)(kDoubleBuffer01 ? 2 : 1) * FT * 16 * s.lds_stride * 4 + (size_t)(thr01 / 64) * 160 * 4 + 16;
@@ -949,8 +972,8 @@
             P.tile_parts = std::max(1, std::min(groups2, 256 * occ / std::max(1, P.n_chunks)));
             if (plan_->opt.debug) fprintf(stderr, "[front] occ %d threads %d lds %zu chunks %d tile_parts %d\n", occ, thr01, lds2, P.n_chunks, P.tile_parts);
 #ifdef HIGSFA_DIAG
-            if (plan_->opt.stamp_stage == 0 && x_dtype == HG_F32) {
-                fn = direct ? pick_stage01d(HG_F32, true, wgq) : pick_stage01p(HG_F32, true, rem4, fspec);
+            if (plan_->opt.stamp_stage == 0 && x_dtype == HG_F32 && (direct || !fold)) {
+                fn = direct ? pick_stage01d(HG_F32, true, wgq, fold) : pick_stage01p(HG_F32, true, rem4, fspec, fold);
                 stamps_begin(P, P.n_chunks * P.tile_parts, 12, st);
             }
 #endif
@@ -970,6 +993,7 @@
 #endif
             return true;
         }
+        if (fold) fail(HG_ERR_STATE, "internal: an unfused first-layer kernel on a plan whose link 0 -> 1 is folded");
         const bool persistent = T == 4 && P.vec4 && s.contig4 && s.has_exp && s.mt1 == 1 && s.mt2 == 1 && s.kb1 == 1 &&
                                 s.nf <= 2 && s.max_chunk_nodes <= 16 && 64 * s.max_chunk_pieces <= 8 * 512;
         if (persistent) {
@@ -1270,6 +1294,7 @@
 std::unique_ptr<Executor> make_fused_executor(const TNode& root, std::string* why_not) {
     fused::FusedOptions opt = fused::FusedOptions::from_env();
     opt.hoist = getenv("HIGSFA_NO_HOIST") == nullptr;
+    opt.fold01 = getenv("HIGSFA_NO_FOLD01") == nullptr;
     auto plan = fused::build_fused_plan(root, opt, why_not);
     if (!plan) return nullptr;
     return std::make_unique<FusedExecutor>(std::move(plan));
diff --git a/pyfaceanalysis_amd/csrc/hg_fused_dev.hpp b/pyfaceanalysis_amd/csrc/hg_fused_dev.hpp
--- a/pyfaceanalysis_amd/csrc/hg_fused_dev.hpp
+++ b/pyfaceanalysis_amd/csrc/hg_fused_dev.hpp
@@ -50,6 +50,8 @@
     int32_t* err;
     int32_t whatif;
     int32_t sum_in, n_kids;
+    const f32x4* fold_frag;
+    const float* fold_bias;
 };
 
 __device__ __forceinline__ unsigned long long stamp_now() {
@@ -360,9 +362,9 @@
 
 StageFn pick_stage0(int mt1, int mt2, int T, int x_dtype);
 StageFn pick_stage0p(int x_dtype);
-StageFn2 pick_stage01p(int x_dtype, bool stamp, bool rem4, bool fspec);
+StageFn2 pick_stage01p(int x_dtype, bool stamp, bool rem4, bool fspec, bool fold = false, bool scalar = false);
 int stage01p_tiles(bool rem4, bool fspec);
-StageFn2 pick_stage01d(int x_dtype, bool stamp, bool wgq);
+StageFn2 pick_stage01d(int x_dtype, bool stamp, bool wgq, bool fold = false);
 StageFn pick_igsfa(int ms, int mo, int T, int kb1);
 StageFn pick_igfold(int mo, int T, bool fs = false);
 StageFn pick_prod(int mt1, int mt2, int T);
diff --git a/pyfaceanalysis_amd/csrc/hg_fused_front.hip b/pyfaceanalysis_amd/csrc/hg_fused_front.hip
--- a/pyfaceanalysis_amd/csrc/hg_fused_front.hip
+++ b/pyfaceanalysis_amd/csrc/hg_fused_front.hip
@@ -210,7 +210,7 @@
     }
 }
 
-template <typename XT, bool STAMP = false, bool REM4 = false, int TT = 2, int FSPEC = 0>
+template <typename XT, bool STAMP = false, bool REM4 = false, int TT = 2, int FSPEC = 0, bool FOLD = false, bool SCALAR = false>
 __global__ void __launch_bounds__(512) __attribute__((amdgpu_waves_per_eu(TT == 2 ? 3 : TT == 1 ? 4 : 2, TT == 2 ? 3 : TT == 1 ? 4 : 2))) k_stage01p(StageParams P, StageParams Q) {
     extern __shared__ __attribute__((aligned(16))) f32x4 smem[];
     float* lds = (float*)smem;
@@ -253,23 +253,35 @@
         if (j == 0) *(f32x4*)(cst + (C_MU + sl) * 16 + g * 4) = *(const f32x4*)(P.kmean + ent);
         const f32x4* wp = P.afrag + (size_t)ni * P.node_blocks * 64 + lane;
         w_a1[sl] = wp[0];
-        w_a2[sl][0] = wp[64];
-        w_a2[sl][1] = P.nf > 1 ? wp[128] : wp[64];
+        if constexpr (!FOLD) {
+            w_a2[sl][0] = wp[64];
+            w_a2[sl][1] = P.nf > 1 ? wp[128] : wp[64];
+        }
         const float* bp = P.bias + (size_t)ni * P.bias_floats + g * 4;
         if (j == 0) {
             *(f32x4*)(cst + (C_B1 + sl) * 16 + g * 4) = *(const f32x4*)bp;
-            *(f32x4*)(cst + (C_B2 + sl) * 16 + g * 4) = *(const f32x4*)(bp + 16);
+            if constexpr (!FOLD) *(f32x4*)(cst + (C_B2 + sl) * 16 + g * 4) = *(const f32x4*)(bp + 16);
         }
     }
     const int n1 = (ck.node_begin >> 1) + (w_ok ? wave : 0);
-    f32x4 q_a1[2][2], q_a2[2][2][2];
+    f32x4 q_a1[2][2], q_a2[2][2][2], ff[2][2][2];
     {
         const f32x4* wq = Q.afrag + (size_t)n1 * Q.node_blocks * 64 + lane;
-#pragma unroll
-        for (int kb = 0; kb < 2; ++kb)
-#pragma unroll
-            for (int mt = 0; mt < 2; ++mt) q_a1[kb][mt] = wq[(kb * 2 + mt) * 64];
-        const f32x4* wq2 = wq + Q.kb1 * 2 * 64;
+        if constexpr (FOLD) {
+            const f32x4* wf = Q.fold_frag + (size_t)n1 * 8 * 64 + lane;
+#pragma unroll
+            for (int sl = 0; sl < 2; ++sl)
+#pragma unroll
+                for (int fi = 0; fi < 2; ++fi)
+#pragma unroll
+                    for (int mt = 0; mt < 2; ++mt) ff[sl][fi][mt] = wf[((sl * 2 + fi) * 2 + mt) * 64];
+        } else {
+#pragma unroll
+            for (int kb = 0; kb < 2; ++kb)
+#pragma unroll
+                for (int mt = 0; mt < 2; ++mt) q_a1[kb][mt] = wq[(kb * 2 + mt) * 64];
+        }
+        const f32x4* wq2 = FOLD ? wq : wq + Q.kb1 * 2 * 64;
 #pragma unroll
         for (int m1 = 0; m1 < 2; ++m1)
 #pragma unroll
@@ -277,10 +289,11 @@
 #pragma unroll
                 for (int mt = 0; mt < 2; ++mt) q_a2[m1][fi][mt] = wq2[((m1 * Q.nf + (fi < Q.nf ? fi : 0)) * 2 + mt) * 64];
         const float* bq = Q.bias + (size_t)n1 * Q.bias_floats + g * 4;
+        const float* bq1 = FOLD ? Q.fold_bias + (size_t)n1 * 32 + g * 4 : bq;
 #pragma unroll
         for (int mt = 0; mt < 2; ++mt)
             if (j == 0) {
-                *(f32x4*)(cst + (C_QB1 + mt) * 16 + g * 4) = *(const f32x4*)(bq + mt * 16);
+                *(f32x4*)(cst + (C_QB1 + mt) * 16 + g * 4) = *(const f32x4*)(bq1 + mt * 16);
                 *(f32x4*)(cst + (C_QB2 + mt) * 16 + g * 4) = *(const f32x4*)(bq + 32 + mt * 16);
             }
     }
@@ -288,9 +301,11 @@
         const int src = ((lane & 48) | ((lane & 3) << 2)) << 2;
 #pragma unroll
         for (int r = 0; r < 4; ++r) {
-#pragma unroll
-            for (int kb = 0; kb < 2; ++kb)
-                q_a1[kb][1][r] = __int_as_float(__builtin_amdgcn_ds_bpermute(src, __float_as_int(q_a1[kb][1][r])));
+            if constexpr (!FOLD) {
+#pragma unroll
+                for (int kb = 0; kb < 2; ++kb)
+                    q_a1[kb][1][r] = __int_as_float(__builtin_amdgcn_ds_bpermute(src, __float_as_int(q_a1[kb][1][r])));
+            }
 #pragma unroll
             for (int m1 = 0; m1 < 2; ++m1)
 #pragma unroll
@@ -312,6 +327,20 @@
                 v[k] = Vec4Load<XT>::ld(p_src[k] + goff);
             else
                 v[k] = f32x4{0.f, 0.f, 0.f, 0.f};
+        }
+    };
+    constexpr bool scalar_in = SCALAR;
+    auto stage_scalar = [&](int grp, float* tile_lds) {
+        const int nw = nthr >> 6;
+        for (int sj = wave; sj < T * 16; sj += nw) {
+            const int64_t row = (int64_t)grp * (T * 16) + sj;
+            const bool ok = row < P.n_rows;
+            const XT* srow = x + (ok ? row : 0) * P.ldx;
+            float* dst = tile_lds + sj * stride;
+            for (int ri = 0; ri < ck.run_count; ++ri) {
+                const DRun rn = P.runs[ck.run_begin + ri];
+                for (int e = lane; e < rn.len; e += 64) dst[rn.lds_off + e] = ok ? (float)srow[rn.start + e] : 0.f;
+            }
         }
     };
     f32x4 v[NB];
@@ -326,7 +355,7 @@
     uint32_t q_raw = 0;
     bool q_more = tid == 0;
     if (q_more) q_raw = grab_raw();
-    if (part < n_groups) fetch(part, v);
+    if (part < n_groups && !scalar_in) fetch(part, v);
     const int buf_words = T * 16 * stride;
     float* lds0 = lds;
     int flip = 0;
@@ -362,9 +391,13 @@
             __syncthreads();
         }
         flip ^= 1;
-#pragma unroll
-        for (int k = 0; k < NB; ++k)
-            if (p_dst[k] >= 0) *(f32x4*)(lds + (p_dst[k] & 0xffffff)) = v[k];
+        if (scalar_in) {
+            stage_scalar(grp, lds);
+        } else {
+#pragma unroll
+            for (int k = 0; k < NB; ++k)
+                if (p_dst[k] >= 0) *(f32x4*)(lds + (p_dst[k] & 0xffffff)) = v[k];
+        }
         if (tid < T * 16) lds[tid * stride + stride - 1] = 0.f;
         if (tid == 0) {
             const int q_next = q_more ? grab_group(q_raw) : n_groups;
@@ -374,7 +407,7 @@
         __syncthreads();
         const int grp_next = __builtin_amdgcn_readfirstlane(qslot[slot]);
         if (STAMP) { unsigned long long t = stamp_now(); t_w += t - ts; ts = t; }
-        if (grp_next < n_groups) fetch(grp_next, v);
+        if (grp_next < n_groups && !scalar_in) fetch(grp_next, v);
         if (DEFER) flush();
         if (q_more) q_raw = grab_raw();
         if (STAMP) { unsigned long long t = stamp_now(); t_f += t - ts; ts = t; }
@@ -382,6 +415,49 @@
             int tile[T];
 #pragma unroll
             for (int t = 0; t < T; ++t) tile[t] = grp * T + t;
+            f32x4 z1[2][T], y1[2][T];
+#pragma unroll
+            for (int mt = 0; mt < 2; ++mt)
+#pragma unroll
+                for (int t = 0; t < T; ++t) {
+                    z1[mt][t] = *(const f32x4*)(cst + (C_QB1 + mt) * 16 + g * 4);
+                    y1[mt][t] = *(const f32x4*)(cst + (C_QB2 + mt) * 16 + g * 4);
+                }
+            f32x4 d4[T];
+#pragma unroll
+            for (int t = 0; t < T; ++t) d4[t] = f32x4{0.f, 0.f, 0.f, 0.f};
+            if constexpr (FOLD) {
+#pragma unroll
+                for (int sl = 0; sl < NPW; ++sl) {
+                    f32x4 z[T], bf[T];
+                    const f32x4 mu = *(const f32x4*)(cst + (C_MU + sl) * 16 + g * 4);
+                    const f32x4 cb1 = *(const f32x4*)(cst + (C_B1 + sl) * 16 + g * 4);
+#pragma unroll
+                    for (int t = 0; t < T; ++t) {
+                        bf[t] = *(const f32x4*)(lds + (t * 16 + j) * stride + w_off[sl]) - mu;
+                        z[t] = cb1;
+                    }
+#pragma unroll
+                    for (int r = 0; r < 4; ++r)
+#pragma unroll
+                        for (int t = 0; t < T; ++t) z[t] = MFMA16(w_a1[sl][r], bf[t][r], z[t]);
+#pragma unroll
+                    for (int fi = 0; fi < 2; ++fi) {
+                        f32x4 e[T];
+#pragma unroll
+                        for (int t = 0; t < T; ++t)
+                            e[t] = FSPEC == 1 ? (fi == 0 ? z[t] : pow_abs4(z[t], ex1)) : apply_func(fi == 0 ? fk0 : fk1, fi == 0 ? ex0 : ex1, z[t]);
+#pragma unroll
+                        for (int r = 0; r < 4; ++r) {
+#pragma unroll
+                            for (int t = 0; t < T; ++t) z1[0][t] = MFMA16(ff[sl][fi][0][r], e[t][r], z1[0][t]);
+#pragma unroll
+                            for (int t = 0; t < T; ++t) d4[t] = MFMA4(ff[sl][fi][1][r], e[t][r], d4[t]);
+                        }
+                    }
+                }
+                if (STAMP) { unsigned long long t = stamp_now(); t_l0 += t - ts; ts = t; }
+            } else {
             f32x4 y0[NPW][T];
 #pragma unroll
             for (int sl = 0; sl < NPW; ++sl) {
@@ -418,17 +494,6 @@
                 }
             }
             if (STAMP) { unsigned long long t = stamp_now(); t_l0 += t - ts; ts = t; }
-            f32x4 z1[2][T], y1[2][T];
-#pragma unroll
-            for (int mt = 0; mt < 2; ++mt)
-#pragma unroll
-                for (int t = 0; t < T; ++t) {
-                    z1[mt][t] = *(const f32x4*)(cst + (C_QB1 + mt) * 16 + g * 4);
-                    y1[mt][t] = *(const f32x4*)(cst + (C_QB2 + mt) * 16 + g * 4);
-                }
-            f32x4 d4[T];
-#pragma unroll
-            for (int t = 0; t < T; ++t) d4[t] = f32x4{0.f, 0.f, 0.f, 0.f};
 #pragma unroll
             for (int kb = 0; kb < 2; ++kb)
 #pragma unroll
@@ -441,6 +506,7 @@
                         else z1[1][t] = MFMA16(q_a1[kb][1][r], y0[kb][t][r], z1[1][t]);
                     }
                 }
+            }
             if constexpr (REM4) {
 #pragma unroll
                 for (int t = 0; t < T; ++t) {
@@ -519,7 +585,7 @@
     }
 }
 
-template <typename XT, bool STAMP = false, bool WGQ = true>
+template <typename XT, bool STAMP = false, bool WGQ = true, bool FOLD = false>
 __global__ void __launch_bounds__(256) __attribute__((amdgpu_waves_per_eu(4, 4))) k_stage01d(StageParams P, StageParams Q) {
     extern __shared__ __attribute__((aligned(16))) f32x4 smem[];
     unsigned long long rt_entry = 0;
@@ -554,24 +620,36 @@
         if (j == 0) *(f32x4*)(cst + (C_MU + sl) * 16 + g * 4) = *(const f32x4*)(P.kmean + ent);
         const f32x4* wp = P.afrag + (size_t)ni * P.node_blocks * 64 + lane;
         w_a1[sl] = wp[0];
-        w_a2[sl][0] = wp[64];
-        w_a2[sl][1] = wp[128];
+        if constexpr (!FOLD) {
+            w_a2[sl][0] = wp[64];
+            w_a2[sl][1] = wp[128];
+        }
         const float* bp = P.bias + (size_t)ni * P.bias_floats + g * 4;
         if (j == 0) {
             *(f32x4*)(cst + (C_B1 + sl) * 16 + g * 4) = *(const f32x4*)bp;
-            *(f32x4*)(cst + (C_B2 + sl) * 16 + g * 4) = *(const f32x4*)(bp + 16);
+            if constexpr (!FOLD) *(f32x4*)(cst + (C_B2 + sl) * 16 + g * 4) = *(const f32x4*)(bp + 16);
         }
     }
     const int n1 = (ck.node_begin >> 1) + wave;
-    f32x4 q_a1[2][2], q_a2[2][2];
+    f32x4 q_a1[2][2], q_a2[2][2], ff[2][2][2];
     float q_a2t[2][2];
     {
         const f32x4* wq = Q.afrag + (size_t)n1 * Q.node_blocks * 64 + lane;
-#pragma unroll
-        for (int kb = 0; kb < 2; ++kb)
-#pragma unroll
-            for (int mt = 0; mt < 2; ++mt) q_a1[kb][mt] = wq[(kb * 2 + mt) * 64];
-        const f32x4* wq2 = wq + Q.kb1 * 2 * 64;
+        if constexpr (FOLD) {
+            const f32x4* wf = Q.fold_frag + (size_t)n1 * 8 * 64 + lane;
+#pragma unroll
+            for (int sl = 0; sl < 2; ++sl)
+#pragma unroll
+                for (int fi = 0; fi < 2; ++fi)
+#pragma unroll
+                    for (int mt = 0; mt < 2; ++mt) ff[sl][fi][mt] = wf[((sl * 2 + fi) * 2 + mt) * 64];
+        } else {
+#pragma unroll
+            for (int kb = 0; kb < 2; ++kb)
+#pragma unroll
+                for (int mt = 0; mt < 2; ++mt) q_a1[kb][mt] = wq[(kb * 2 + mt) * 64];
+        }
+        const f32x4* wq2 = FOLD ? wq : wq + Q.kb1 * 2 * 64;
 #pragma unroll
         for (int fi = 0; fi < 2; ++fi)
 #pragma unroll
@@ -580,10 +658,11 @@
                 q_a2t[fi][mt] = wq2[((2 + fi) * 2 + mt) * 64][0];
             }
         const float* bq = Q.bias + (size_t)n1 * Q.bias_floats + g * 4;
+        const float* bq1 = FOLD ? Q.fold_bias + (size_t)n1 * 32 + g * 4 : bq;
 #pragma unroll
         for (int mt = 0; mt < 2; ++mt)
             if (j == 0) {
-                *(f32x4*)(cst + (C_QB1 + mt) * 16 + g * 4) = *(const f32x4*)(bq + mt * 16);
+                *(f32x4*)(cst + (C_QB1 + mt) * 16 + g * 4) = *(const f32x4*)(bq1 + mt * 16);
                 *(f32x4*)(cst + (C_QB2 + mt) * 16 + g * 4) = *(const f32x4*)(bq + 32 + mt * 16);
             }
     }
@@ -591,9 +670,11 @@
         const int bsrc = ((lane & 48) | ((lane & 3) << 2)) << 2;
 #pragma unroll
         for (int r = 0; r < 4; ++r) {
-#pragma unroll
-            for (int kb = 0; kb < 2; ++kb)
-                q_a1[kb][1][r] = __int_as_float(__builtin_amdgcn_ds_bpermute(bsrc, __float_as_int(q_a1[kb][1][r])));
+            if constexpr (!FOLD) {
+#pragma unroll
+                for (int kb = 0; kb < 2; ++kb)
+                    q_a1[kb][1][r] = __int_as_float(__builtin_amdgcn_ds_bpermute(bsrc, __float_as_int(q_a1[kb][1][r])));
+            }
 #pragma unroll
             for (int fi = 0; fi < 2; ++fi)
                 q_a2[fi][1][r] = __int_as_float(__builtin_amdgcn_ds_bpermute(bsrc, __float_as_int(q_a2[fi][1][r])));
@@ -700,6 +781,30 @@
         flush();
         if (grabber && q_more && lane == 0) q_raw = grab_raw();
         if (STAMP) { unsigned long long t = stamp_now(); t_top += t - ts; ts = t; }
+        f32x4 z1[2], y1[2];
+        f32x4 d4 = f32x4{0.f, 0.f, 0.f, 0.f};
+        if constexpr (FOLD) {
+#pragma unroll
+            for (int mt = 0; mt < 2; ++mt) {
+                z1[mt] = *(const f32x4*)(cst + (C_QB1 + mt) * 16 + g * 4);
+                y1[mt] = *(const f32x4*)(cst + (C_QB2 + mt) * 16 + g * 4);
+            }
+#pragma unroll
+            for (int sl = 0; sl < 2; ++sl) {
+#pragma unroll
+                for (int r = 0; r < 4; ++r) {
+                    z1[0] = MFMA16(ff[sl][0][0][r], z0[sl][r], z1[0]);
+                    d4 = MFMA4(ff[sl][0][1][r], z0[sl][r], d4);
+                }
+                const f32x4 e = pow_abs4(z0[sl], ex1);
+#pragma unroll
+                for (int r = 0; r < 4; ++r) {
+                    z1[0] = MFMA16(ff[sl][1][0][r], e[r], z1[0]);
+                    d4 = MFMA4(ff[sl][1][1][r], e[r], d4);
+                }
+            }
+            if (STAMP) { unsigned long long t = stamp_now(); t_l0 += t - ts; ts = t; }
+        } else {
         f32x4 y0[2];
 #pragma unroll
         for (int sl = 0; sl < 2; ++sl) {
@@ -711,13 +816,11 @@
             for (int r = 0; r < 4; ++r) y0[sl] = MFMA16(w_a2[sl][1][r], e[r], y0[sl]);
         }
         if (STAMP) { unsigned long long t = stamp_now(); t_l0 += t - ts; ts = t; }
-        f32x4 z1[2], y1[2];
 #pragma unroll
         for (int mt = 0; mt < 2; ++mt) {
             z1[mt] = *(const f32x4*)(cst + (C_QB1 + mt) * 16 + g * 4);
             y1[mt] = *(const f32x4*)(cst + (C_QB2 + mt) * 16 + g * 4);
         }
-        f32x4 d4 = f32x4{0.f, 0.f, 0.f, 0.f};
 #pragma unroll
         for (int kb = 0; kb < 2; ++kb)
 #pragma unroll
@@ -725,6 +828,7 @@
                 z1[0] = MFMA16(q_a1[kb][0][r], y0[kb][r], z1[0]);
                 d4 = MFMA4(q_a1[kb][1][r], y0[kb][r], d4);
             }
+        }
         if constexpr (HG_REM4_LDS) z1[1][0] += rem4_total_lds(d4, rscr, lane);
         else add_rem4(z1[1], d4);
         d4 = f32x4{0.f, 0.f, 0.f, 0.f};
@@ -763,10 +867,15 @@
     }
 }
 
-StageFn2 pick_stage01d(int x_dtype, bool stamp, bool wgq) {
+StageFn2 pick_stage01d(int x_dtype, bool stamp, bool wgq, bool fold) {
 #ifdef HIGSFA_DIAG
+    if (stamp && x_dtype == HG_F32 && fold) return wgq ? (StageFn2)k_stage01d<float, true, true, true> : (StageFn2)k_stage01d<float, true, false, true>;
     if (stamp && x_dtype == HG_F32) return wgq ? (StageFn2)k_stage01d<float, true, true> : (StageFn2)k_stage01d<float, true, false>;
 #endif
+    if (fold) {
+        if (!wgq) return x_dtype == HG_U8 ? (StageFn2)k_stage01d<uint8_t, false, false, true> : x_dtype == HG_F32 ? (StageFn2)k_stage01d<float, false, false, true> : (StageFn2)k_stage01d<double, false, false, true>;
+        return x_dtype == HG_U8 ? (StageFn2)k_stage01d<uint8_t, false, true, true> : x_dtype == HG_F32 ? (StageFn2)k_stage01d<float, false, true, true> : (StageFn2)k_stage01d<double, false, true, true>;
+    }
     if (!wgq) return x_dtype == HG_U8 ? (StageFn2)k_stage01d<uint8_t, false, false> : x_dtype == HG_F32 ? (StageFn2)k_stage01d<float, false, false> : (StageFn2)k_stage01d<double, false, false>;
     return x_dtype == HG_U8 ? (StageFn2)k_stage01d<uint8_t> : x_dtype == HG_F32 ? (StageFn2)k_stage01d<float> : (StageFn2)k_stage01d<double>;
 }
@@ -806,7 +915,21 @@
 }
 int stage01p_tiles(bool rem4, bool fspec) { return fspec ? 1 : 2; }
 
-StageFn2 pick_stage01p(int x_dtype, bool stamp, bool rem4, bool fspec) {
+StageFn2 pick_stage01p(int x_dtype, bool stamp, bool rem4, bool fspec, bool fold, bool scalar) {
+    if (rem4 && fold && scalar) {
+        if (fspec)
+            return x_dtype == HG_U8 ? (StageFn2)k_stage01p<uint8_t, false, true, 1, 1, true, true>
+                                    : x_dtype == HG_F32 ? (StageFn2)k_stage01p<float, false, true, 1, 1, true, true> : (StageFn2)k_stage01p<double, false, true, 1, 1, true, true>;
+        return x_dtype == HG_U8 ? (StageFn2)k_stage01p<uint8_t, false, true, 2, 0, true, true>
+                                : x_dtype == HG_F32 ? (StageFn2)k_stage01p<float, false, true, 2, 0, true, true> : (StageFn2)k_stage01p<double, false, true, 2, 0, true, true>;
+    }
+    if (rem4 && fold) {
+        if (fspec)
+            return x_dtype == HG_U8 ? (StageFn2)k_stage01p<uint8_t, false, true, 1, 1, true>
+                                    : x_dtype == HG_F32 ? (StageFn2)k_stage01p<float, false, true, 1, 1, true> : (StageFn2)k_stage01p<double, false, true, 1, 1, true>;
+        return x_dtype == HG_U8 ? (StageFn2)k_stage01p<uint8_t, false, true, 2, 0, true>
+                                : x_dtype == HG_F32 ? (StageFn2)k_stage01p<float, false, true, 2, 0, true> : (StageFn2)k_stage01p<double, false, true, 2, 0, true>;
+    }
     if (rem4) {
 #ifdef HIGSFA_DIAG
         if (stamp && x_dtype == HG_F32) return fspec ? (StageFn2)k_stage01p<float, true, true, 1, 1> : (StageFn2)k_stage01p<float, true, true>;
diff --git a/pyfaceanalysis_amd/csrc/hg_fused_plan.cpp b/pyfaceanalysis_amd/csrc/hg_fused_plan.cpp
--- a/pyfaceanalysis_amd/csrc/hg_fused_plan.cpp
+++ b/pyfaceanalysis_amd/csrc/hg_fused_plan.cpp
@@ -144,6 +144,7 @@
     fn.A1 = std::move(A1);
     fn.A2 = std::move(A2);
     fn.is_ig = false;
+    fn.was_ig = true;
 }
 
 bool canon(const ChainT& c, int in_off, FNode& fn, std::string& why, const FusedOptions& opt) {
@@ -306,6 +307,44 @@
     return true;
 }
 
+namespace {
+struct LinkFold {
+    std::vector<double> bias;
+    std::vector<std::vector<double>> W;
+};
+LinkFold fold_link(const FStage& ch, const FStage& pa, int pj, const std::vector<int>& owner, const std::vector<int>& col0, const std::vector<int>& kids) {
+    const FNode& pn = pa.nodes[pj];
+    const int P = pn.A1.out;
+    LinkFold lf;
+    lf.bias = pn.A1.b;
+    lf.W.resize(ch.nodes.size());
+    for (int ci : kids) lf.W[ci].assign((size_t)ch.nodes[ci].A2.in * P, 0.0);
+    for (int c = 0; c < pn.in_dim; ++c) {
+        const int pc = pa.conn[pn.in_off + c], ci = owner[pc], k = pc - col0[ci];
+        const Aff& A2 = ch.nodes[ci].A2;
+        const double* w1 = &pn.A1.W[(size_t)c * P];
+        const double d = A2.b[k] - pn.A1.a[c];
+        for (int o = 0; o < P; ++o) lf.bias[o] += d * w1[o];
+        std::vector<double>& W = lf.W[ci];
+        for (int e = 0; e < A2.in; ++e) {
+            const double w2 = A2.W[(size_t)e * A2.out + k];
+            if (w2 == 0.0) continue;
+            for (int o = 0; o < P; ++o) W[(size_t)e * P + o] += w2 * w1[o];
+        }
+    }
+    for (int ci : kids) {
+        const Aff& A2 = ch.nodes[ci].A2;
+        for (int e = 0; e < A2.in; ++e) {
+            const double a = A2.a[e];
+            if (a == 0.0) continue;
+            for (int o = 0; o < P; ++o) lf.bias[o] -= a * lf.W[ci][(size_t)e * P + o];
+        }
+    }
+    return lf;
+}
+
+}
+
 std::vector<int> hoist_first_affines(std::vector<FStage>& fs, const FusedOptions& opt) {
     (void)opt;
     std::vector<int> parents;
@@ -360,30 +399,12 @@
         for (int pj = 0; pj < np; ++pj) {
             FNode& pn = pa.nodes[pj];
             const int P = pn.A1.out;
-            pn.sum_bias = pn.A1.b;
+            LinkFold lf = fold_link(ch, pa, pj, owner, col0, kids[pj]);
+            pn.sum_bias = std::move(lf.bias);
             pn.kids = kids[pj];
-            std::vector<std::vector<double>> Wf(nc);
-            for (int ci : kids[pj]) Wf[ci].assign((size_t)ch.nodes[ci].A2.in * P, 0.0);
-            for (int c = 0; c < pn.in_dim; ++c) {
-                const int pc = pa.conn[pn.in_off + c], ci = owner[pc], k = pc - col0[ci];
-                const Aff& A2 = ch.nodes[ci].A2;
-                const double* w1 = &pn.A1.W[(size_t)c * P];
-                const double d = A2.b[k] - pn.A1.a[c];
-                for (int o = 0; o < P; ++o) pn.sum_bias[o] += d * w1[o];
-                std::vector<double>& W = Wf[ci];
-                for (int e = 0; e < A2.in; ++e) {
-                    const double w2 = A2.W[(size_t)e * A2.out + k];
-                    if (w2 == 0.0) continue;
-                    for (int o = 0; o < P; ++o) W[(size_t)e * P + o] += w2 * w1[o];
-                }
-            }
+            std::vector<std::vector<double>>& Wf = lf.W;
             for (int ci : kids[pj]) {
                 FNode& cn = ch.nodes[ci];
-                for (int e = 0; e < cn.A2.in; ++e) {
-                    const double a = cn.A2.a[e];
-                    if (a == 0.0) continue;
-                    for (int o = 0; o < P; ++o) pn.sum_bias[o] -= a * Wf[ci][(size_t)e * P + o];
-                }
                 Aff f;
                 f.in = cn.A2.in;
                 f.out = P;
@@ -703,6 +724,7 @@
         if (fuse01) {
             stages[0].name += "  [+ stage 1 fused in the same persistent kernel when the input allows 16-byte loads]";
         }
+        if (opt.fold01) plan_fold01(fs);
         col_base.resize(out_dim);
         col_of.assign((size_t)std::max(prev_nb, 1) * 16, -1);
         for (int c = 0; c < out_dim; ++c) {
@@ -1420,6 +1442,104 @@
         }
     }
 
+    void plan_fold01(const std::vector<FStage>& fs) {
+        if (stages.size() < 2) return;
+        auto refuse = [&](const std::string& why) {
+            fold01_note = "link 0 -> 1 stays as it is: " + why;
+            stages[1].name += "  [" + fold01_note + "]";
+        };
+        if (!fuse01) {
+            bool ig = false;
+            for (size_t l = 0; l < 2 && l < fs.size(); ++l)
+                for (auto& n : fs[l].nodes) ig = ig || n.is_ig || n.was_ig;
+            return refuse(ig ? "an iGSFA front end" : "layers 0 and 1 do not share the front kernel");
+        }
+        const FStage &ch = fs[0], &pa = fs[1];
+        HostStage &a = stages[0], &b = stages[1];
+        for (auto& n : pa.nodes)
+            if (n.was_ig) return refuse("layer 1 is an iGSFA layer (identity first affine, no remainder tiles)");
+        for (auto& n : ch.nodes)
+            if (n.was_ig) return refuse("layer 0 is an iGSFA layer");
+        auto id_pow = [](const HostStage& hs) { return hs.nf == 2 && hs.funcs[0].kind == E_IDENTITY && hs.funcs[1].kind == E_ABS_POW; };
+        if (!id_pow(a) || !id_pow(b)) return refuse("both layers must expand with exactly (identity, |x|^p)");
+        if (opt.no_rem4) return refuse("4x4 remainder tiles are switched off (HIGSFA_NO_REM4)");
+        if (!(b.p_max >= 17 && b.p_max <= 20 && b.s_max >= 17 && b.s_max <= 20 && b.nk2[1][0] <= 1 && b.nk2[1][1] <= 1))
+            return refuse("layer 1 has no 4x4 remainder tiles (affines of " + std::to_string(b.p_max) + " and " + std::to_string(b.s_max) + " outputs, not 17..20)");
+        const int nc = (int)ch.nodes.size(), np = (int)pa.nodes.size();
+        std::vector<int> owner, col0(nc, 0);
+        for (int ci = 0; ci < nc; ++ci) {
+            col0[ci] = (int)owner.size();
+            owner.insert(owner.end(), ch.nodes[ci].out_dim, ci);
+        }
+        for (int q = 0; q < np; ++q) {
+            const FNode& pn = pa.nodes[q];
+            if (pn.A1.in != pn.in_dim) return refuse("internal: layer-1 first affine");
+            for (int c = 0; c < pn.in_dim; ++c) {
+                const int pc = pa.conn[pn.in_off + c];
+                if (pc < 0 || pc >= (int)owner.size() || owner[pc] >> 1 != q) return refuse("a layer-1 node reads other nodes than 2n and 2n + 1");
+            }
+        }
+        b.fold_frag.assign((size_t)np * 8 * 256, 0.f);
+        b.fold_bias.assign((size_t)np * 32, 0.f);
+        auto to4x4 = [](float* blk) {
+            float old[256];
+            std::copy(blk, blk + 256, old);
+            for (int l = 0; l < 64; ++l) {
+                const int src = (l & 48) | ((l & 3) << 2);
+                for (int r = 0; r < 4; ++r) blk[l * 4 + r] = old[src * 4 + r];
+            }
+        };
+        for (int q = 0; q < np; ++q) {
+            const FNode& pn = pa.nodes[q];
+            const int P = pn.A1.out;
+            const LinkFold lf = fold_link(ch, pa, q, owner, col0, {2 * q, 2 * q + 1});
+            for (int sl = 0; sl < 2; ++sl) {
+                const FNode& cn = ch.nodes[2 * q + sl];
+                const std::vector<double>& F = lf.W[2 * q + sl];
+                const int p0 = cn.A1.out;
+                int eo = 0;
+                for (int fi = 0; fi < 2; ++fi) {
+                    const int used = cn.funcs[fi].used(p0);
+                    for (int mt = 0; mt < 2; ++mt) {
+                        float* blk = b.fold_frag.data() + ((((size_t)q * 2 + sl) * 2 + fi) * 2 + mt) * 256;
+                        for (int lane = 0; lane < 64; ++lane) {
+                            const int i = lane & 15, gg = lane >> 4;
+                            const int fo = 16 * mt + q_of_row(i);
+                            if (fo >= P) continue;
+                            for (int r = 0; r < 4; ++r) {
+                                const int fz = 4 * r + gg;
+                                if (fz >= used) continue;
+                                blk[lane * 4 + r] = (float)F[(size_t)(eo + fz) * P + fo];
+                            }
+                        }
+                        if (mt == 1) to4x4(blk);
+                    }
+                    eo += cn.funcs[fi].out_dim(p0);
+                }
+            }
+            for (int mt = 0; mt < 2; ++mt)
+                for (int gg = 0; gg < 4; ++gg)
+                    for (int r = 0; r < 4; ++r) {
+                        const int fo = 16 * mt + 4 * r + gg;
+                        b.fold_bias[(size_t)q * 32 + mt * 16 + gg * 4 + r] = fo < P ? (float)lf.bias[fo] : 0.f;
+                    }
+        }
+        const int64_t before = padded_flops;
+        padded_flops -= (a.mfma16_tile * 2048 + a.mfma4_tile * 512) / 16 + (b.mfma16_tile * 2048 + b.mfma4_tile * 512) / 16;
+        a.mfma16_tile = a.ks1_tile;
+        a.mfma4_tile = 0;
+        b.mfma16_tile = a.ks2_tile + b.ks2_tile;
+        b.mfma4_tile = a.ks2_tile + b.ks2_tile;
+        padded_flops += (a.mfma16_tile * 2048 + a.mfma4_tile * 512) / 16 + (b.mfma16_tile * 2048 + b.mfma4_tile * 512) / 16;
+        fold01_flops = padded_flops - before;
+        fold01 = true;
+        fold01_note = "link 0 -> 1 folded: layer 0's second affine multiplied into this layer's first, z = bias' + sum over the two children of "
+                      "[z0, |z0|^p] (A2 A1[rows of the child, :]) inside the front kernel, which then issues " + std::to_string(a.mfma16_tile) +
+                      " x 16x16x4 for layer 0 and " + std::to_string(b.mfma16_tile) + " x 16x16x4 + " + std::to_string(b.mfma4_tile) +
+                      " x 4x4x1 for this layer (the counts on the two stage lines are the flow's as given)";
+        b.name += "  [" + fold01_note + "]";
+    }
+
     bool can_fuse01() const {
         if (stages.size() < 2) return false;
         const HostStage& a = stages[0];
@@ -1508,6 +1628,7 @@
             try {
                 FusedOptions o = opt;
                 o.hoist = false;
+                o.fold01 = false;
                 given = Planner(root, std::move(plain), o).padded_flops;
             } catch (const Error&) {
             }
@@ -1515,7 +1636,7 @@
     }
     try {
         Planner p(root, std::move(stages), opt);
-        p.padded_flops_given = given >= 0 ? given : p.padded_flops;
+        p.padded_flops_given = given >= 0 ? given : p.padded_flops - p.fold01_flops;
         return std::make_unique<const FusedPlan>(std::move(static_cast<FusedPlan&>(p)));
     } catch (const Error& e) {
         if (why_not) *why_not = e.what();
diff --git a/pyfaceanalysis_amd/csrc/hg_fused_plan.hpp b/pyfaceanalysis_amd/csrc/hg_fused_plan.hpp
--- a/pyfaceanalysis_amd/csrc/hg_fused_plan.hpp
+++ b/pyfaceanalysis_amd/csrc/hg_fused_plan.hpp
@@ -36,6 +36,7 @@
     int splitm_max_wgs = 512;
     int sum_lds_kib = 32;
     bool hoist = false;
+    bool fold01 = false;
     static FusedOptions from_env() {
         FusedOptions o;
         o.no_rem4 = getenv("HIGSFA_NO_REM4") != nullptr;
@@ -101,12 +102,15 @@
     std::string name;
     bool sum_in = false;
     int n_kids = 0;
+    std::vector<float> fold_frag, fold_bias;
 };
 
 struct FusedPlan {
     FusedOptions opt;
     int out_dim = 0;
     bool s0_transpose = false, fuse01 = false;
+    bool fold01 = false;
+    std::string fold01_note;
     std::vector<HostStage> stages;
     std::vector<int32_t> col_base, col_of;
     int tail_begin = -1;
@@ -114,6 +118,7 @@
     std::vector<SubRun> sub_runs;
     int max_nb = 0;
     int64_t padded_flops = 0;
+    int64_t fold01_flops = 0;
     int64_t padded_flops_given = 0;
 
     bool sub_run_pays(const SubRun& r, int n_tiles) const;
diff --git a/pyfaceanalysis_amd/csrc/hg_fused_stages.hpp b/pyfaceanalysis_amd/csrc/hg_fused_stages.hpp
--- a/pyfaceanalysis_amd/csrc/hg_fused_stages.hpp
+++ b/pyfaceanalysis_amd/csrc/hg_fused_stages.hpp
@@ -21,6 +21,7 @@
     bool has_clip = false;
     double clip_lo = 0, clip_hi = 0;
     bool is_ig = false, ig_has_lr = false;
+    bool was_ig = false;
     int ig_k = 0;
     std::vector<double> ig_mean;
     Aff ig_sfa, ig_lr, ig_pca;
```

New measurement: 9.496 million sub-images/s, median of 6. +1.6%, better.
